# dfm/tinygp

Measured on AMD Instinct MI355X. Metric: GP log_probability evals/sec + Cholesky TFLOP/s (fp64), N=16,384, higher is better.
Workload: dtype f64; 1 GPU; c2: 1.5^2 ExpSquared(2.5), 1-D X, N=16384, fp64, diag=0.01, constant-density synthetic inputs (SURVEY 8d), dense Cholesky + tri-solve; n=16384, d=1, parallelism=single, nb_outer=1024

## Files before the change

### tinygp_amd/csrc/capi.hip

```cpp
#include <cmath>
#include <cstdlib>
#include <chrono>
#include <cstring>
#include <string>

#include "tgp_common.h"
#define CHAIN_HD __host__ __device__
#include "chain_tasks.h"
#define TILE_HD
#include "tile_order.h"

namespace tgp {

static thread_local std::string g_error;

void set_error(const char* fmt, ...) {
  char buf[1024];
  va_list ap;
  va_start(ap, fmt);
  vsnprintf(buf, sizeof(buf), fmt, ap);
  va_end(ap);
  g_error = buf;
}

// ... 17 lines not shown
}

int ensure_work(tgp_ctx* ctx, size_t bytes) { return grow(&ctx->d_work, &ctx->work_bytes, bytes); }

template <typename F>
static int dispatch(int dtype, F&& f) {
  if (dtype == TGP_F64) return f(double{});
  if (dtype == TGP_F32) return f(float{});
  set_error("dtype must be TGP_F32 (0) or TGP_F64 (1), got %d", dtype);
  return TGP_E_ARG;
}

static inline size_t esize(int dtype) { return dtype == TGP_F64 ? 8 : 4; }

}

using namespace tgp;

struct tgp_solver {
  tgp_ctx* ctx = nullptr;
  int dtype = TGP_F64;
  int64_t n = 0, npad = 0;
  int d = 1;
  void* X = nullptr;
  void* diag = nullptr;
  void* A = nullptr;
  void* dinv = nullptr;
  void* vec = nullptr;
  void* vec2 = nullptr;
  void* resid = nullptr;
  void* scratch = nullptr;
  void* Minv = nullptr;
  void* winv = nullptr;
  bool winv_valid = false;
  size_t scratch_bytes = 0;
  KProg kp{};
  bool has_prog = false, factored = false, has_resid = false;
  int32_t info = 0;
  double logdet_half = 0;
  double ms[8] = {0, 0, 0, 0, 0, 0, 0, 0};
};

#define CTX_GUARD(ctx)                                                \
  TGP_ARG_CHECK((ctx) != nullptr, "null context");                    \
  std::unique_lock<std::recursive_mutex> _tgp_lock((ctx)->mu);        \
  TGP_HIP_TRY(hipSetDevice((ctx)->device))

#define SOLVER_GUARD(s)                                               \
  TGP_ARG_CHECK((s) != nullptr && (s)->ctx != nullptr, "null solver"); \
  std::unique_lock<std::recursive_mutex> _tgp_lock((s)->ctx->mu);     \
  TGP_HIP_TRY(hipSetDevice((s)->ctx->device))

template <typename T>
static int assemble_lower(tgp_ctx* ctx, const tgp::KProg& kp, int64_t n, int d, const T* X,
                          const T* diag, T* A, int64_t npad) {
  using namespace tgp;
  const int64_t tc = npad / 128;
  int64_t t1 = tc;
  if (ctx->lookahead != 0 && ctx->asm_stream != nullptr) {
    int64_t nb = ctx->nb_outer / 128;
    if (nb < 1) nb = 1;
    nb = std::max<int64_t>(nb, first_panel_cols(ctx, npad) / 128);
    if (nb < tc) t1 = nb;
  }
  const int flags = KMAT_LOWER | KMAT_PAD_IDENTITY;
  if (t1 < tc) {
    TGP_TRY(ev_record(ctx, ctx->ev_asm, ctx->stream));
    TGP_TRY(st_wait(ctx, ctx->asm_stream, ctx->ev_asm));
  }
  TGP_TRY(launch_kmat_cols<T>(ctx, ctx->stream, kp, n, n, d, X, X, diag, A, npad, npad, npad, flags, 0, t1));
  if (t1 < tc) {
    auto side = [=]() -> int {
      TGP_TRY(launch_kmat_cols<T>(ctx, ctx->asm_stream, kp, n, n, d, X, X, diag, A, npad, npad, npad,
                                  flags, t1, tc - t1));
      return ev_record(ctx, ctx->ev_asm, ctx->asm_stream);
    };
    if (ctx->asm_defer != 0) {
      ctx->deferred_asm = side;
    } else {
      TGP_TRY(side());
    }
    ctx->asm_pending = true;
  }
  return TGP_OK;
}

template <typename T>
static int ensure_winv(tgp_solver* s) {
  if (s->winv_valid) return TGP_OK;
  if (!s->winv) TGP_HIP_TRY(hipMalloc(&s->winv, 4 * size_t(s->npad / TILE) * 16384 * sizeof(T)));
  TGP_TRY(compute_winv<T>(s->ctx, s->npad, (const T*)s->A, s->npad, (T*)s->winv));
  s->winv_valid = true;
  return TGP_OK;
}

extern "C" {

int tgp_abi_version(void) { return TGP_ABI_VERSION; }
const char* tgp_last_error(void) { return g_error.c_str(); }

int tgp_ctx_create(int device, void* stream, tgp_ctx** out) {
  TGP_ARG_CHECK(out != nullptr, "null output pointer");
  int count = 0;
  hipError_t e = hipGetDeviceCount(&count);
  if (e != hipSuccess || count <= 0) {
    set_error("no HIP device visible (%s); tinygp_amd has no CPU fallback",
              e == hipSuccess ? "device count 0" : hipGetErrorString(e));
    return TGP_E_HIP;
  }
  TGP_ARG_CHECK(device >= 0 && device < count, "device %d out of range (0..%d)", device, count - 1);
  TGP_HIP_TRY(hipSetDevice(device));
  tgp_ctx* ctx = new tgp_ctx();
  ctx->device = device;
  ctx->has_device = true;
  if (stream) {
    ctx->stream = static_cast<hipStream_t>(stream);
  } else {
    TGP_HIP_TRY(hipStreamCreateWithFlags(&ctx->stream, hipStreamNonBlocking));
    ctx->own_stream = true;
  }
  int lo = 0, hi = 0;
  TGP_HIP_TRY(hipDeviceGetStreamPriorityRange(&lo, &hi));
  {
    int can = 0;
    if (hipDeviceGetAttribute(&can, hipDeviceAttributeCanUseStreamWaitValue, device) != hipSuccess) can = 0;
    (void)hipGetLastError();
    ctx->can_wait_value = can == 1;
  }
  {
    const char* a = getenv("ROCPROF_COUNTER_COLLECTION");
    const char* b = getenv("TGP_SERIALIZED_KERNELS");
    auto on = [](const char* v) { return v != nullptr && *v && strcmp(v, "0") != 0 && strcasecmp(v, "false") != 0; };
    if (on(a) || on(b)) {
      ctx->serializing_tool = true;
      ctx->chain_polls = 0;
    }
  }
  TGP_HIP_TRY(hipStreamCreateWithPriority(&ctx->panel_stream, hipStreamNonBlocking, hi));
  TGP_HIP_TRY(hipStreamCreateWithPriority(&ctx->update_stream, hipStreamNonBlocking, hi));
  TGP_HIP_TRY(hipStreamCreateWithPriority(&ctx->asm_stream, hipStreamNonBlocking, lo));
  TGP_HIP_TRY(hipEventCreateWithFlags(&ctx->ev_asm, hipEventDisableTiming));
  TGP_HIP_TRY(hipEventCreateWithFlags(&ctx->ev_d, hipEventDisableTiming));
  TGP_HIP_TRY(hipEventCreateWithFlags(&ctx->ev_e, hipEventDisableTiming));
  TGP_HIP_TRY(hipEventCreateWithFlags(&ctx->ev_f, hipEventDisableTiming));
  TGP_HIP_TRY(hipEventCreateWithFlags(&ctx->ev_g1, hipEventDisableTiming));
  TGP_HIP_TRY(hipEventCreateWithFlags(&ctx->ev_g2, hipEventDisableTiming));
  TGP_HIP_TRY(hipEventCreateWithFlags(&ctx->ev_h, hipEventDisableTiming));
  TGP_HIP_TRY(hipEventCreateWithFlags(&ctx->ev_i, hipEventDisableTiming));
  TGP_HIP_TRY(hipEventCreateWithFlags(&ctx->ev_j, hipEventDisableTiming));
  TGP_HIP_TRY(hipEventCreateWithFlags(&ctx->ev_c, hipEventDisableTiming));
  TGP_HIP_TRY(hipEventCreateWithFlags(&ctx->ev_join, hipEventDisableTiming));
  TGP_HIP_TRY(hipEventCreateWithFlags(&ctx->ev_a, hipEventDisableTiming));
  TGP_HIP_TRY(hipEventCreateWithFlags(&ctx->ev_b, hipEventDisableTiming));
  TGP_HIP_TRY(hipMalloc(&ctx->d_scal, 16 * sizeof(double)));
  TGP_HIP_TRY(hipMalloc(&ctx->d_info, sizeof(int32_t)));
  TGP_HIP_TRY(hipMalloc(&ctx->d_step_flag, 64));
  TGP_HIP_TRY(hipMemset(ctx->d_step_flag, 0, 64));
  TGP_HIP_TRY(hipMalloc(&ctx->d_chain_flags, size_t(tgp::CHAIN_MAX_ROW_TILES) * 64 * sizeof(uint32_t)));
  TGP_HIP_TRY(hipMemset(ctx->d_chain_flags, 0, size_t(tgp::CHAIN_MAX_ROW_TILES) * 64 * sizeof(uint32_t)));
  TGP_HIP_TRY(hipMalloc(&ctx->d_chain_ticket, 4096));
  TGP_HIP_TRY(hipMemset(ctx->d_chain_ticket, 0, 4096));
  TGP_HIP_TRY(hipMalloc(&ctx->d_chain_red, size_t(2) * CHAIN_MAX_ROW_TILES * sizeof(double)));
  hipDeviceProp_t prop;
  TGP_HIP_TRY(hipGetDeviceProperties(&prop, device));
  ctx->cus = prop.multiProcessorCount;
  *out = ctx;
  return TGP_OK;
}

int tgp_ctx_destroy(tgp_ctx* ctx) {
  if (!ctx) return TGP_OK;
  hipSetDevice(ctx->device);
  hipStreamSynchronize(ctx->stream);
  if (ctx->panel_stream) hipStreamSynchronize(ctx->panel_stream);
  if (ctx->solve_stream) {
    hipStreamSynchronize(ctx->solve_stream);
    hipStreamDestroy(ctx->solve_stream);
  }
  if (ctx->ev_c) hipEventDestroy(ctx->ev_c);
  if (ctx->ev_join) hipEventDestroy(ctx->ev_join);
  if (ctx->ev_asm_gate) hipEventDestroy(ctx->ev_asm_gate);
  if (ctx->rescue_stream) hipStreamDestroy(ctx->rescue_stream);
  if (ctx->update_stream) {
    hipStreamSynchronize(ctx->update_stream);
    hipStreamDestroy(ctx->update_stream);
  }
  if (ctx->asm_stream) {
    hipStreamSynchronize(ctx->asm_stream);
    hipStreamDestroy(ctx->asm_stream);
  }
  if (ctx->ev_asm) hipEventDestroy(ctx->ev_asm);
  if (ctx->ev_d) hipEventDestroy(ctx->ev_d);
  if (ctx->ev_e) hipEventDestroy(ctx->ev_e);
  if (ctx->ev_f) hipEventDestroy(ctx->ev_f);
  if (ctx->ev_g1) hipEventDestroy(ctx->ev_g1);
  if (ctx->ev_g2) hipEventDestroy(ctx->ev_g2);
  if (ctx->ev_h) hipEventDestroy(ctx->ev_h);
  if (ctx->ev_i) hipEventDestroy(ctx->ev_i);
  if (ctx->ev_j) hipEventDestroy(ctx->ev_j);
  for (auto e : ctx->ev_pool) hipEventDestroy(e);
  if (ctx->ev_a) hipEventDestroy(ctx->ev_a);
  if (ctx->ev_b) hipEventDestroy(ctx->ev_b);
  if (ctx->d_scal) hipFree(ctx->d_scal);
  if (ctx->d_info) hipFree(ctx->d_info);
  if (ctx->d_step_flag) hipFree(ctx->d_step_flag);
  if (ctx->d_chain_flags) hipFree(ctx->d_chain_flags);
  if (ctx->d_chain_ticket) hipFree(ctx->d_chain_ticket);
  if (ctx->d_chain_red) hipFree(ctx->d_chain_red);
  if (ctx->d_chain_stamps) hipFree(ctx->d_chain_stamps);
  for (auto& kv : ctx->chain_tables)
    if (kv.second.dev) hipFree(kv.second.dev);
  if (ctx->d_dinv) hipFree(ctx->d_dinv);
  if (ctx->d_work) hipFree(ctx->d_work);
  if (ctx->d_gemm_ws) hipFree(ctx->d_gemm_ws);
  if (ctx->d_gemm_prefix_count) hipFree(ctx->d_gemm_prefix_count);
  if (ctx->panel_stream) hipStreamDestroy(ctx->panel_stream);
  if (ctx->own_stream && ctx->stream) hipStreamDestroy(ctx->stream);
  delete ctx;
  return TGP_OK;
}

int tgp_ctx_sync(tgp_ctx* ctx) {
  CTX_GUARD(ctx);
  TGP_HIP_TRY(hipStreamSynchronize(ctx->stream));
  return TGP_OK;
}

static int64_t* option_slot(tgp_ctx* ctx, const char* key) {
  if (!strcmp(key, "nb_outer")) return &ctx->nb_outer;
  if (!strcmp(key, "lookahead")) return &ctx->lookahead;
  if (!strcmp(key, "profile")) return &ctx->profile;
  if (!strcmp(key, "first_split")) return &ctx->first_split;
  if (!strcmp(key, "first_small_tiles")) return &ctx->first_small_tiles;
  if (!strcmp(key, "keep_grad_buffers")) return &ctx->keep_grad_buffers;
  if (!strcmp(key, "stream_trsv")) return &ctx->stream_trsv;
  if (!strcmp(key, "trsv_groups")) return &ctx->trsv_groups;
  if (!strcmp(key, "nb_wide_rows")) return &ctx->nb_wide_rows;
  if (!strcmp(key, "dist_solve_aux")) return &ctx->dist_solve_aux;
  if (!strcmp(key, "solve_on_update")) return &ctx->solve_on_update;
  if (!strcmp(key, "fused_step")) return &ctx->fused_step;
  if (!strcmp(key, "chain_kernel")) return &ctx->chain_kernel;
  if (!strcmp(key, "chain_stamps")) return &ctx->chain_stamps;
  if (!strcmp(key, "chain_full_rows")) return &ctx->chain_full_rows;
  if (!strcmp(key, "chain_lds_pad")) return &ctx->chain_lds_pad;
  if (!strcmp(key, "chain_depth2")) return &ctx->chain_depth2;
  if (!strcmp(key, "chain_merged")) return &ctx->chain_merged;
  if (!strcmp(key, "chain_sub_panel")) return &ctx->chain_sub_panel;
  if (!strcmp(key, "chain_sub_min_rows")) return &ctx->chain_sub_min_rows;
  if (!strcmp(key, "chain_sub_role")) return &ctx->chain_sub_role;
  if (!strcmp(key, "chain_pre_wait")) return &ctx->chain_pre_wait;
  if (!strcmp(key, "chain_gate_split")) return &ctx->chain_gate_split;
  if (!strcmp(key, "chain_polls")) return &ctx->chain_polls;
  if (!strcmp(key, "chain_fwd_tasks")) return &ctx->chain_fwd_tasks;
  if (!strcmp(key, "chain_fast_update")) return &ctx->chain_fast_update;
  if (!strcmp(key, "chain_batch")) return &ctx->chain_batch;
  if (!strcmp(key, "chain_batch_lag")) return &ctx->chain_batch_lag;
  if (!strcmp(key, "chain_batch_rowlag")) return &ctx->chain_batch_rowlag;
  if (!strcmp(key, "chain_batch_minrows")) return &ctx->chain_batch_minrows;
  if (!strcmp(key, "kmat_plain_div")) return &ctx->kmat_plain_div;
  if (!strcmp(key, "chain_reserve")) return &ctx->chain_reserve;
  if (!strcmp(key, "gate_split")) return &ctx->gate_split;
  if (!strcmp(key, "reserve_max_tiles")) return &ctx->reserve_max_tiles;
  if (!strcmp(key, "sub_panel")) return &ctx->sub_panel;
  if (!strcmp(key, "sub_panel_min_rows")) return &ctx->sub_panel_min_rows;
  if (!strcmp(key, "nb_first")) return &ctx->nb_first;
  if (!strcmp(key, "split_tail")) return &ctx->split_tail;
  if (!strcmp(key, "gemm_role")) return &ctx->gemm_role;
  if (!strcmp(key, "gemm_reserve")) return &ctx->gemm_reserve;
  if (!strcmp(key, "gemm_prefix_cols")) return &ctx->gemm_prefix_cols;
  if (!strcmp(key, "gemm_prefix_count")) return &ctx->gemm_prefix_count;
  if (!strcmp(key, "host_join")) return &ctx->host_join;
  if (!strcmp(key, "late_join")) return &ctx->late_join;
  if (!strcmp(key, "chain_reduce")) return &ctx->chain_reduce;
  if (!strcmp(key, "asm_defer")) return &ctx->asm_defer;
  if (!strcmp(key, "tile_band")) return &ctx->tile_band;
  if (!strcmp(key, "fault_inject")) return &ctx->fault_inject;
  if (!strcmp(key, "poll_timeout_ms")) return &ctx->poll_timeout_ms;
  if (!strcmp(key, "timeout_retries")) return &ctx->timeout_retries;
  return nullptr;
}

static int set_option_checked(tgp_ctx* ctx, const char* key, int64_t value, int64_t* old) {
  int64_t* slot = option_slot(ctx, key);
  TGP_ARG_CHECK(slot != nullptr, "unknown option '%s'", key);
  if (slot == &ctx->nb_outer)
    TGP_ARG_CHECK(value >= TILE && value % TILE == 0, "nb_outer must be a positive multiple of %d", TILE);
  if (slot == &ctx->sub_panel || slot == &ctx->nb_first)
    TGP_ARG_CHECK(value >= 0 && value % TILE == 0, "%s must be a multiple of %d (0: off)", key, TILE);
  if (slot == &ctx->chain_batch) TGP_ARG_CHECK(value >= 0 && value <= 32, "chain_batch must be in [0, 32]");
  if (slot == &ctx->chain_batch_lag) TGP_ARG_CHECK(value >= 1 && value <= 64, "chain_batch_lag must be in [1, 64]");
  if (slot == &ctx->chain_batch_minrows) TGP_ARG_CHECK(value >= 0 && value <= 4096, "chain_batch_minrows must be in [0, 4096]");
  if (slot == &ctx->chain_batch_rowlag) TGP_ARG_CHECK(value >= 2 && value <= 4096, "chain_batch_rowlag must be in [2, 4096]");
  if (old) *old = *slot;
  if (slot == &ctx->poll_timeout_ms && ctx->has_device) return set_poll_limit(ctx, value);
  *slot = value;
  return TGP_OK;
}

int tgp_ctx_set_option(tgp_ctx* ctx, const char* key, int64_t value, int64_t* old) {
  TGP_ARG_CHECK(ctx != nullptr && key != nullptr, "null argument");
  return set_option_checked(ctx, key, value, old);
}

int tgp_ctx_get_option(tgp_ctx* ctx, const char* key, int64_t* value) {
  TGP_ARG_CHECK(ctx != nullptr && key != nullptr && value != nullptr, "null argument");
  int64_t* slot = option_slot(ctx, key);
  TGP_ARG_CHECK(slot != nullptr, "unknown option '%s'", key);
  if (slot == &ctx->poll_timeout_ms && ctx->has_device) ctx->poll_timeout_ms = tgp::poll_limit_ms();
  *value = *slot;
  return TGP_OK;
}

static int apply_options(tgp_ctx* ctx, const char* options) {
  if (options == nullptr) return TGP_OK;
  std::string all(options);
  size_t pos = 0;
  while (pos < all.size()) {
    size_t end = all.find(',', pos);
    if (end == std::string::npos) end = all.size();
    const std::string item = all.substr(pos, end - pos);
    pos = end + 1;
    if (item.empty()) continue;
    const size_t eq = item.find('=');
    TGP_ARG_CHECK(eq != std::string::npos && eq > 0, "option '%s' is not key=value", item.c_str());
    char* stop = nullptr;
    const long long v = strtoll(item.c_str() + eq + 1, &stop, 10);
    TGP_ARG_CHECK(stop != nullptr && *stop == 0 && eq + 1 < item.size(), "option '%s': bad integer", item.c_str());
    TGP_TRY(set_option_checked(ctx, item.substr(0, eq).c_str(), (int64_t)v, nullptr));
  }
  return TGP_OK;
}

int tgp_ctx_device_info(tgp_ctx* ctx, char* name, int name_len, int32_t* cus, int64_t* mem_bytes,
                        int32_t* clock_khz) {
  CTX_GUARD(ctx);
  hipDeviceProp_t prop;
  TGP_HIP_TRY(hipGetDeviceProperties(&prop, ctx->device));
  if (name && name_len > 0) {
    snprintf(name, (size_t)name_len, "%s (%s)", prop.name, prop.gcnArchName);
  }
  if (cus) *cus = prop.multiProcessorCount;
  if (mem_bytes) *mem_bytes = (int64_t)prop.totalGlobalMem;
  if (clock_khz) *clock_khz = prop.clockRate;
  return TGP_OK;
}

int tgp_malloc(tgp_ctx* ctx, size_t bytes, void** dev) {
  CTX_GUARD(ctx);
  TGP_ARG_CHECK(dev != nullptr, "null output pointer");
  TGP_HIP_TRY(hipMalloc(dev, bytes ? bytes : 8));
  return TGP_OK;
}
int tgp_free(tgp_ctx* ctx, void* dev) {
  CTX_GUARD(ctx);
  if (dev) {
    TGP_HIP_TRY(hipStreamSynchronize(ctx->stream));
    TGP_HIP_TRY(hipFree(dev));
  }
  return TGP_OK;
}
int tgp_memcpy_h2d(tgp_ctx* ctx, void* dst, const void* src, size_t bytes) {
  CTX_GUARD(ctx);
  TGP_HIP_TRY(hipMemcpyAsync(dst, src, bytes, hipMemcpyHostToDevice, ctx->stream));
  TGP_HIP_TRY(hipStreamSynchronize(ctx->stream));
  return TGP_OK;
}
int tgp_memcpy_d2h(tgp_ctx* ctx, void* dst, const void* src, size_t bytes) {
  CTX_GUARD(ctx);
  TGP_HIP_TRY(hipMemcpyAsync(dst, src, bytes, hipMemcpyDeviceToHost, ctx->stream));
  TGP_HIP_TRY(hipStreamSynchronize(ctx->stream));
  return TGP_OK;
}
int tgp_memset(tgp_ctx* ctx, void* dst, int byte, size_t bytes) {
  CTX_GUARD(ctx);
  TGP_HIP_TRY(hipMemsetAsync(dst, byte, bytes, ctx->stream));
  return TGP_OK;
}

int tgp_kmat(tgp_ctx* ctx, int dtype, const tgp_kop* prog, int nops, int64_t n1, int64_t n2,
             int32_t d, const void* X1, const void* X2, const void* diag, void* out, int64_t ld,
             int64_t rows_out, int64_t cols_out, int lower_only) {
  CTX_GUARD(ctx);
  KProg kp;
  TGP_TRY(make_kprog(prog, nops, &kp));
  TGP_ARG_CHECK(n1 >= 0 && n2 >= 0 && X1 && X2 && out, "kmat: null or negative argument");
  return dispatch(dtype, [&](auto tag) {
    using T = decltype(tag);
    const int flags = (lower_only ? KMAT_LOWER : 0) | KMAT_PAD_IDENTITY;
    return launch_kmat<T>(ctx, kp, n1, n2, d, (const T*)X1, (const T*)X2, (const T*)diag, (T*)out,
                          ld, rows_out, cols_out, flags);
  });
}

int tgp_kdiag(tgp_ctx* ctx, int dtype, const tgp_kop* prog, int nops, int64_t n, int32_t d,
              const void* X, void* out) {
  CTX_GUARD(ctx);
  KProg kp;
  TGP_TRY(make_kprog(prog, nops, &kp));
  return dispatch(dtype, [&](auto tag) {
    using T = decltype(tag);
    return launch_kdiag<T>(ctx, kp, n, d, (const T*)X, (const T*)nullptr, (T*)out);
  });
}

int tgp_kmat_gemv(tgp_ctx* ctx, int dtype, const tgp_kop* prog, int nops, int64_t n1, int64_t n2,
                  int32_t d, const void* X1, const void* X2, const void* v, void* out) {
  CTX_GUARD(ctx);
  KProg kp;
  TGP_TRY(make_kprog(prog, nops, &kp));
  return dispatch(dtype, [&](auto tag) {
    using T = decltype(tag);
    return launch_kmat_gemv<T>(ctx, kp, n1, n2, d, (const T*)X1, (const T*)X2, (const T*)v, (T*)out);
  });
}

int tgp_kmat_gemv_multi(tgp_ctx* ctx, int dtype, const tgp_kop* prog, int nops, int64_t n1, int64_t n2,
                        int32_t d, const void* X1, const void* X2, const void* V, int64_t nv, void* out) {
  CTX_GUARD(ctx);
  KProg kp;
  TGP_TRY(make_kprog(prog, nops, &kp));
  TGP_ARG_CHECK(nv >= 1 && X1 && X2 && V && out, "kmat_gemv_multi: bad argument");
  return dispatch(dtype, [&](auto tag) {
    using T = decltype(tag);
    return launch_kmat_gemv_multi<T>(ctx, kp, n1, n2, d, (const T*)X1, (const T*)X2, (const T*)V, nv, (T*)out);
  });
}

int tgp_potrf(tgp_ctx* ctx, int dtype, int64_t n, void* A, int64_t ld, int32_t* info) {
  CTX_GUARD(ctx);
  TGP_ARG_CHECK(A != nullptr && n >= 0, "potrf: null matrix");
  TGP_TRY(ensure_dinv(ctx, size_t(n / TILE + 1) * 2048 * esize(dtype)));
  return dispatch(dtype, [&](auto tag) {
    using T = decltype(tag);
    return potrf<T>(ctx, n, (T*)A, ld, (T*)ctx->d_dinv, info);
  });
}

int tgp_trsv(tgp_ctx* ctx, int dtype, int64_t n, const void* L, int64_t ld, int transpose, void* y) {
  CTX_GUARD(ctx);
  TGP_TRY(ensure_dinv(ctx, size_t(n / TILE + 1) * 2048 * esize(dtype)));
  return dispatch(dtype, [&](auto tag) {
    using T = decltype(tag);
    TGP_TRY(compute_dinv<T>(ctx, n, (const T*)L, ld, (T*)ctx->d_dinv));
    return trsv<T>(ctx, n, (const T*)L, ld, (const T*)ctx->d_dinv, transpose, (T*)y);
  });
}

int tgp_trsm_right_lt(tgp_ctx* ctx, int dtype, int64_t m, int64_t n, const void* L, int64_t ldl,
                      void* B, int64_t ldb) {
  CTX_GUARD(ctx);
  TGP_TRY(ensure_dinv(ctx, size_t(n / TILE + 1) * 2048 * esize(dtype)));
  return dispatch(dtype, [&](auto tag) {
    using T = decltype(tag);
    TGP_TRY(compute_dinv<T>(ctx, n, (const T*)L, ldl, (T*)ctx->d_dinv));
    return trsm_right_lt<T>(ctx, m, n, (const T*)L, ldl, (const T*)ctx->d_dinv, (T*)B, ldb);
  });
}

int tgp_gemv_sub(tgp_ctx* ctx, int dtype, int64_t m, int64_t k, const void* P, int64_t ld,
                 const void* x, void* y) {
  CTX_GUARD(ctx);
  return dispatch(dtype, [&](auto tag) {
    using T = decltype(tag);
    return gemv_sub<T>(ctx, m, k, (const T*)P, ld, (const T*)x, (T*)y);
  });
}

int tgp_gemm_nt(tgp_ctx* ctx, int dtype, int64_t m, int64_t n, int64_t k, double alpha,
                const void* A, int64_t lda, const void* B, int64_t ldb, double beta, void* C,
                int64_t ldc, int lower) {
  CTX_GUARD(ctx);
  int mode;
  if (alpha == -1.0 && beta == 1.0) mode = 0;
  else if (alpha == 1.0 && beta == 0.0) mode = 1;
  else {
    set_error("gemm_nt: (alpha, beta) must be (-1, 1) or (1, 0)");
    return TGP_E_UNSUPPORTED;
  }
  const bool counted = ctx->gemm_role == 0 && ctx->gemm_prefix_cols > 0;
  if (ctx->gemm_role == 0) ctx->reserve_hint = ctx->gemm_reserve;
  if (counted) {
    if (!ctx->d_gemm_prefix_count) TGP_HIP_TRY(hipMalloc(&ctx->d_gemm_prefix_count, sizeof(int32_t)));
    TGP_HIP_TRY(hipMemsetAsync(ctx->d_gemm_prefix_count, 0, sizeof(int32_t), ctx->stream));
    ctx->prefix_hint_cols = ctx->gemm_prefix_cols;
    ctx->prefix_hint_counter = ctx->d_gemm_prefix_count;
  }
  const int rc = dispatch(dtype, [&](auto tag) {
    using T = decltype(tag);
    return launch_gemm_nt<T>(ctx, ctx->stream, m, n, k, (const T*)A, lda, (const T*)B, ldb, (T*)C,
                             ldc, lower, mode, (int)ctx->gemm_role);
  });
  ctx->reserve_hint = 0;
  ctx->prefix_hint_cols = 0;
  ctx->prefix_hint_counter = nullptr;
  if (counted && rc == TGP_OK) {
    int32_t done = 0;
    TGP_HIP_TRY(hipStreamSynchronize(ctx->stream));
    TGP_HIP_TRY(hipMemcpy(&done, ctx->d_gemm_prefix_count, sizeof(int32_t), hipMemcpyDeviceToHost));
    ctx->gemm_prefix_count = done;
  }
  return rc;
}

int tgp_sum_log_diag(tgp_ctx* ctx, int dtype, int64_t n, const void* L, int64_t ld, double* out) {
  CTX_GUARD(ctx);
  TGP_TRY(dispatch(dtype, [&](auto tag) {
    using T = decltype(tag);
    return launch_sum_log_diag<T>(ctx, n, (const T*)L, ld, 0);
  }));
  TGP_HIP_TRY(hipMemcpyAsync(out, ctx->d_scal, sizeof(double), hipMemcpyDeviceToHost, ctx->stream));
  TGP_HIP_TRY(hipStreamSynchronize(ctx->stream));
  return TGP_OK;
}

int tgp_sum_squares(tgp_ctx* ctx, int dtype, int64_t n, const void* y, double* out) {
  CTX_GUARD(ctx);
  TGP_TRY(dispatch(dtype, [&](auto tag) {
    using T = decltype(tag);
    return launch_sum_squares<T>(ctx, n, (const T*)y, 0);
  }));
  TGP_HIP_TRY(hipMemcpyAsync(out, ctx->d_scal, sizeof(double), hipMemcpyDeviceToHost, ctx->stream));
  TGP_HIP_TRY(hipStreamSynchronize(ctx->stream));
  return TGP_OK;
}

int tgp_ubench_mfma(tgp_ctx* ctx, int dtype, double* tflops_out) {
  CTX_GUARD(ctx);
  TGP_ARG_CHECK(tflops_out != nullptr && (dtype == TGP_F32 || dtype == TGP_F64), "bad argument");
  return ubench_mfma(ctx, dtype, tflops_out);
}

int tgp_ubench(tgp_ctx* ctx, int kind, int blocks_per_cu, double* tflops_out,
               double* cycles_per_op_out) {
  CTX_GUARD(ctx);
  TGP_ARG_CHECK(tflops_out != nullptr, "null output pointer");
  return ubench(ctx, kind, blocks_per_cu, tflops_out, cycles_per_op_out);
}

static int solver_scratch(tgp_solver* s, size_t bytes) {
  return tgp::grow(&s->scratch, &s->scratch_bytes, bytes);
}

int tgp_solver_create(tgp_ctx* ctx, int dtype, int64_t n, int32_t d, const void* X_host,
                      const void* noise_diag_host, tgp_solver** out) {
  CTX_GUARD(ctx);
  TGP_ARG_CHECK(out != nullptr, "null output pointer");
  TGP_ARG_CHECK(dtype == TGP_F32 || dtype == TGP_F64, "dtype must be TGP_F32 or TGP_F64");
  TGP_ARG_CHECK(n >= 1, "need at least one data point (n = %lld)", (long long)n);
  TGP_ARG_CHECK(d >= 1 && d <= TGP_MAX_DIM, "input dimension must be 1..%d (got %d)", TGP_MAX_DIM, d);
  TGP_ARG_CHECK(X_host != nullptr && noise_diag_host != nullptr, "null input array");
  tgp_solver* s = new tgp_solver();
  s->ctx = ctx;
  s->dtype = dtype;
  s->n = n;
  s->npad = round_up(n, TILE);
  s->d = d;
  const size_t es = esize(dtype);
  auto fail = [&](int code) { tgp_solver_destroy(s); return code; };
#define S_TRY(expr) do { hipError_t _e = (expr); if (_e != hipSuccess) { \
    set_error("%s failed: %s", #expr, hipGetErrorString(_e));            \
    return fail(_e == hipErrorOutOfMemory ? TGP_E_NOMEM : TGP_E_HIP); } } while (0)
  S_TRY(hipMalloc(&s->X, size_t(n) * d * es));
  S_TRY(hipMalloc(&s->diag, size_t(n) * es));
  S_TRY(hipMalloc(&s->A, size_t(s->npad) * s->npad * es));
  S_TRY(hipMalloc(&s->dinv, size_t(s->npad / TILE) * 2048 * es));
  S_TRY(hipMalloc(&s->vec, size_t(s->npad) * es));
  S_TRY(hipMalloc(&s->vec2, size_t(s->npad) * es));
  S_TRY(hipMalloc(&s->resid, size_t(s->npad) * es));
  S_TRY(hipMemcpyAsync(s->X, X_host, size_t(n) * d * es, hipMemcpyHostToDevice, ctx->stream));
  S_TRY(hipMemcpyAsync(s->diag, noise_diag_host, size_t(n) * es, hipMemcpyHostToDevice, ctx->stream));
  S_TRY(hipMemsetAsync(s->vec, 0, size_t(s->npad) * es, ctx->stream));
  S_TRY(hipMemsetAsync(s->vec2, 0, size_t(s->npad) * es, ctx->stream));
  S_TRY(hipMemsetAsync(s->resid, 0, size_t(s->npad) * es, ctx->stream));
  S_TRY(hipStreamSynchronize(ctx->stream));
#undef S_TRY
  *out = s;
  return TGP_OK;
}

int tgp_solver_destroy(tgp_solver* s) {
  if (!s) return TGP_OK;
  if (s->ctx) {
    hipSetDevice(s->ctx->device);
    hipStreamSynchronize(s->ctx->stream);
  }
  void* bufs[] = {s->X, s->diag, s->A, s->dinv, s->vec, s->vec2, s->resid, s->scratch, s->Minv, s->winv};
  for (void* b : bufs)
    if (b) hipFree(b);
  delete s;
  return TGP_OK;
}

int tgp_solver_set_noise(tgp_solver* s, const void* noise_diag_host) {
  SOLVER_GUARD(s);
  TGP_ARG_CHECK(noise_diag_host != nullptr, "null input array");
  TGP_HIP_TRY(hipMemcpyAsync(s->diag, noise_diag_host, size_t(s->n) * esize(s->dtype),
                             hipMemcpyHostToDevice, s->ctx->stream));
  TGP_HIP_TRY(hipStreamSynchronize(s->ctx->stream));
  return TGP_OK;
}

static int upload_vec(tgp_solver* s, void* dst, const void* src_host) {
  const size_t es = esize(s->dtype);
  TGP_HIP_TRY(hipMemcpyAsync(dst, src_host, size_t(s->n) * es, hipMemcpyHostToDevice, s->ctx->stream));
  if (s->npad > s->n)
    TGP_HIP_TRY(hipMemsetAsync((char*)dst + size_t(s->n) * es, 0, size_t(s->npad - s->n) * es,
                               s->ctx->stream));
  return TGP_OK;
}

static int factor_body(tgp_solver* s, const tgp_kop* prog, int nops, const void* cov_host,
                       int32_t* info, int fused, const void* resid_host, double* logprob);

static int factor_impl(tgp_solver* s, const tgp_kop* prog, int nops, const void* cov_host,
                       int32_t* info, int fused, const void* resid_host, double* logprob) {
  int st = factor_body(s, prog, nops, cov_host, info, fused, resid_host, logprob);
  if (st == TGP_E_TIMEOUT && s->ctx->chain_kernel != 0) {
    tgp_ctx* ctx = s->ctx;
    for (hipStream_t q : {ctx->asm_stream, ctx->panel_stream, ctx->update_stream, ctx->solve_stream, ctx->stream})
      if (q) (void)hipStreamSynchronize(q);
    (void)hipGetLastError();
    ctx->asm_pending = false;
    ctx->deferred_asm = nullptr;
    ctx->ev_used = 0;
    ctx->timeout_retries++;
    const int64_t keep = ctx->chain_kernel;
    ctx->chain_kernel = 0;
    st = factor_body(s, prog, nops, cov_host, info, fused, resid_host, logprob);
    ctx->chain_kernel = keep;
  }
  if (st < 0) {
    tgp_ctx* ctx = s->ctx;
    ctx->asm_pending = false;
    ctx->deferred_asm = nullptr;
    ctx->ev_used = 0;
    s->factored = false;
    for (hipStream_t q : {ctx->asm_stream, ctx->panel_stream, ctx->update_stream, ctx->solve_stream,
                          ctx->stream})
      if (q) (void)hipStreamSynchronize(q);
    (void)hipGetLastError();
  }
  return st;
}

static int factor_body(tgp_solver* s, const tgp_kop* prog, int nops, const void* cov_host,
                       int32_t* info, int fused, const void* resid_host, double* logprob) {
  tgp_ctx* ctx = s->ctx;
  if (nops > 0) {
    TGP_TRY(make_kprog(prog, nops, &s->kp));
    s->has_prog = true;
  } else {
    s->has_prog = false;
  }
  TGP_ARG_CHECK(s->has_prog || cov_host != nullptr, "factor needs a kernel program or a covariance");
  s->winv_valid = false;
  const auto host0 = std::chrono::steady_clock::now();
  const size_t es = esize(s->dtype);
  hipEvent_t e0 = nullptr, e1 = nullptr, e2 = nullptr;
  const bool prof = ctx->profile != 0;
  if (prof) {
    TGP_HIP_TRY(hipEventCreate(&e0));
    TGP_HIP_TRY(hipEventCreate(&e1));
    TGP_HIP_TRY(hipEventCreate(&e2));
    TGP_HIP_TRY(hipEventRecord(e0, ctx->stream));
  }
  int status = dispatch(s->dtype, [&](auto tag) {
    using T = decltype(tag);
    T* A = (T*)s->A;
    if (fused) {
      if (resid_host) {
        TGP_TRY(upload_vec(s, s->vec, resid_host));
      } else {
        TGP_ARG_CHECK(s->has_resid, "no resident residual: call tgp_solver_set_resid first");
        TGP_HIP_TRY(hipMemcpyAsync(s->vec, s->resid, size_t(s->npad) * es, hipMemcpyDeviceToDevice,
                                   ctx->stream));
      }
    }
    if (cov_host != nullptr) {
      TGP_TRY(solver_scratch(s, size_t(s->n) * s->n * es));
      TGP_HIP_TRY(hipMemcpyAsync(s->scratch, cov_host, size_t(s->n) * s->n * es,
                                 hipMemcpyHostToDevice, ctx->stream));
      TGP_TRY(launch_set_lower_from_rowmajor<T>(ctx, s->n, s->npad, (const T*)s->scratch, A, s->npad));
    } else {
      TGP_TRY(assemble_lower<T>(ctx, s->kp, s->n, s->d, (const T*)s->X, (const T*)s->diag, A, s->npad));
    }
    if (prof) TGP_HIP_TRY(hipEventRecord(e1, ctx->stream));
    int32_t inf = 0;
    ctx->defer_join = ctx->late_join != 0;
    ctx->join_deferred = false;
    reductions_begin(ctx, s->npad, fused != 0);
    int st = potrf<T>(ctx, s->npad, A, s->npad, (T*)s->dinv, &inf, fused ? (T*)s->vec : (T*)nullptr);
    ctx->defer_join = false;
    const bool reduce = reductions_end(ctx);
    if (st < 0) return st;
    s->info = inf;
    if (prof) TGP_HIP_TRY(hipEventRecord(e2, ctx->stream));
    if (reduce) {
      TGP_TRY(launch_sum_log_diag<T>(ctx, s->n, A, s->npad, 1));
      if (fused) TGP_TRY(launch_sum_squares<T>(ctx, s->n, (const T*)s->vec, 0));
    }
    return TGP_OK;
  });
  if (status < 0) return status;
  double two[2] = {0, 0};
  int32_t inf_late = 0;
  const bool late = ctx->join_deferred;
  ctx->join_deferred = false;
  TGP_HIP_TRY(hipMemcpyAsync(two, ctx->d_scal, 2 * sizeof(double), hipMemcpyDeviceToHost, ctx->stream));
  if (late) TGP_HIP_TRY(hipMemcpyAsync(&inf_late, ctx->d_info, sizeof(int32_t), hipMemcpyDeviceToHost, ctx->stream));
  TGP_HIP_TRY(hipStreamSynchronize(ctx->stream));
  if (late) {
    if (inf_late == INT32_MIN) {
      tgp::set_error("potrf: a device-side hand-off did not arrive within poll_timeout_ms (a lost or starved chain launch)");
      if (prof) { hipEventDestroy(e0); hipEventDestroy(e1); hipEventDestroy(e2); }
      return TGP_E_TIMEOUT;
    }
    s->info = inf_late;
  }
  s->ms[5] = std::chrono::duration<double, std::milli>(ctx->submitted - host0).count();
  s->logdet_half = two[1];
  if (fused && logprob)
    *logprob = -0.5 * two[0] - (s->logdet_half + 0.5 * double(s->n) * std::log(2.0 * M_PI));
  if (prof) {
    float a = 0, b = 0;
    TGP_HIP_TRY(hipEventElapsedTime(&a, e0, e1));
    TGP_HIP_TRY(hipEventElapsedTime(&b, e1, e2));
    s->ms[0] = a;
    s->ms[1] = b;
    s->ms[2] = ctx->prof_syrk_ms;
    s->ms[3] = (double)ctx->prof_syrk_launches;
    s->ms[6] = ctx->prof_syrk_flops;
    s->ms[7] = ctx->prof_syrk_union_ms;
    hipEventDestroy(e0);
    hipEventDestroy(e1);
    hipEventDestroy(e2);
  }
  s->factored = true;
  if (info) *info = s->info;
  return s->info > 0 ? s->info : TGP_OK;
}

int tgp_solver_factor(tgp_solver* s, const tgp_kop* prog, int nops, const void* cov_host,
                      int32_t* info) {
  SOLVER_GUARD(s);
  return factor_impl(s, prog, nops, cov_host, info, 0, nullptr, nullptr);
}

int tgp_solver_factor_logprob(tgp_solver* s, const tgp_kop* prog, int nops, const void* cov_host,
                              const void* resid_host, int32_t* info, double* logprob) {
  SOLVER_GUARD(s);
  TGP_ARG_CHECK(logprob != nullptr, "null output pointer");
  return factor_impl(s, prog, nops, cov_host, info, 1, resid_host, logprob);
}

#define NEED_FACTOR(s) TGP_ARG_CHECK((s)->factored, "solver has not been factored yet")

int tgp_solver_normalization(tgp_solver* s, double* out) {
  SOLVER_GUARD(s);
  NEED_FACTOR(s);
  TGP_ARG_CHECK(out != nullptr, "null output pointer");
  *out = s->logdet_half + 0.5 * double(s->n) * std::log(2.0 * M_PI);
  return TGP_OK;
}

int tgp_solver_solve_tri(tgp_solver* s, int transpose, int64_t nrhs, const void* y_host,
                         void* x_host) {
  SOLVER_GUARD(s);
  NEED_FACTOR(s);
  TGP_ARG_CHECK(nrhs >= 1 && y_host && x_host, "solve_tri: bad argument");
  tgp_ctx* ctx = s->ctx;
  const size_t es = esize(s->dtype);
  return dispatch(s->dtype, [&](auto tag) {
    using T = decltype(tag);
    const T* L = (const T*)s->A;
    if (nrhs == 1) {
      TGP_TRY(upload_vec(s, s->vec, y_host));
      const T* winv = nullptr;
      if (ctx->stream_trsv != 0 && s->info == 0) {
        TGP_TRY(ensure_winv<T>(s));
        winv = (const T*)s->winv;
      }
      TGP_TRY(trsv<T>(ctx, s->npad, L, s->npad, (const T*)s->dinv, transpose, (T*)s->vec, winv));
      TGP_HIP_TRY(hipMemcpyAsync(x_host, s->vec, size_t(s->n) * es, hipMemcpyDeviceToHost, ctx->stream));
      TGP_HIP_TRY(hipStreamSynchronize(ctx->stream));
      return TGP_OK;
    }
    if (!transpose) {
      const int64_t mpad = round_up(nrhs, TILE);
      TGP_TRY(solver_scratch(s, size_t(mpad) * s->npad * es));
      TGP_HIP_TRY(hipMemsetAsync(s->scratch, 0, size_t(mpad) * s->npad * es, ctx->stream));
      TGP_HIP_TRY(hipMemcpy2DAsync(s->scratch, size_t(mpad) * es, y_host, size_t(nrhs) * es,
                                   size_t(nrhs) * es, size_t(s->n), hipMemcpyHostToDevice, ctx->stream));
      TGP_TRY(trsm_right_lt<T>(ctx, mpad, s->npad, L, s->npad, (const T*)s->dinv, (T*)s->scratch, mpad));
      TGP_HIP_TRY(hipMemcpy2DAsync(x_host, size_t(nrhs) * es, s->scratch, size_t(mpad) * es,
                                   size_t(nrhs) * es, size_t(s->n), hipMemcpyDeviceToHost, ctx->stream));
      TGP_HIP_TRY(hipStreamSynchronize(ctx->stream));
      return TGP_OK;
    }
    const T* winv_t = nullptr;
    if (ctx->stream_trsv != 0 && s->info == 0) {
      TGP_TRY(ensure_winv<T>(s));
      winv_t = (const T*)s->winv;
    }
    for (int64_t r = 0; r < nrhs; ++r) {
      TGP_HIP_TRY(hipMemsetAsync(s->vec, 0, size_t(s->npad) * es, ctx->stream));
      TGP_HIP_TRY(hipMemcpy2DAsync(s->vec, es, (const char*)y_host + r * es, size_t(nrhs) * es, es,
                                   size_t(s->n), hipMemcpyHostToDevice, ctx->stream));
      TGP_TRY(trsv<T>(ctx, s->npad, L, s->npad, (const T*)s->dinv, 1, (T*)s->vec, winv_t));
      TGP_HIP_TRY(hipMemcpy2DAsync((char*)x_host + r * es, size_t(nrhs) * es, s->vec, es, es,
                                   size_t(s->n), hipMemcpyDeviceToHost, ctx->stream));
    }
    TGP_HIP_TRY(hipStreamSynchronize(ctx->stream));
    return TGP_OK;
  });
}

int tgp_solver_dot_tri(tgp_solver* s, int64_t nrhs, const void* y_host, void* out_host) {
  SOLVER_GUARD(s);
  NEED_FACTOR(s);
  TGP_ARG_CHECK(nrhs >= 1 && y_host && out_host, "dot_tri: bad argument");
  tgp_ctx* ctx = s->ctx;
  const size_t es = esize(s->dtype);
  return dispatch(s->dtype, [&](auto tag) {
    using T = decltype(tag);
    if (nrhs >= 8) {
      const int64_t mpad = round_up(nrhs, TILE);
      const size_t bytes = size_t(mpad) * s->npad * es;
      TGP_TRY(solver_scratch(s, 2 * bytes));
      char* Zt = (char*)s->scratch;
      char* Ct = Zt + bytes;
      TGP_HIP_TRY(hipMemsetAsync(Zt, 0, bytes, ctx->stream));
      TGP_HIP_TRY(hipMemcpy2DAsync(Zt, size_t(mpad) * es, y_host, size_t(nrhs) * es, size_t(nrhs) * es,
                                   size_t(s->n), hipMemcpyHostToDevice, ctx->stream));
      TGP_TRY(launch_gemm_nt<T>(ctx, ctx->stream, mpad, s->npad, s->npad, (const T*)Zt, mpad,
                                (const T*)s->A, s->npad, (T*)Ct, mpad, 0, 3, 1));
      TGP_HIP_TRY(hipMemcpy2DAsync(out_host, size_t(nrhs) * es, Ct, size_t(mpad) * es, size_t(nrhs) * es,
                                   size_t(s->n), hipMemcpyDeviceToHost, ctx->stream));
      TGP_HIP_TRY(hipStreamSynchronize(ctx->stream));
      return TGP_OK;
    }
    for (int64_t r = 0; r < nrhs; ++r) {
      TGP_HIP_TRY(hipMemcpy2DAsync(s->vec, es, (const char*)y_host + r * es, size_t(nrhs) * es, es,
                                   size_t(s->n), hipMemcpyHostToDevice, ctx->stream));
      TGP_TRY(launch_trmv_lower<T>(ctx, s->n, (const T*)s->A, s->npad, (const T*)s->vec, (T*)s->vec2));
      TGP_HIP_TRY(hipMemcpy2DAsync((char*)out_host + r * es, size_t(nrhs) * es, s->vec2, es, es,
                                   size_t(s->n), hipMemcpyDeviceToHost, ctx->stream));
    }
    TGP_HIP_TRY(hipStreamSynchronize(ctx->stream));
    return TGP_OK;
  });
}

int tgp_solver_set_resid(tgp_solver* s, const void* resid_host) {
  SOLVER_GUARD(s);
  TGP_ARG_CHECK(resid_host != nullptr, "null input array");
  TGP_TRY(upload_vec(s, s->resid, resid_host));
  TGP_HIP_TRY(hipStreamSynchronize(s->ctx->stream));
  s->has_resid = true;
  return TGP_OK;
}

static int logprob_device(tgp_solver* s, const void* resid_host, double* out) {
  tgp_ctx* ctx = s->ctx;
// ... 425 lines not shown
```

### tinygp_amd/csrc/chol.hip

```cpp
#include <algorithm>
#include <atomic>
#include <functional>
#include <type_traits>

#include <thread>

#include "tgp_common.h"
#define CHAIN_HD __host__ __device__
#include "chain_tasks.h"

namespace tgp {

namespace {

typedef double d4 __attribute__((ext_vector_type(4)));
typedef float f4 __attribute__((ext_vector_type(4)));

template <typename T> struct Mfma;
template <> struct Mfma<double> {
  using acc_t = d4;
  static __device__ __forceinline__ acc_t mma(double a, double b, acc_t c) {
    return __builtin_amdgcn_mfma_f64_16x16x4f64(a, b, c, 0, 0, 0);
  }
  static __device__ __forceinline__ int drow(int lane, int r) { return (lane >> 4) + 4 * r; }
  static constexpr bool FAST4 = false;
  static __device__ __forceinline__ double mma4(double a, double b, double c) {
    return __builtin_amdgcn_mfma_f64_4x4x4f64(a, b, c, 0, 0, 0);
  }
  static __device__ __forceinline__ int rot4(int lane, int t) { return 4 * ((((lane >> 2) & 3) + t) & 3) + (lane & 3); }
  static __device__ __forceinline__ int arow4(int lane) { return 4 * ((lane >> 2) & 3) + (lane >> 4); }
};
template <> struct Mfma<float> {
  using acc_t = f4;
  static __device__ __forceinline__ acc_t mma(float a, float b, acc_t c) {
    return __builtin_amdgcn_mfma_f32_16x16x4f32(a, b, c, 0, 0, 0);
  }
  static __device__ __forceinline__ int drow(int lane, int r) { return (lane >> 4) * 4 + r; }
  static constexpr bool FAST4 = false;
  static __device__ __forceinline__ float mma4(float a, float b, float c) { return c + a * b; }
  static __device__ __forceinline__ int rot4(int lane, int t) { return (lane + t) & 15; }
  static __device__ __forceinline__ int arow4(int lane) { return lane & 15; }
};

__device__ __forceinline__ double fast_rcp(double x) {
  double r = __builtin_amdgcn_rcp(x);
  double e = __builtin_fma(-x, r, 1.0);
  r = __builtin_fma(r, e, r);
  e = __builtin_fma(-x, r, 1.0);
  return __builtin_fma(r, e, r);
}
__device__ __forceinline__ float fast_rcp(float x) {
  float r = __builtin_amdgcn_rcpf(x);
  float e = __builtin_fmaf(-x, r, 1.0f);
  return __builtin_fmaf(r, e, r);
}
__device__ __forceinline__ double fast_rsqrt(double x) {
  double y = __builtin_amdgcn_rsq(x);
  double e = __builtin_fma(-x * y, y, 1.0);
  y = __builtin_fma(0.5 * y, e, y);
  e = __builtin_fma(-x * y, y, 1.0);
  return __builtin_fma(0.5 * y, e, y);
}
__device__ __forceinline__ float fast_rsqrt(float x) {
  float y = __builtin_amdgcn_rsqf(x);
  float e = __builtin_fmaf(-x * y, y, 1.0f);
  return __builtin_fmaf(0.5f * y, e, y);
}

__device__ __forceinline__ double readlane(double v, int lane) {
  int lo = __double2loint(v), hi = __double2hiint(v);
  lo = __builtin_amdgcn_readlane(lo, lane);
  hi = __builtin_amdgcn_readlane(hi, lane);
  return __hiloint2double(hi, lo);
}
__device__ __forceinline__ float readlane(float v, int lane) {
  return __int_as_float(__builtin_amdgcn_readlane(__float_as_int(v), lane));
}

#define TGP_HD __device__ __forceinline__
#include "potf2_layout.h"
#define TGP_OPAQUE_VGPR(x) asm volatile("" : "+v"(x))

#ifdef TGP_POTF2_STAMPS
__device__ long long g_potf2_stamps[64];
#define POTF2_STAMP(i) do { if (threadIdx.x == 0) g_potf2_stamps[i] = __builtin_readcyclecounter(); } while (0)
#else
#define POTF2_STAMP(i) do {} while (0)
#endif

__device__ void potf2_prefix_wait(const int32_t* count, int32_t target, int32_t* info);

template <typename T, bool FOLD>
__global__ __launch_bounds__(512) __attribute__((amdgpu_waves_per_eu(4, 4))) void potf2_kernel(T* __restrict__ A, int64_t ld,
                                                    T* __restrict__ dinv,
                                                    int32_t* __restrict__ info,
                                                    int32_t pivot_base,
                                                    const T* __restrict__ Xp, int64_t ldx,
                                                    const int32_t* __restrict__ wait_count, int32_t wait_target) {
  __shared__ __attribute__((aligned(16))) T S[36 * 256];
  __shared__ T Rs[2 * 16];
  __shared__ T Dg[256];
  if (wait_count != nullptr) {
    if (threadIdx.x == 0) potf2_prefix_wait(wait_count, wait_target, info);
    __syncthreads();
  }
#include "potf2_body.inc"
}

constexpr int32_t STEP_TIMEOUT = INT32_MIN;

__device__ long long g_poll_limit = 400000000LL;
struct PollClock {
  long long t0 = 0;
  __device__ __forceinline__ bool expired(long spin) {
    if ((spin & 255) != 255) return false;
    const long long now = (long long)__builtin_amdgcn_s_memrealtime();
    if (t0 == 0) {
      t0 = now;
      return false;
    }
    return now - t0 > __hip_atomic_load(&g_poll_limit, __ATOMIC_RELAXED, __HIP_MEMORY_SCOPE_AGENT);
  }
};
__device__ __forceinline__ bool poisoned(const int32_t* info) {
  return __hip_atomic_load(info, __ATOMIC_RELAXED, __HIP_MEMORY_SCOPE_AGENT) == STEP_TIMEOUT;
}

template <typename T, bool FOLD>
__device__ __forceinline__ void trsm_fold_body(T* S, int it, const T* __restrict__ Ljj,
                                               int64_t ld, const T* __restrict__ dinv,
                                               const T* __restrict__ Xp, const uint32_t* flag,
                                               uint32_t epoch, int wait_flag, int32_t* info) {
  using M = Mfma<T>;
  using acc_t = typename M::acc_t;
  typedef T T2 __attribute__((ext_vector_type(2)));
  const int tid = threadIdx.x, lane = tid & 63;
  const int w = __builtin_amdgcn_readfirstlane(tid >> 6);
  const int lrow = lane & 15, lk = lane >> 4;
  __builtin_amdgcn_s_setprio(2);
  T* Bt = const_cast<T*>(Ljj) + TILE + int64_t(it) * TILE;

  if constexpr (FOLD) {
    constexpr int FK = 16, F_LD = 144;
    static_assert(4 * FK * F_LD == 36 * 256, "the fold's operand buffers are exactly potf2's tile image");
    T* sA = S;
    T* sB = S + 2 * FK * F_LD;
    const T* Xi = Xp + TILE + int64_t(it) * TILE;
    const int wr = w >> 1, wc = w & 1;
    T2 ra[2], rb[2];
    auto load_global = [&](int kt) {
#pragma unroll
      for (int r = 0; r < 2; ++r) {
        const int64_t kk = int64_t(kt) * FK + w + 8 * r;
        ra[r] = *reinterpret_cast<const T2*>(Xi + kk * ld + lane * 2);
        rb[r] = *reinterpret_cast<const T2*>(Xp + kk * ld + lane * 2);
      }
    };
    auto store_lds = [&](int buf) {
#pragma unroll
      for (int r = 0; r < 2; ++r) {
        const int kk = w + 8 * r;
        *reinterpret_cast<T2*>(&sA[buf * FK * F_LD + kk * F_LD + lane * 2]) = ra[r];
        *reinterpret_cast<T2*>(&sB[buf * FK * F_LD + kk * F_LD + lane * 2]) = rb[r];
      }
    };
    acc_t acc[4][2];
#pragma unroll
    for (int a = 0; a < 4; ++a)
#pragma unroll
      for (int b = 0; b < 2; ++b) acc[a][b] = acc_t{0, 0, 0, 0};
    load_global(0);
    store_lds(0);
    __syncthreads();
    constexpr int nkt = TILE / FK;
    for (int kt = 0; kt < nkt; ++kt) {
      const int buf = kt & 1;
      if (kt + 1 < nkt) load_global(kt + 1);
      const T* pa = &sB[buf * FK * F_LD + lk * F_LD + wc * 64 + lrow];
      const T* pb = &sA[buf * FK * F_LD + lk * F_LD + wr * 32 + lrow];
#pragma unroll
      for (int ks = 0; ks < FK / 4; ++ks) {
        T aop[4], bop[2];
#pragma unroll
        for (int a = 0; a < 4; ++a) aop[a] = pa[ks * 4 * F_LD + a * 16];
#pragma unroll
        for (int b = 0; b < 2; ++b) bop[b] = pb[ks * 4 * F_LD + b * 16];
#pragma unroll
        for (int a = 0; a < 4; ++a)
#pragma unroll
          for (int b = 0; b < 2; ++b) acc[a][b] = M::mma(aop[a], bop[b], acc[a][b]);
      }
      if (kt + 1 < nkt) store_lds(buf ^ 1);
      __syncthreads();
    }
    T* Cu = Bt + int64_t(wc * 64) * ld + wr * 32;
    const uint32_t coff = uint32_t(M::drow(lane, 0) * int(ld) + lrow);
#pragma unroll
    for (int a = 0; a < 4; ++a) {
      T c[2][4];
#pragma unroll
      for (int b = 0; b < 2; ++b)
#pragma unroll
        for (int r = 0; r < 4; ++r) c[b][r] = (Cu + int64_t(a * 16 + M::drow(0, r)) * ld + b * 16)[coff];
#pragma unroll
      for (int b = 0; b < 2; ++b)
#pragma unroll
        for (int r = 0; r < 4; ++r) (Cu + int64_t(a * 16 + M::drow(0, r)) * ld + b * 16)[coff] = c[b][r] - acc[a][b][r];
      __builtin_amdgcn_sched_barrier(0);
    }
    __syncthreads();
  }

  T* bu = Bt + w * 16;
  const uint32_t boff = uint32_t(M::drow(lane, 0) * int(ld) + lrow);
  acc_t V[8];
#pragma unroll
  for (int jb = 0; jb < 8; ++jb)
#pragma unroll
    for (int r = 0; r < 4; ++r) V[jb][r] = (bu + int64_t(jb * 16 + M::drow(0, r)) * ld)[boff];
  asm volatile("s_waitcnt vmcnt(0)" ::: "memory");
  __builtin_amdgcn_sched_barrier(0);

  if (wait_flag) {
    if (tid == 0) {
      uint32_t seen = __hip_atomic_load(flag, __ATOMIC_RELAXED, __HIP_MEMORY_SCOPE_AGENT);
      PollClock clk;
      for (unsigned spin = 0; seen != epoch; ++spin) {
        __builtin_amdgcn_s_sleep(2);
        seen = __hip_atomic_load(flag, __ATOMIC_RELAXED, __HIP_MEMORY_SCOPE_AGENT);
        if (clk.expired(spin)) break;
      }
      if (seen != epoch) atomicExch(info, STEP_TIMEOUT);
      __builtin_amdgcn_fence(__ATOMIC_ACQUIRE, "agent");
    }
    __syncthreads();
  }

  {
    T tr[5][4];
#pragma unroll
    for (int trip = 0; trip < 5; ++trip) {
      const int b = w + 8 * trip;
      if (b < 36) {
        int i = 0;
        while ((i + 1) * (i + 2) / 2 <= b) ++i;
        const int j = b - i * (i + 1) / 2;
        if (i == j) {
#pragma unroll
          for (int q = 0; q < 4; ++q) tr[trip][q] = dinv[i * 256 + q * 64 + lane];
        } else {
          const int voff = lk * int(ld) + lrow;
#pragma unroll
          for (int q = 0; q < 4; ++q) tr[trip][q] = (Ljj + int64_t(j * 16 + q * 4) * ld + i * 16)[voff];
        }
      }
    }
#pragma unroll
    for (int trip = 0; trip < 5; ++trip) {
      const int b = w + 8 * trip;
      if (b < 36) {
#pragma unroll
        for (int q = 0; q < 4; ++q) S[b * 256 + q * 64 + lane] = tr[trip][q];
      }
    }
  }
  __syncthreads();
  T* bs = bu;
  asm volatile("" : "+s"(bs));
#pragma unroll
  for (int jb = 0; jb < 8; ++jb) {
    acc_t acc = V[jb], acc2 = acc_t{0, 0, 0, 0};
#pragma unroll
    for (int kb = 0; kb < jb; ++kb) {
      const T* Lb = &S[blk(jb, kb)];
#pragma unroll
      for (int s = 0; s < 4; ++s) {
        const T l = Lb[M::drow(lane, s) * 16 + lrow];
        if (s & 1) acc2 = M::mma(l, V[kb][s], acc2);
        else acc = M::mma(l, V[kb][s], acc);
      }
    }
    acc += acc2;
    const T* Db = &S[blk(jb, jb)];
    acc_t y = acc_t{0, 0, 0, 0}, y2 = acc_t{0, 0, 0, 0};
#pragma unroll
    for (int s = 0; s < 4; ++s) {
      const T d = Db[M::drow(lane, s) * 16 + lrow];
      if (s & 1) y2 = M::mma(d, acc[s], y2);
      else y = M::mma(d, acc[s], y);
    }
    y += y2;
#pragma unroll
    for (int r = 0; r < 4; ++r) (bs + int64_t(jb * 16 + M::drow(0, r)) * ld)[boff] = y[r];
    V[jb] = -y;
  }
}

template <typename T, bool FOLD>
__global__ __launch_bounds__(512) __attribute__((amdgpu_waves_per_eu(4, 4))) void panel_step_kernel(
    T* __restrict__ A, int64_t ld, T* __restrict__ dinv, int32_t* __restrict__ info, int32_t pivot_base,
    const T* __restrict__ Xp, int has_p, uint32_t* __restrict__ flag, uint32_t epoch) {
  __shared__ __attribute__((aligned(16))) T S[36 * 256];
  __shared__ T Rs[2 * 16];
  __shared__ T Dg[256];
  const int b = __builtin_amdgcn_readfirstlane(blockIdx.x);
  if (b < has_p) {
    {
      const int64_t ldx = ld;
#include "potf2_body.inc"
    }
    asm volatile("s_waitcnt vmcnt(0)" ::: "memory");
    __syncthreads();
    if (threadIdx.x == 0) {
      __builtin_amdgcn_fence(__ATOMIC_RELEASE, "agent");
      asm volatile("s_waitcnt vmcnt(0)" ::: "memory");
      __hip_atomic_store(flag, epoch, __ATOMIC_RELAXED, __HIP_MEMORY_SCOPE_AGENT);
    }
    return;
  }
  trsm_fold_body<T, FOLD>(S, b - has_p, A, ld, dinv, Xp, flag, epoch, has_p, info);
}

template <typename T> struct AgentBits;
template <> struct AgentBits<double> { using t = unsigned long long; };
template <> struct AgentBits<float> { using t = unsigned int; };
template <typename T>
__device__ __forceinline__ void st_agent(T* p, T v) {
  typename AgentBits<T>::t b;
  __builtin_memcpy(&b, &v, sizeof(T));
  __hip_atomic_store(reinterpret_cast<typename AgentBits<T>::t*>(p), b, __ATOMIC_RELAXED, __HIP_MEMORY_SCOPE_AGENT);
}

__device__ __forceinline__ void chain_stamp(long long* st, int k) {
  if (st != nullptr && threadIdx.x == 0) st[4 + k] = (long long)__builtin_amdgcn_s_memrealtime();
}

constexpr int CHAIN_FLAG_LD = 64;
constexpr uint32_t CHAIN_FINAL = 127;
constexpr int CHAIN_COLCNT_OFF = 16;
constexpr int CHAIN_QCNT_OFF = 96;
constexpr int CHAIN_XSTEP_OFF = 160;
constexpr int CHAIN_ZFLAG_OFF = 224;
constexpr int CHAIN_YSTATE_OFF = 288;
constexpr int CHAIN_TICKET_WORDS = CHAIN_YSTATE_OFF + int(CHAIN_MAX_ROW_TILES) / CHAIN_FWD_GROUP;
constexpr int CHAIN_PREFIX_OFF = CHAIN_TICKET_WORDS + 16;

template <typename T>
struct ChainArgs {
  T* A0;
  int64_t ld;
  T* dinv;
  int32_t* info;
  uint32_t* flags;
  int32_t* ticket;
  uint32_t epoch32;
  int32_t pivot_base;
  int32_t R;
  int32_t nblk;
  int32_t cb, ce;
  long long* stamps;
  int32_t launch;
  int32_t fast_update;
  const uint64_t* tasks;
  T* y;
  int32_t fgs;
  int32_t fprev;
  double* red;
  double* scal;
  int32_t red_total;
};

template <int NAP>
__device__ __forceinline__ void chain_wait(const uint32_t* f0, uint32_t v0, const uint32_t* f1, uint32_t v1,
                                           const uint32_t* f2, uint32_t v2, int32_t* info) {
  if (threadIdx.x < 64) {
    const int lane = threadIdx.x;
    const uint32_t* f = lane == 0 ? f0 : (lane == 1 ? f1 : (lane == 2 ? f2 : nullptr));
    const uint32_t want = lane == 0 ? v0 : (lane == 1 ? v1 : v2);
    bool ok = f == nullptr || __hip_atomic_load(f, __ATOMIC_RELAXED, __HIP_MEMORY_SCOPE_AGENT) == want;
    unsigned spin = 0;
    PollClock clk;
    while (!__all(ok)) {
      __builtin_amdgcn_s_sleep(NAP);
      if (!ok) ok = __hip_atomic_load(f, __ATOMIC_RELAXED, __HIP_MEMORY_SCOPE_AGENT) == want;
      bool dead = false;
      if ((spin & 255) == 255 && lane == 0)
        dead = clk.expired(spin) || poisoned(info);
      ++spin;
      if (__any(dead)) {
        if (lane == 0) atomicExch(info, STEP_TIMEOUT);
        break;
      }
    }
    if (lane == 0) __builtin_amdgcn_fence(__ATOMIC_ACQUIRE, "agent");
  }
  __syncthreads();
}

__device__ __forceinline__ void chain_publish(uint32_t* word, uint32_t value, int32_t* colcnt = nullptr) {
  asm volatile("s_waitcnt vmcnt(0)" ::: "memory");
  __syncthreads();
  if (threadIdx.x == 0) {
    __hip_atomic_store(word, value, __ATOMIC_RELAXED, __HIP_MEMORY_SCOPE_AGENT);
    if (colcnt != nullptr) __hip_atomic_fetch_add(colcnt, 1, __ATOMIC_RELAXED, __HIP_MEMORY_SCOPE_AGENT);
  }
}

__device__ void potf2_prefix_wait(const int32_t* count, int32_t target, int32_t* info) {
  PollClock clk;
  for (unsigned spin = 0;; ++spin) {
    if (__hip_atomic_load(count, __ATOMIC_RELAXED, __HIP_MEMORY_SCOPE_AGENT) >= target) break;
    __builtin_amdgcn_s_sleep(8);
    if ((spin & 255) == 255 && (clk.expired(spin) || poisoned(info))) {
      atomicExch(info, STEP_TIMEOUT);
      break;
    }
  }
  __builtin_amdgcn_fence(__ATOMIC_ACQUIRE, "agent");
}

__global__ __launch_bounds__(64) void chain_poll_kernel(const int32_t* __restrict__ count, int32_t target,
                                                        int32_t* __restrict__ info) {
  if (threadIdx.x != 0) return;
  PollClock clk;
  for (unsigned spin = 0;; ++spin) {
    if (__hip_atomic_load(count, __ATOMIC_RELAXED, __HIP_MEMORY_SCOPE_AGENT) >= target) break;
    __builtin_amdgcn_s_sleep(16);
    if ((spin & 255) == 255 && (clk.expired(spin) || poisoned(info))) {
      atomicExch(info, STEP_TIMEOUT);
      break;
    }
  }
}

template <typename T, int PARTS>
__device__ __forceinline__ void chain_update_full(const ChainArgs<T>& q, T* S, int i, int c, int k, int part) {
  static_assert(PARTS == 1 || PARTS == 4 || PARTS == 8, "whole tile, row quarters or row eighths");
  using M = Mfma<T>;
  using acc_t = typename M::acc_t;
  typedef T T2 __attribute__((ext_vector_type(2)));
  const int tid = threadIdx.x, lane = tid & 63;
  const int w = __builtin_amdgcn_readfirstlane(tid >> 6);
  const int lrow = lane & 15, lk = lane >> 4;
  const int64_t ld = q.ld;
  constexpr int FK = 16, F_LD = 144;
  static_assert(4 * FK * F_LD == 36 * 256, "the operand buffers are exactly potf2's tile image");
  T* sA = S;
  T* sB = S + 2 * FK * F_LD;
  const int rbase = PARTS == 1 ? (w >> 1) * 32 : (PARTS == 4 ? part * 32 : part * 16);
  const int cbase = PARTS == 1 ? (w & 1) * 64 : w * 16;
  constexpr int NA = PARTS == 1 ? 4 : 1;
  constexpr int NBR = PARTS == 8 ? 1 : 2;
  acc_t acc[NA][NBR];
#pragma unroll
  for (int a = 0; a < NA; ++a)
#pragma unroll
    for (int b = 0; b < NBR; ++b) acc[a][b] = acc_t{0, 0, 0, 0};
  const T* Xi = q.A0 + int64_t(k) * TILE * ld + int64_t(i) * TILE;
  const T* Xj = q.A0 + int64_t(k) * TILE * ld + int64_t(c) * TILE;
  T2 ra[2], rb[2];
  auto load_global = [&](int kt) {
#pragma unroll
    for (int r = 0; r < 2; ++r) {
      const int64_t kk = int64_t(kt) * FK + w + 8 * r;
      ra[r] = *reinterpret_cast<const T2*>(Xi + kk * ld + lane * 2);
      rb[r] = *reinterpret_cast<const T2*>(Xj + kk * ld + lane * 2);
    }
  };
  auto store_lds = [&](int buf) {
#pragma unroll
    for (int r = 0; r < 2; ++r) {
      const int kk = w + 8 * r;
      *reinterpret_cast<T2*>(&sA[buf * FK * F_LD + kk * F_LD + lane * 2]) = ra[r];
      *reinterpret_cast<T2*>(&sB[buf * FK * F_LD + kk * F_LD + lane * 2]) = rb[r];
    }
  };
  int rot[4];
#pragma unroll
  for (int t = 0; t < 4; ++t) rot[t] = M::rot4(lane, t);
  load_global(0);
  store_lds(0);
  __syncthreads();
  constexpr int nkt = TILE / FK;
  for (int kt = 0; kt < nkt; ++kt) {
    const int buf = kt & 1;
    if (kt + 1 < nkt) load_global(kt + 1);
    const T* pa = &sB[buf * FK * F_LD + lk * F_LD + cbase + lrow];
    if constexpr (M::FAST4) {
      const T* pb = &sA[buf * FK * F_LD + lk * F_LD + rbase];
#pragma unroll
      for (int ks = 0; ks < FK / 4; ++ks) {
        T aop[NA];
#pragma unroll
        for (int a = 0; a < NA; ++a) aop[a] = pa[ks * 4 * F_LD + a * 16];
#pragma unroll
        for (int b = 0; b < NBR; ++b) {
          T bop[4];
#pragma unroll
          for (int t = 0; t < 4; ++t) bop[t] = pb[ks * 4 * F_LD + b * 16 + rot[t]];
#pragma unroll
          for (int a = 0; a < NA; ++a)
#pragma unroll
            for (int t = 0; t < 4; ++t) acc[a][b][t] = M::mma4(aop[a], bop[t], acc[a][b][t]);
        }
      }
    } else {
      const T* pb = &sA[buf * FK * F_LD + lk * F_LD + rbase + lrow];
#pragma unroll
      for (int ks = 0; ks < FK / 4; ++ks) {
        T aop[NA], bop[NBR];
#pragma unroll
        for (int a = 0; a < NA; ++a) aop[a] = pa[ks * 4 * F_LD + a * 16];
#pragma unroll
        for (int b = 0; b < NBR; ++b) bop[b] = pb[ks * 4 * F_LD + b * 16];
#pragma unroll
        for (int a = 0; a < NA; ++a)
#pragma unroll
          for (int b = 0; b < NBR; ++b) acc[a][b] = M::mma(aop[a], bop[b], acc[a][b]);
      }
    }
    if (kt + 1 < nkt) store_lds(buf ^ 1);
    __syncthreads();
  }
  T* Cu = q.A0 + int64_t(c) * TILE * ld + int64_t(i) * TILE + int64_t(cbase) * ld + rbase;
  if constexpr (M::FAST4) {
    const int64_t ccol = M::arow4(lane);
#pragma unroll
    for (int a = 0; a < NA; ++a) {
      T cc[NBR][4];
      T* col = Cu + (int64_t(a * 16) + ccol) * ld;
#pragma unroll
      for (int b = 0; b < NBR; ++b)
#pragma unroll
        for (int t = 0; t < 4; ++t) cc[b][t] = col[b * 16 + rot[t]];
#pragma unroll
      for (int b = 0; b < NBR; ++b)
#pragma unroll
        for (int t = 0; t < 4; ++t) st_agent(col + b * 16 + rot[t], T(cc[b][t] - acc[a][b][t]));
      __builtin_amdgcn_sched_barrier(0);
    }
  } else {
    const uint32_t coff = uint32_t(M::drow(lane, 0) * int(ld) + lrow);
#pragma unroll
    for (int a = 0; a < NA; ++a) {
      T cc[NBR][4];
#pragma unroll
      for (int b = 0; b < NBR; ++b)
#pragma unroll
        for (int r = 0; r < 4; ++r) cc[b][r] = (Cu + int64_t(a * 16 + M::drow(0, r)) * ld + b * 16)[coff];
#pragma unroll
      for (int b = 0; b < NBR; ++b)
#pragma unroll
        for (int r = 0; r < 4; ++r)
          st_agent(Cu + int64_t(a * 16 + M::drow(0, r)) * ld + b * 16 + coff, T(cc[b][r] - acc[a][b][r]));
      __builtin_amdgcn_sched_barrier(0);
    }
  }
}

__device__ __forceinline__ void chain_update_fast(const ChainArgs<double>& q, double* S, int i, int c, int k, int k1) {
  using M = Mfma<double>;
  const int tid = threadIdx.x, lane = tid & 63;
  const int wu = __builtin_amdgcn_readfirstlane(tid >> 6);
  const int wr = wu >> 1, wc = wu & 1;
  const int lk = lane >> 4, lrow = lane & 15;
  constexpr int FK = 16, F_LD = 144;
  const int64_t ld = q.ld;
  const double* Xi = q.A0 + int64_t(k) * TILE * ld + int64_t(i) * TILE;
  const double* Xj = q.A0 + int64_t(k) * TILE * ld + int64_t(c) * TILE;
  double* sA = S;
  double* sB = S + 2 * FK * F_LD;
  const uint32_t lds_a = uint32_t(size_t((__attribute__((address_space(3))) double*)(sA))) + uint32_t(wu * F_LD * 8);
  const uint32_t lds_b = uint32_t(size_t((__attribute__((address_space(3))) double*)(sB))) + uint32_t(wu * F_LD * 8);
  const uint32_t lane16 = uint32_t(lane) * 16u;
  auto issue_tile = [&](int kt, int buf) {
#pragma unroll
    for (int r = 0; r < 2; ++r) {
      const double* ap = Xi + (int64_t(kt) * FK + wu + 8 * r) * ld;
      const double* bp = Xj + (int64_t(kt) * FK + wu + 8 * r) * ld;
// ... 130 lines not shown
        for (int tt = 0; tt < 5; ++tt) {
          if (tt < nt) {
            const int t = t0 + tt;
            const bool first = t <= pr;
            const int jj = first ? t : t - pr - 1;
            Cf[tt] = M::mma(row[jj * 16], first ? b1 : b2, Cf[tt]);
          }
        }
      }
    }
  }
  T* Acc = q.A0 + int64_t(c) * TILE * ld + int64_t(c) * TILE;
#pragma unroll
  for (int tt = 0; tt < 5; ++tt) {
    if (tt < nt) {
      const int t = t0 + tt;
      const bool first = t <= pr;
      const int ii = first ? i1 : i2, jj = first ? t : t - pr - 1;
#pragma unroll
      for (int r = 0; r < 4; ++r) {
        const int br = M::FAST4 ? M::rot4(lane, r) : lrow, bc = M::FAST4 ? M::arow4(lane) : M::drow(lane, r);
        T* pe = Acc + int64_t(jj * 16 + bc) * ld + ii * 16 + br;
        st_agent(pe, T(*pe - Cf[tt][r]));
      }
    }
  }
}

template <typename T>
__device__ __forceinline__ void chain_load_tile(const ChainArgs<T>& q, int i, int c, typename Mfma<T>::acc_t (&V)[8]) {
  using M = Mfma<T>;
  const int lane = threadIdx.x & 63;
  const int w = __builtin_amdgcn_readfirstlane(threadIdx.x >> 6);
  const int64_t ld = q.ld;
  const T* bu = q.A0 + int64_t(c) * TILE * ld + int64_t(i) * TILE + w * 16;
  const uint32_t boff = uint32_t(M::drow(lane, 0) * int(ld) + (lane & 15));
#pragma unroll
  for (int jb = 0; jb < 8; ++jb)
#pragma unroll
    for (int r = 0; r < 4; ++r) V[jb][r] = (bu + int64_t(jb * 16 + M::drow(0, r)) * ld)[boff];
  asm volatile("s_waitcnt vmcnt(0)" ::: "memory");
  __builtin_amdgcn_sched_barrier(0);
}

template <typename T>
__device__ __forceinline__ void chain_solve(const ChainArgs<T>& q, T* S, int i, int c,
                                            typename Mfma<T>::acc_t (&V)[8], long long* st, int s0) {
  using M = Mfma<T>;
  using acc_t = typename M::acc_t;
  const int tid = threadIdx.x, lane = tid & 63;
  const int w = __builtin_amdgcn_readfirstlane(tid >> 6);
  const int lrow = lane & 15, lk = lane >> 4;
  const int64_t ld = q.ld;
  T* Bt = q.A0 + int64_t(c) * TILE * ld + int64_t(i) * TILE;
  const T* Ljj = q.A0 + int64_t(c) * TILE * ld + int64_t(c) * TILE;
  const T* dinv = q.dinv + int64_t(c) * 2048;
  T* bu = Bt + w * 16;
  const uint32_t boff = uint32_t(M::drow(lane, 0) * int(ld) + lrow);
#pragma unroll
  for (int round = 0; round < 2; ++round) {
    constexpr int NTR = 3;
    T tr[NTR][4];
    const int t_lo = round * NTR, t_n = round == 0 ? NTR : 5 - NTR;
#pragma unroll
    for (int tq = 0; tq < NTR; ++tq) {
      const int b = w + 8 * (t_lo + tq);
      if (tq < t_n && b < 36) {
        int bi = 0;
        while ((bi + 1) * (bi + 2) / 2 <= b) ++bi;
        const int bj = b - bi * (bi + 1) / 2;
        if (bi == bj) {
#pragma unroll
          for (int qq = 0; qq < 4; ++qq) tr[tq][qq] = dinv[bi * 256 + qq * 64 + lane];
        } else {
          const int voff = lk * int(ld) + lrow;
#pragma unroll
          for (int qq = 0; qq < 4; ++qq) tr[tq][qq] = (Ljj + int64_t(bj * 16 + qq * 4) * ld + bi * 16)[voff];
        }
      }
    }
#pragma unroll
    for (int tq = 0; tq < NTR; ++tq) {
      const int b = w + 8 * (t_lo + tq);
      if (tq < t_n && b < 36) {
#pragma unroll
        for (int qq = 0; qq < 4; ++qq) S[b * 256 + qq * 64 + lane] = tr[tq][qq];
      }
    }
    __builtin_amdgcn_sched_barrier(0);
  }
  __syncthreads();
  chain_stamp(st, s0);
  T* bs = bu;
  asm volatile("" : "+s"(bs));
#pragma unroll
  for (int jb = 0; jb < 8; ++jb) {
    acc_t acc = V[jb], acc2 = acc_t{0, 0, 0, 0};
#pragma unroll
    for (int kb = 0; kb < jb; ++kb) {
      const T* Lb = &S[blk(jb, kb)];
#pragma unroll
      for (int s = 0; s < 4; ++s) {
        const T l = Lb[M::drow(lane, s) * 16 + lrow];
        if (s & 1) acc2 = M::mma(l, V[kb][s], acc2);
        else acc = M::mma(l, V[kb][s], acc);
      }
    }
    acc += acc2;
    const T* Db = &S[blk(jb, jb)];
    acc_t y = acc_t{0, 0, 0, 0}, y2 = acc_t{0, 0, 0, 0};
#pragma unroll
    for (int s = 0; s < 4; ++s) {
      const T d = Db[M::drow(lane, s) * 16 + lrow];
      if (s & 1) y2 = M::mma(d, acc[s], y2);
      else y = M::mma(d, acc[s], y);
    }
    y += y2;
#pragma unroll
    for (int r = 0; r < 4; ++r) st_agent(bs + int64_t(jb * 16 + M::drow(0, r)) * ld + boff, T(y[r]));
    V[jb] = -y;
  }
  chain_stamp(st, s0 + 1);
}

template <typename T>
struct ChainStream {
  static constexpr int XC_LD = 144;
  static constexpr int LC = 8 * 256;
  static constexpr int XC = 16 * XC_LD;
  static_assert(2 * (LC + XC) <= 36 * 256, "both double buffers live in S");
};

__device__ __forceinline__ uint32_t chain_wave_wait_ge(const uint32_t* word, uint32_t want, int32_t* info) {
  PollClock clk;
  for (unsigned spin = 0;; ++spin) {
    const uint32_t v = __hip_atomic_load(word, __ATOMIC_RELAXED, __HIP_MEMORY_SCOPE_AGENT);
    if (int32_t(v - want) >= 0 && int32_t(v - want) < 128) return v;
    __builtin_amdgcn_s_sleep(1);
    if ((spin & 255) == 255 && (clk.expired(spin) || poisoned(info))) {
      if ((threadIdx.x & 63) == 0) atomicExch(info, STEP_TIMEOUT);
      return want;
    }
  }
}

__device__ __forceinline__ void chain_lds_barrier() {
  asm volatile("s_waitcnt lgkmcnt(0)\n\ts_barrier" ::: "memory");
}

__device__ __forceinline__ int chain_wave_wait_count(const int32_t* p, int want, int32_t* info) {
  PollClock clk;
  for (unsigned spin = 0;; ++spin) {
    const int v = __hip_atomic_load(p, __ATOMIC_RELAXED, __HIP_MEMORY_SCOPE_AGENT);
    if (v >= want) return v;
    __builtin_amdgcn_s_sleep(1);
    if ((spin & 255) == 255 && (clk.expired(spin) || poisoned(info))) {
      if ((threadIdx.x & 63) == 0) atomicExch(info, STEP_TIMEOUT);
      return want;
    }
  }
}

template <typename T>
__device__ __forceinline__ void chain_xsolve_stream(const ChainArgs<T>& q, T* S, int i, int c,
                                                    typename Mfma<T>::acc_t (&V)[8], const uint32_t* steps,
                                                    const uint32_t* final_word, uint32_t E, int32_t* xstep) {
  using M = Mfma<T>;
  using acc_t = typename M::acc_t;
  using CS = ChainStream<T>;
  using bits_t = typename AgentBits<T>::t;
  const int lane = threadIdx.x & 63;
  const int w = __builtin_amdgcn_readfirstlane(threadIdx.x >> 6);
  const int lrow = lane & 15, lk = lane >> 4;
  const int64_t ld = q.ld;
  const T* Ljj = q.A0 + int64_t(c) * TILE * ld + int64_t(c) * TILE;
  const T* dinv = q.dinv + int64_t(c) * 2048;
  T* bs = q.A0 + int64_t(c) * TILE * ld + int64_t(i) * TILE + w * 16;
  asm volatile("" : "+s"(bs));
  const uint32_t boff = uint32_t(M::drow(lane, 0) * int(ld) + lrow);
  T tr[4];
  auto issue_loads = [&](int jn) {
    const int bi = jn + w;
    if (bi < 8) {
      const T* src = bi == jn ? dinv + jn * 256 + lane : Ljj + int64_t(jn * 16) * ld + bi * 16 + (lk * int(ld) + lrow);
      const int64_t stride = bi == jn ? 64 : 4 * ld;
#pragma unroll
      for (int qq = 0; qq < 4; ++qq) {
        const bits_t u = __hip_atomic_load(reinterpret_cast<const bits_t*>(src + qq * stride), __ATOMIC_RELAXED,
                                           __HIP_MEMORY_SCOPE_AGENT);
        __builtin_memcpy(&tr[qq], &u, sizeof(T));
      }
    }
  };
  int known = steps == nullptr ? 8 : 0;
  bool have = false;
#pragma unroll
  for (int j = 0; j < 8; ++j) {
    T* Lc = S + (j & 1) * CS::LC;
    if (!have) {
      if (known <= j) {
        if (j < 7) known = int(chain_wave_wait_ge(steps, E + uint32_t(j + 1), q.info) - E);
        else { chain_wave_wait_ge(final_word, E + CHAIN_FINAL, q.info); known = 8; }
        known = __builtin_amdgcn_readfirstlane(known);
      }
      issue_loads(j);
    }
    if (j + w < 8) {
#pragma unroll
      for (int qq = 0; qq < 4; ++qq) Lc[w * 256 + qq * 64 + lane] = tr[qq];
    }
    if (j >= 1) asm volatile("s_waitcnt vmcnt(0)" ::: "memory");
    chain_lds_barrier();
    if (j >= 1 && threadIdx.x == 0) __hip_atomic_store(xstep, j, __ATOMIC_RELAXED, __HIP_MEMORY_SCOPE_AGENT);
    have = j < 7 && known > j + 1;
    if (have) issue_loads(j + 1);
    {
      acc_t y = acc_t{0, 0, 0, 0}, y2 = acc_t{0, 0, 0, 0};
#pragma unroll
      for (int s = 0; s < 4; ++s) {
        const T d = Lc[M::drow(lane, s) * 16 + lrow];
        if (s & 1) y2 = M::mma(d, V[j][s], y2);
        else y = M::mma(d, V[j][s], y);
      }
      y += y2;
#pragma unroll
      for (int r = 0; r < 4; ++r) st_agent(bs + int64_t(j * 16 + M::drow(0, r)) * ld + boff, T(y[r]));
      V[j] = -y;
    }
#pragma unroll
    for (int jb = j + 1; jb < 8; ++jb) {
      const T* Lb = Lc + (jb - j) * 256;
#pragma unroll
      for (int s = 0; s < 4; ++s) V[jb] = M::mma(Lb[M::drow(lane, s) * 16 + lrow], V[j][s], V[jb]);
    }
  }
}

template <typename T>
__device__ __forceinline__ void chain_fold_stream(const ChainArgs<T>& q, T* S, int i, int c,
                                                  typename Mfma<T>::acc_t (&Cf)[5], const int32_t* xstep) {
  using M = Mfma<T>;
  using acc_t = typename M::acc_t;
  using CS = ChainStream<T>;
  using bits_t = typename AgentBits<T>::t;
  const int lane = threadIdx.x & 63;
  const int w = __builtin_amdgcn_readfirstlane(threadIdx.x >> 6);
  const int lrow = lane & 15, lk = lane >> 4;
  const int64_t ld = q.ld;
  const T* bu = q.A0 + int64_t(c) * TILE * ld + int64_t(i) * TILE + w * 16;
  const uint32_t boff = uint32_t(M::drow(lane, 0) * int(ld) + lrow);
  const int pr = w & 3, i1 = pr, i2 = 7 - pr;
  const int t0 = (w < 4) ? 0 : 5, nt = (w < 4) ? 5 : 4;
#pragma unroll
  for (int tt = 0; tt < 5; ++tt) Cf[tt] = acc_t{0, 0, 0, 0};
  T xr[4];
  auto issue_loads = [&](int jn) {
#pragma unroll
    for (int r = 0; r < 4; ++r) {
      const bits_t u = __hip_atomic_load(reinterpret_cast<const bits_t*>(bu + int64_t(jn * 16 + M::drow(0, r)) * ld + boff),
                                         __ATOMIC_RELAXED, __HIP_MEMORY_SCOPE_AGENT);
      __builtin_memcpy(&xr[r], &u, sizeof(T));
    }
  };
  int known = xstep == nullptr ? 8 : 0;
  bool have = false;
#pragma unroll
  for (int j = 0; j < 8; ++j) {
    T* Xc = S + (j & 1) * CS::XC;
    if (!have) {
      if (known <= j) known = __builtin_amdgcn_readfirstlane(chain_wave_wait_count(xstep, j + 1, q.info));
      issue_loads(j);
    }
#pragma unroll
    for (int r = 0; r < 4; ++r) Xc[(r * 4 + lk) * CS::XC_LD + w * 16 + lrow] = xr[r];
    chain_lds_barrier();
    have = j < 7 && known > j + 1;
    if (have) issue_loads(j + 1);
#pragma unroll
    for (int ks = 0; ks < 4; ++ks) {
      const T* row = &Xc[(ks * 4 + lk) * CS::XC_LD + lrow];
      const T b1 = row[i1 * 16], b2 = row[i2 * 16];
#pragma unroll
      for (int tt = 0; tt < 5; ++tt) {
        if (tt < nt) {
          const int t = t0 + tt;
          const bool first = t <= pr;
          const int jj = first ? t : t - pr - 1;
          Cf[tt] = M::mma(row[jj * 16], first ? b1 : b2, Cf[tt]);
        }
      }
    }
  }
}

__device__ __forceinline__ void chain_wait_counts(const int32_t* p0, int want0, const int32_t* p1, int want1,
                                                  const int32_t* p2, int want2, int32_t* info) {
  if (threadIdx.x < 64) {
    const int lane = threadIdx.x;
    const int32_t* f = lane == 0 ? p0 : (lane == 1 ? p1 : (lane == 2 ? p2 : nullptr));
    const int want = lane == 0 ? want0 : (lane == 1 ? want1 : want2);
    auto ready = [&]() {
      const int v = __hip_atomic_load(f, __ATOMIC_RELAXED, __HIP_MEMORY_SCOPE_AGENT);
      return lane == 1 ? v == want : v >= want;
    };
    bool ok = f == nullptr || ready();
    unsigned spin = 0;
    PollClock clk;
    while (!__all(ok)) {
      __builtin_amdgcn_s_sleep(4);
      if (!ok) ok = ready();
      bool dead = false;
      if ((spin & 255) == 255 && lane == 0) dead = clk.expired(spin) || poisoned(info);
      ++spin;
      if (__any(dead)) {
        if (lane == 0) atomicExch(info, STEP_TIMEOUT);
        break;
      }
    }
    if (lane == 0) __builtin_amdgcn_fence(__ATOMIC_ACQUIRE, "agent");
  }
  __syncthreads();
}

template <typename T>
__device__ __forceinline__ void chain_fsolve(const ChainArgs<T>& q, T* S, int c, bool prev) {
  const int r = threadIdx.x, rb = (r >> 4) & 7, rl = r & 15;
  const bool act = r < 128;
  const int64_t ld = q.ld;
  const T* Lkk = q.A0 + int64_t(c) * TILE * ld + int64_t(c) * TILE;
  const T* dinv = q.dinv + int64_t(c) * 2048;
  T* y = q.y + int64_t(c) * TILE;
  T* st = S;
  T* sx = S + 128;
  T* sz = S + 256;
  T t = act ? y[r] : T(0);
  if (prev) {
    if (act) sz[r] = y[r - TILE];
    __syncthreads();
    if (act) {
      const T* Xp = Lkk - int64_t(TILE) * ld + r;
      T a0 = 0, a1 = 0;
#pragma unroll 1
      for (int j0 = 0; j0 < TILE; j0 += 16) {
        T v[16];
#pragma unroll
        for (int j = 0; j < 16; ++j) v[j] = Xp[int64_t(j0 + j) * ld];
#pragma unroll
        for (int j = 0; j < 16; j += 2) {
          a0 += v[j] * sz[j0 + j];
          a1 += v[j + 1] * sz[j0 + j + 1];
        }
      }
      t -= a0 + a1;
    }
  }
  T di[16];
#pragma unroll
  for (int qq = 0; qq < 16; ++qq) di[qq] = act ? dinv[rb * 256 + qq * 16 + rl] : T(0);
#pragma unroll 1
  for (int jb = 0; jb < 8; ++jb) {
    T cur[16];
    const bool below = act && rb > jb;
#pragma unroll
    for (int qq = 0; qq < 16; ++qq) cur[qq] = below ? Lkk[int64_t(jb * 16 + qq) * ld + r] : T(0);
    if (act) st[r] = t;
    __syncthreads();
    if (act && rb == jb) {
      T x = 0;
#pragma unroll
      for (int qq = 0; qq < 16; ++qq) x += di[qq] * st[jb * 16 + qq];
      sx[rl] = x;
      t = x;
    }
    __syncthreads();
    if (below) {
#pragma unroll
      for (int qq = 0; qq < 16; ++qq) t -= cur[qq] * sx[qq];
    }
  }
  if (act) st_agent(y + r, t);
  if (q.red != nullptr) {
    __syncthreads();
    double* ra = reinterpret_cast<double*>(S);
    double* rq = ra + 128;
    if (act) {
      const double zv = double(t);
      ra[r] = zv * zv;
      rq[r] = log(double(Lkk[int64_t(r) * ld + r]));
    }
    __syncthreads();
    for (int sft = 64; sft > 0; sft >>= 1) {
      if (r < sft) {
        ra[r] += ra[r + sft];
        rq[r] += rq[r + sft];
      }
      __syncthreads();
    }
    const int g = q.pivot_base / TILE + c;
    if (r == 0) {
      st_agent(q.red + 2 * g, ra[0]);
      st_agent(q.red + 2 * g + 1, rq[0]);
    }
    if (q.red_total > 0 && g == q.red_total - 1) {
      asm volatile("s_waitcnt vmcnt(0)" ::: "memory");
      __syncthreads();
      double* ta = ra + 256;
      double* tb = ta + 512;
      double a = 0, b = 0;
      for (int gg = r; gg < q.red_total; gg += 512) {
        const unsigned long long ua = __hip_atomic_load(reinterpret_cast<const unsigned long long*>(q.red + 2 * gg), __ATOMIC_RELAXED,
                                                        __HIP_MEMORY_SCOPE_AGENT);
        const unsigned long long ub = __hip_atomic_load(reinterpret_cast<const unsigned long long*>(q.red + 2 * gg + 1),
                                                        __ATOMIC_RELAXED, __HIP_MEMORY_SCOPE_AGENT);
        a += __longlong_as_double((long long)ua);
        b += __longlong_as_double((long long)ub);
      }
      ta[r] = a;
      tb[r] = b;
      __syncthreads();
      for (int sft = 256; sft > 0; sft >>= 1) {
        if (r < sft) {
          ta[r] += ta[r + sft];
          tb[r] += tb[r + sft];
        }
        __syncthreads();
      }
      if (r == 0) {
        q.scal[0] = ta[0];
        q.scal[1] = tb[0];
      }
    }
  }
}

template <typename T>
__device__ __forceinline__ void chain_fupdate(const ChainArgs<T>& q, T* S, int c, int g) {
  typedef T T2 __attribute__((ext_vector_type(2)));
  const int tid = threadIdx.x, lane = tid & 63;
  const int w = __builtin_amdgcn_readfirstlane(tid >> 6);
  const int64_t ld = q.ld;
  T* z = S;
  if (tid < 128) z[tid] = q.y[int64_t(c) * TILE + tid];
  __syncthreads();
  const int lo = g * q.fgs > c + 2 ? g * q.fgs : c + 2;
  const int hi = (g + 1) * q.fgs < q.R ? (g + 1) * q.fgs : q.R;
  for (int i = lo + w; i < hi; i += 8) {
    const T* Lic = q.A0 + int64_t(c) * TILE * ld + int64_t(i) * TILE + 2 * lane;
    T a0 = 0, a1 = 0;
#pragma unroll 1
    for (int j0 = 0; j0 < TILE; j0 += 16) {
      T2 v[16];
#pragma unroll
      for (int j = 0; j < 16; ++j) v[j] = *reinterpret_cast<const T2*>(Lic + int64_t(j0 + j) * ld);
#pragma unroll
      for (int j = 0; j < 16; ++j) {
        a0 += v[j].x * z[j0 + j];
        a1 += v[j].y * z[j0 + j];
      }
    }
    T* yi = q.y + int64_t(i) * TILE + 2 * lane;
    st_agent(yi, T(yi[0] - a0));
    st_agent(yi + 1, T(yi[1] - a1));
  }
}

#ifdef TGP_PROBE_WIDE
#define CHAIN_WAVES_PER_EU(T) 2
#else
#define CHAIN_WAVES_PER_EU(T) (sizeof(T) == 8 ? 4 : 3)
#endif
template <typename T>
__global__ __launch_bounds__(512) __attribute__((amdgpu_waves_per_eu(CHAIN_WAVES_PER_EU(T), 4))) void chain_kernel(const ChainArgs<T> q) {
  __shared__ __attribute__((aligned(16))) T S[36 * 256];
  __shared__ T Rs[2 * 16];
  __shared__ T Dg[256];
  __shared__ int s_task[7];
  using acc_t = typename Mfma<T>::acc_t;
  if (threadIdx.x == 0) {
    const int t = atomicAdd(q.ticket, 1);
    s_task[4] = t;
    const ChainTask task = chain_unpack(q.tasks[t]);
    const int kind = task.kind, ti = task.i, tc = task.c, tk = task.k;
    s_task[5] = task.part;
    s_task[6] = task.k0;
    s_task[0] = kind; s_task[1] = ti; s_task[2] = tc; s_task[3] = tk;
  }
  __syncthreads();
  const int kind = __builtin_amdgcn_readfirstlane(s_task[0]);
  const int ti = __builtin_amdgcn_readfirstlane(s_task[1]);
  const int tc = __builtin_amdgcn_readfirstlane(s_task[2]);
  const int tk = __builtin_amdgcn_readfirstlane(s_task[3]);
  if (kind > 8) return;
  long long* st = nullptr;
  if (q.stamps != nullptr) {
    st = q.stamps + int64_t(__builtin_amdgcn_readfirstlane(s_task[4])) * 16;
    if (threadIdx.x == 0) {
      st[0] = kind; st[1] = kind == 1 ? tc : ti; st[2] = tc; st[3] = q.launch | (tk << 8) | (s_task[6] << 16);
      for (int k = 1; k < 12; ++k) st[4 + k] = 0;
    }
    chain_stamp(st, 0);
  }
  const uint32_t E = q.epoch32;
  const bool head_final = q.cb == 0;
  if (kind == 7) {
    const int c = tc;
    const int g = c / q.fgs;
    const bool prev = c > 0 || q.fprev != 0;
    chain_wait_counts(c - 1 > q.cb ? q.ticket + CHAIN_YSTATE_OFF + g : nullptr, c - 1 - q.cb,
                      (c == 0 && head_final) ? nullptr : reinterpret_cast<const int32_t*>(q.flags + c * CHAIN_FLAG_LD + c),
                      int32_t(E + CHAIN_FINAL), c > q.cb ? q.ticket + CHAIN_ZFLAG_OFF + (c - 1) : nullptr, 1, q.info);
    chain_stamp(st, 1);
    chain_fsolve<T>(q, S, c, prev);
    chain_stamp(st, 2);
    asm volatile("s_waitcnt vmcnt(0)" ::: "memory");
    __syncthreads();
    if (threadIdx.x == 0) __hip_atomic_store(q.ticket + CHAIN_ZFLAG_OFF + c, 1, __ATOMIC_RELAXED, __HIP_MEMORY_SCOPE_AGENT);
    chain_stamp(st, 3);
    return;
  }
  if (kind == 8) {
    const int c = tc, g = ti;
    const int target = q.R - c - ((c == 0 && head_final) ? 1 : 0);
    chain_wait_counts(q.ticket + CHAIN_COLCNT_OFF + c, target, q.ticket + CHAIN_ZFLAG_OFF + c, 1,
                      c > q.cb ? q.ticket + CHAIN_YSTATE_OFF + g : nullptr, c - q.cb, q.info);
    chain_stamp(st, 1);
    chain_fupdate<T>(q, S, c, g);
    chain_stamp(st, 2);
    asm volatile("s_waitcnt vmcnt(0)" ::: "memory");
    __syncthreads();
    if (threadIdx.x == 0)
      __hip_atomic_store(q.ticket + CHAIN_YSTATE_OFF + g, c - q.cb + 1, __ATOMIC_RELAXED, __HIP_MEMORY_SCOPE_AGENT);
    chain_stamp(st, 3);
    return;
  }
  if constexpr (sizeof(T) == 8) {
    if (kind == 6) {
      const int i = ti, c = tc, k = tk, k0 = __builtin_amdgcn_readfirstlane(s_task[6]);
      uint32_t* wt = q.flags + i * CHAIN_FLAG_LD + c;
      chain_wait<8>(q.flags + i * CHAIN_FLAG_LD + k, E + CHAIN_FINAL, q.flags + c * CHAIN_FLAG_LD + k, E + CHAIN_FINAL,
                    k0 > q.cb ? wt : nullptr, E + uint32_t(k0), q.info);
      chain_stamp(st, 1);
      chain_update_fast(q, S, i, c, k0, k + 1);
      chain_stamp(st, 2);
      chain_publish(wt, E + uint32_t(k + 1));
      chain_stamp(st, 3);
      return;
    }
  }
  if (kind >= 2 && kind <= 4) {
    const int i = ti, c = tc, k = tk;
    uint32_t* wt = q.flags + i * CHAIN_FLAG_LD + c;
    chain_wait<8>(q.flags + i * CHAIN_FLAG_LD + k, E + CHAIN_FINAL, q.flags + c * CHAIN_FLAG_LD + k, E + CHAIN_FINAL,
                  k > q.cb ? wt : nullptr, E + uint32_t(k), q.info);
    chain_stamp(st, 1);
    if (kind == 2) {
      if constexpr (sizeof(T) == 8) {
        if (q.fast_update) chain_update_fast(q, S, i, c, k, k + 1);
        else chain_update_full<T, 1>(q, S, i, c, k, 0);
      } else {
        chain_update_full<T, 1>(q, S, i, c, k, 0);
      }
    }
    else if (kind == 4) chain_update_full<T, CHAIN_CRIT_PARTS>(q, S, i, c, k, __builtin_amdgcn_readfirstlane(s_task[5]));
    else chain_update_diag<T>(q, S, c, k);
    chain_stamp(st, 2);
    if (kind == 4) {
      asm volatile("s_waitcnt vmcnt(0)" ::: "memory");
      __syncthreads();
      if (threadIdx.x == 0 &&
          __hip_atomic_fetch_add(q.ticket + CHAIN_QCNT_OFF + k, 1, __ATOMIC_RELAXED, __HIP_MEMORY_SCOPE_AGENT) ==
              CHAIN_CRIT_PARTS - 1)
        __hip_atomic_store(wt, E + uint32_t(k + 1), __ATOMIC_RELAXED, __HIP_MEMORY_SCOPE_AGENT);
    } else {
      chain_publish(wt, E + uint32_t(k + 1));
    }
    chain_stamp(st, 3);
    return;
  }
  __builtin_amdgcn_s_setprio(2);
  if (kind == 0) {
    const int i = ti, c = tc;
    uint32_t* wt = q.flags + i * CHAIN_FLAG_LD + c;
    const uint32_t* wl = q.flags + c * CHAIN_FLAG_LD + c;
    if (c > q.cb) chain_wait<4>(wt, E + uint32_t(c), nullptr, 0, nullptr, 0, q.info);
    acc_t V[8];
    chain_load_tile<T>(q, i, c, V);
    if (!(c == 0 && head_final)) chain_wait<4>(wl, E + CHAIN_FINAL, nullptr, 0, nullptr, 0, q.info);
    chain_stamp(st, 1);
    chain_solve<T>(q, S, i, c, V, st, 2);
    chain_publish(wt, E + CHAIN_FINAL, q.ticket + CHAIN_COLCNT_OFF + c);
    chain_stamp(st, 4);
    return;
  }
  const int c = tc;
  T* A = q.A0 + int64_t(c) * TILE * q.ld + int64_t(c) * TILE;
  const int64_t ld = q.ld;
  T* dinv = q.dinv + int64_t(c) * 2048;
  int32_t* info = q.info;
  const int32_t pivot_base = q.pivot_base + c * TILE;
  uint32_t* frow = q.flags + c * CHAIN_FLAG_LD;
  if (kind == 5) {
    acc_t Vx[8];
    if (c - 1 > q.cb) chain_wait<4>(frow + (c - 1), E + uint32_t(c - 1), nullptr, 0, nullptr, 0, q.info);
    chain_load_tile<T>(q, c, c - 1, Vx);
    chain_stamp(st, 1);
    const uint32_t* steps = c - 1 >= 1 ? q.flags + (c - 2) * CHAIN_FLAG_LD + (c - 1) : nullptr;
    int32_t* xstep = q.ticket + CHAIN_XSTEP_OFF + c;
    chain_xsolve_stream<T>(q, S, c, c - 1, Vx, steps, q.flags + (c - 1) * CHAIN_FLAG_LD + (c - 1), E, xstep);
    chain_stamp(st, 3);
    chain_publish(frow + (c - 1), E + CHAIN_FINAL, q.ticket + CHAIN_COLCNT_OFF + (c - 1));
    if (threadIdx.x == 0) __hip_atomic_store(xstep, 8, __ATOMIC_RELAXED, __HIP_MEMORY_SCOPE_AGENT);
    chain_stamp(st, 4);
    return;
  }
  acc_t Vx[8];
  acc_t Cfx[5];
  chain_fold_stream<T>(q, S, c, c - 1, Cfx, c > q.cb ? q.ticket + CHAIN_XSTEP_OFF + c : nullptr);
  chain_stamp(st, 3);
  if (c - 1 > q.cb) chain_wait<1>(frow + c, E + uint32_t(c - 1), nullptr, 0, nullptr, 0, q.info);
  else __syncthreads();
  chain_stamp(st, 5);
  {
    constexpr bool FOLD = true;
    uint32_t* step_word = q.flags + (c - 1) * CHAIN_FLAG_LD + c;
#define POTF2_ST(p, v) st_agent((p), T(v))
#define POTF2_V_IN_REGS Vx
#define POTF2_CF_IN_REGS Cfx
#define POTF2_PRE_SYNC(kb) do { if ((kb) >= 1) asm volatile("s_waitcnt vmcnt(0)" ::: "memory"); } while (0)
#define POTF2_POST_SYNC(kb)                                                                            \
  do {                                                                                                \
    if ((kb) >= 1 && threadIdx.x == 0)                                                                \
      __hip_atomic_store(step_word, E + uint32_t(kb), __ATOMIC_RELAXED, __HIP_MEMORY_SCOPE_AGENT);    \
  } while (0)
#include "potf2_body.inc"
#undef POTF2_POST_SYNC
#undef POTF2_PRE_SYNC
#undef POTF2_CF_IN_REGS
#undef POTF2_V_IN_REGS
#undef POTF2_ST
  }
  chain_stamp(st, 6);
  chain_publish(frow + c, E + CHAIN_FINAL, q.ticket + CHAIN_COLCNT_OFF + c);
  chain_stamp(st, 7);
}

template <typename T>
__global__ __launch_bounds__(256) void dinv_kernel(int64_t n, const T* __restrict__ L, int64_t ld,
                                                   T* __restrict__ dinv) {
  const int64_t t = int64_t(blockIdx.x) * 256 + threadIdx.x;
  const int64_t blk = t >> 4;
  const int c = int(t & 15);
  if (blk * 16 >= n) return;
  const T* D = L + blk * 16 * ld + blk * 16;
  T x[16];
#pragma unroll
  for (int i = 0; i < 16; ++i) {
    T s = (i == c) ? T(1) : T(0);
#pragma unroll
    for (int k = 0; k < i; ++k) s -= D[int64_t(k) * ld + i] * x[k];
    x[i] = s / D[int64_t(i) * ld + i];
  }
#pragma unroll
  for (int i = 0; i < 16; ++i) dinv[blk * 256 + c * 16 + i] = x[i];
}

template <typename T>
__global__ __launch_bounds__(256) __attribute__((amdgpu_waves_per_eu(2))) void trsm_kernel(int64_t m, const T* __restrict__ L, int64_t ldl,
                                                   const T* __restrict__ dinv, T* __restrict__ B,
                                                   int64_t ldb) {
  using M = Mfma<T>;
  using acc_t = typename M::acc_t;
  __builtin_amdgcn_s_setprio(2);
  const int lane = threadIdx.x & 63;
  const int64_t r0 = (int64_t(blockIdx.x) * 4 + (threadIdx.x >> 6)) * 16;
  if (r0 >= m) return;
  const int lrow = lane & 15;
  T* bp = B + r0 + lrow;
  acc_t V[8];
#pragma unroll
  for (int jb = 0; jb < 8; ++jb)
#pragma unroll
    for (int r = 0; r < 4; ++r) V[jb][r] = bp[int64_t(jb * 16 + M::drow(lane, r)) * ldb];
  T Dn[4], Ln[7][4];
#pragma unroll
  for (int s = 0; s < 4; ++s) Dn[s] = dinv[M::drow(lane, s) * 16 + lrow];
#pragma unroll
  for (int jb = 0; jb < 8; ++jb) {
    T Dc[4], Lc[7][4];
#pragma unroll
    for (int s = 0; s < 4; ++s) Dc[s] = Dn[s];
#pragma unroll
    for (int kb = 0; kb < jb; ++kb)
#pragma unroll
      for (int s = 0; s < 4; ++s) Lc[kb][s] = Ln[kb][s];
    if (jb + 1 < 8) {
#pragma unroll
      for (int s = 0; s < 4; ++s) Dn[s] = dinv[(jb + 1) * 256 + M::drow(lane, s) * 16 + lrow];
#pragma unroll
      for (int kb = 0; kb <= jb; ++kb)
#pragma unroll
        for (int s = 0; s < 4; ++s)
          Ln[kb][s] = L[int64_t(kb * 16 + M::drow(lane, s)) * ldl + (jb + 1) * 16 + lrow];
    }
    acc_t acc = V[jb], acc2 = acc_t{0, 0, 0, 0};
#pragma unroll
    for (int kb = 0; kb < jb; ++kb) {
#pragma unroll
      for (int s = 0; s < 4; ++s) {
        if (s & 1) acc2 = M::mma(Lc[kb][s], V[kb][s], acc2);
        else acc = M::mma(Lc[kb][s], V[kb][s], acc);
      }
    }
    acc += acc2;
    acc_t y = acc_t{0, 0, 0, 0}, y2 = acc_t{0, 0, 0, 0};
#pragma unroll
    for (int s = 0; s < 4; ++s) {
      if (s & 1) y2 = M::mma(Dc[s], acc[s], y2);
      else y = M::mma(Dc[s], acc[s], y);
    }
    y += y2;
#pragma unroll
    for (int r = 0; r < 4; ++r) bp[int64_t(jb * 16 + M::drow(lane, r)) * ldb] = y[r];
    V[jb] = -y;
  }
}

template <typename T>
__global__ __launch_bounds__(128) void trsv_diag_fwd_kernel(const T* __restrict__ Lkk,
                                                            int64_t ld,
                                                            const T* __restrict__ dinv,
                                                            T* __restrict__ y) {
  __shared__ T st[128];
  __shared__ T sx[16];
  const int r = threadIdx.x, rb = r >> 4, rl = r & 15;
  T di[16];
#pragma unroll
  for (int q = 0; q < 16; ++q) di[q] = dinv[rb * 256 + q * 16 + rl];
  T cur[16], nxt[16];
#pragma unroll
  for (int q = 0; q < 16; ++q) cur[q] = (rb > 0) ? Lkk[int64_t(q) * ld + r] : T(0);
  T t = y[r];
#pragma unroll
  for (int jb = 0; jb < 8; ++jb) {
    if (jb + 1 < 7) {
#pragma unroll
      for (int q = 0; q < 16; ++q)
        nxt[q] = (rb > jb + 1) ? Lkk[int64_t((jb + 1) * 16 + q) * ld + r] : T(0);
    }
    st[r] = t;
    __syncthreads();
    if (rb == jb) {
      T x = 0;
#pragma unroll
      for (int q = 0; q < 16; ++q) x += di[q] * st[jb * 16 + q];
      sx[rl] = x;
      t = x;
    }
    __syncthreads();
    if (jb < 7) {
      if (rb > jb) {
#pragma unroll
        for (int q = 0; q < 16; ++q) t -= cur[q] * sx[q];
      }
#pragma unroll
      for (int q = 0; q < 16; ++q) cur[q] = nxt[q];
    }
  }
  y[r] = t;
}

template <typename T>
__global__ __launch_bounds__(128, 1) void trsv_diag_bwd_kernel(const T* __restrict__ Lkk,
                                                               int64_t ld,
                                                               const T* __restrict__ dinv,
                                                               T* __restrict__ y) {
  __shared__ T st[128];
  __shared__ T sx[16];
  const int c = threadIdx.x, cb = c >> 4, cl = c & 15;
  T Lc[7][16];
#pragma unroll
  for (int jb = 1; jb < 8; ++jb)
#pragma unroll
    for (int q = 0; q < 16; ++q) Lc[jb - 1][q] = (cb < jb) ? Lkk[int64_t(c) * ld + jb * 16 + q] : T(0);
  T di[16];
#pragma unroll
  for (int q = 0; q < 16; ++q) di[q] = dinv[cb * 256 + cl * 16 + q];
  T t = y[c];
#pragma unroll
  for (int jb = 7; jb >= 0; --jb) {
    st[c] = t;
    __syncthreads();
    if (cb == jb) {
      T x = 0;
#pragma unroll
      for (int q = 0; q < 16; ++q) x += di[q] * st[jb * 16 + q];
// ... 357 lines not shown
    if (tid < 128) {
      PollClock xclk;
      for (long spin = 0; xb == Sent<T>::value && !xclk.expired(spin); ++spin) {
        if (spin) __builtin_amdgcn_s_sleep(1);
        xb = load_x_bits<T>(x + int64_t(c) * 128 + tid);
      }
      sx[slot][tid] = bits_to<T>(xb);
    }
    __syncthreads();
    if (tid < 128) xb = (next == 1) ? load_x_bits<T>(x + int64_t(c - 2) * 128 + tid) : Sent<T>::value;
    const T x0 = sx[slot][2 * rq], x1 = sx[slot][2 * rq + 1];
#pragma unroll
    for (int j = 0; j < NC; ++j) acc[j] += cur[j].x * x0 + cur[j].y * x1;
  };
  auto finish = [&](T2 (&wf)[NC]) {
#pragma unroll
    for (int j = 0; j < NC; ++j) redT[cg][j][rq] = acc[j];
    __syncthreads();
    {
      const int jj = tid >> 2, h = tid & 3;
      const T* src = &redT[jj / NC][jj % NC][16 * h];
      T s0 = 0, s1 = 0;
#pragma unroll
      for (int l = 0; l < 16; l += 2) {
        s0 += src[l];
        s1 += src[l + 1];
      }
      red[h][jj] = s0 + s1;
    }
    __syncthreads();
    if (helper) {
      if (tid < 128) {
        const T pv = (red[0][tid] + red[1][tid]) + (red[2][tid] + red[3][tid]);
        bits_t out;
        __builtin_memcpy(&out, &pv, sizeof(T));
        if (out == Sent<T>::value) out ^= 1;
        __hip_atomic_store(reinterpret_cast<bits_t*>(part + int64_t(b) * 128 + tid), out, __ATOMIC_RELAXED,
                           __HIP_MEMORY_SCOPE_AGENT);
      }
      return;
    }
    if (tid < 128) {
      T pv = T(0);
      if (b + 2 <= nblk - 1) {
        bits_t pb = Sent<T>::value;
        PollClock pclk;
        for (long spin = 0; pb == Sent<T>::value && !pclk.expired(spin); ++spin) {
          if (spin) __builtin_amdgcn_s_sleep(1);
          pb = load_x_bits<T>(part + int64_t(b) * 128 + tid);
        }
        pv = bits_to<T>(pb);
      }
      sr[tid] = (zin[int64_t(b) * 128 + tid] - ((red[0][tid] + red[1][tid]) + (red[2][tid] + red[3][tid]))) - pv;
    }
    __syncthreads();
    T p0 = 0, p1 = 0;
#pragma unroll
    for (int j0 = 0; j0 < NC; j0 += 8) {
#pragma unroll
      for (int j = j0; j < j0 + 8; ++j) {
        const T rj = sr[NC * cg + j];
        p0 += wf[j].x * rj;
        p1 += wf[j].y * rj;
      }
      __builtin_amdgcn_sched_barrier(0);
    }
    __syncthreads();
    red[cg][2 * rq] = p0;
    red[cg][2 * rq + 1] = p1;
    __syncthreads();
    if (tid < 128) {
      const T xv = ((red[0][tid] + red[1][tid]) + (red[2][tid] + red[3][tid])) +
                   ((red[4][tid] + red[5][tid]) + (red[6][tid] + red[7][tid]));
      bits_t out;
      __builtin_memcpy(&out, &xv, sizeof(T));
      if (out == Sent<T>::value) out ^= 1;
      __hip_atomic_store(reinterpret_cast<bits_t*>(x + int64_t(b) * 128 + tid), out, __ATOMIC_RELAXED,
                         __HIP_MEMORY_SCOPE_AGENT);
    }
  };
  const int last = helper ? b + 2 : b + 1;
  if (last > nblk - 1) {
    if (helper) return;
    load_w(bufA);
    finish(bufA);
    return;
  }
  const int cnt = (nblk - 1 - last) / 2 + 1;
  int c = last + 2 * (cnt - 1), left = cnt;
  load_tile(bufA, c);
  for (; left > 2; left -= 2, c -= 4) {
    step(c, bufA, bufB, 1);
    step(c - 2, bufB, bufA, 1);
  }
  const int tail_next = helper ? 0 : 2;
  if (left == 2) {
    step(c, bufA, bufB, 1);
    step(c - 2, bufB, bufA, tail_next);
    finish(bufA);
  } else {
    step(c, bufA, bufB, tail_next);
    finish(bufB);
  }
}

}

int run_deferred_asm(tgp_ctx* ctx, hipStream_t behind) {
  if (!ctx->deferred_asm) return TGP_OK;
  auto f = std::move(ctx->deferred_asm);
  ctx->deferred_asm = nullptr;
  if (behind != nullptr && ctx->asm_stream != nullptr) {
    if (ctx->ev_asm_gate == nullptr) TGP_HIP_TRY(hipEventCreateWithFlags(&ctx->ev_asm_gate, hipEventDisableTiming));
    TGP_HIP_TRY(hipEventRecord(ctx->ev_asm_gate, behind));
    TGP_HIP_TRY(hipStreamWaitEvent(ctx->asm_stream, ctx->ev_asm_gate, 0));
  }
  return f();
}

static std::atomic<int64_t> g_poll_ms_host{4000};
int64_t poll_limit_ms() { return g_poll_ms_host.load(); }
int set_poll_limit(tgp_ctx* ctx, int64_t ms) {
  TGP_ARG_CHECK(ms >= 1 && ms <= 3600000, "poll_timeout_ms must be in [1, 3600000]");
  const long long ticks = (long long)ms * 100000LL;
  TGP_HIP_TRY(hipMemcpyToSymbol(HIP_SYMBOL(g_poll_limit), &ticks, sizeof(ticks)));
  g_poll_ms_host.store(ms);
  ctx->poll_timeout_ms = ms;
  return TGP_OK;
}

int join_bounded(tgp_ctx* ctx, hipStream_t st, int64_t n) {
  TGP_TRY(ev_record(ctx, ctx->ev_join, st));
  const auto t0 = std::chrono::steady_clock::now();
  const double budget_ms = double(poll_limit_ms()) + 3.0 * (double(n) * double(n) * double(n) / 3.0) / 2e13 * 1e3;
  for (long spin = 0;; ++spin) {
    const hipError_t e = hipEventQuery(ctx->ev_join);
    if (e == hipSuccess) return TGP_OK;
    if (e != hipErrorNotReady) {
      set_error("hipEventQuery failed: %s", hipGetErrorString(e));
      return TGP_E_HIP;
    }
    (void)hipGetLastError();
    if (ctx->fault_inject == 1) {
      ctx->fault_inject = 0;
      break;
    }
    if ((spin & 63) != 63) continue;
    const double ms = std::chrono::duration<double, std::milli>(std::chrono::steady_clock::now() - t0).count();
    if (ms > budget_ms) break;
    if (ms > 50.0) std::this_thread::sleep_for(std::chrono::microseconds(200));
  }
  if (ctx->rescue_stream == nullptr) TGP_HIP_TRY(hipStreamCreateWithFlags(&ctx->rescue_stream, hipStreamNonBlocking));
  for (int c = 0; c < CHAIN_FLAG_LD; ++c)
    (void)hipStreamWriteValue32(ctx->rescue_stream, ctx->d_chain_ticket + CHAIN_COLCNT_OFF + c, 0x7fffffffu, 0);
  for (hipStream_t q : {ctx->rescue_stream, ctx->asm_stream, ctx->panel_stream, ctx->update_stream, ctx->solve_stream, ctx->stream})
    if (q) (void)hipStreamSynchronize(q);
  (void)hipGetLastError();
  set_error("potrf: the followers of a chain launch were still waiting after %.0f ms (stream wait-values released by the host)", budget_ms);
  return TGP_E_TIMEOUT;
}

template <typename T>
int launch_potf2(tgp_ctx* ctx, hipStream_t st, T* A, int64_t ld, T* dinv, int32_t* info,
                 int32_t pivot_base, const T* Xp, int64_t ldx) {
  if (ctx->trace) {
    trace_push(ctx, 1, st, trace_off(ctx, A), trace_off(ctx, Xp), ld);
    return TGP_OK;
  }
  const int32_t* wc = ctx->potf2_wait_counter;
  const int32_t wt = (int32_t)ctx->potf2_wait_target;
  ctx->potf2_wait_counter = nullptr;
  if (Xp != nullptr)
    hipLaunchKernelGGL((potf2_kernel<T, true>), dim3(1), dim3(512), 0, st, A, ld, dinv, info, pivot_base, Xp, ldx, wc, wt);
  else
    hipLaunchKernelGGL((potf2_kernel<T, false>), dim3(1), dim3(512), 0, st, A, ld, dinv, info, pivot_base, Xp, ldx, wc, wt);
  TGP_HIP_TRY(hipGetLastError());
  return TGP_OK;
}

template <typename T>
int launch_trsm(tgp_ctx* ctx, hipStream_t st, int64_t m, const T* L, int64_t ldl, const T* dinv,
                T* B, int64_t ldb) {
  if (m == 0) return TGP_OK;
  TGP_ARG_CHECK(m % 16 == 0, "trsm: m must be a multiple of 16");
  if (ctx->trace) {
    trace_push(ctx, 2, st, trace_off(ctx, L), trace_off(ctx, B), m, ldl);
    return TGP_OK;
  }
  hipLaunchKernelGGL((trsm_kernel<T>), dim3((unsigned)((m + 63) / 64)), dim3(256), 0, st, m, L,
                     ldl, dinv, B, ldb);
  TGP_HIP_TRY(hipGetLastError());
  return TGP_OK;
}

template <typename T>
int launch_panel_step(tgp_ctx* ctx, hipStream_t st, int64_t m, T* Ljj, int64_t ld, T* dj, int32_t* info,
                      int32_t pivot_base, const T* Xp, bool has_p) {
  TGP_ARG_CHECK(m >= 0 && m % TILE == 0, "panel step: rows below must be a multiple of %d", TILE);
  if (ctx->trace) {
    trace_push(ctx, 10, st, trace_off(ctx, Ljj), trace_off(ctx, Xp), m, ld, has_p ? 1 : 0);
    return TGP_OK;
  }
  const unsigned grid = (unsigned)(m / TILE) + (has_p ? 1u : 0u);
  if (grid == 0) return TGP_OK;
  const uint32_t epoch = ++ctx->step_epoch;
  if (Xp != nullptr)
    hipLaunchKernelGGL((panel_step_kernel<T, true>), dim3(grid), dim3(512), 0, st, Ljj, ld, dj, info, pivot_base,
                       Xp, has_p ? 1 : 0, ctx->d_step_flag, epoch);
  else
    hipLaunchKernelGGL((panel_step_kernel<T, false>), dim3(grid), dim3(512), 0, st, Ljj, ld, dj, info, pivot_base,
                       Xp, has_p ? 1 : 0, ctx->d_step_flag, epoch);
  TGP_HIP_TRY(hipGetLastError());
  return TGP_OK;
}

template <typename T>
ChainPolicy chain_policy(const tgp_ctx* ctx) {
  if (sizeof(T) != 8 || ctx->chain_batch <= 1) return ChainPolicy{1, 1, 2, 0};
  return ChainPolicy{(int)ctx->chain_batch, (int)ctx->chain_batch_lag, (int)ctx->chain_batch_rowlag, (int)ctx->chain_batch_minrows};
}

template <typename T>
int launch_chain(tgp_ctx* ctx, hipStream_t st, T* A0, int64_t ld, T* dinv0, int64_t pivot_base, int64_t R,
                 int64_t nblk, int64_t cb, int64_t ce, bool head_done, hipEvent_t counters_ready, T* y0, bool fprev) {
  TGP_ARG_CHECK(R >= 1 && R <= CHAIN_MAX_ROW_TILES && cb >= 0 && cb < ce && ce <= nblk && nblk <= CHAIN_FLAG_LD && nblk <= R,
                "chain: bad panel shape (R=%lld, columns [%lld, %lld))", (long long)R, (long long)cb, (long long)ce);
  if (cb == 0 && !head_done) {
    TGP_TRY(launch_potf2<T>(ctx, st, A0, ld, dinv0, ctx->d_info, (int32_t)pivot_base));
    if (!ctx->trace) TGP_TRY(run_deferred_asm(ctx, st));
  }
  if (ctx->chain_polls_pending) {
    TGP_TRY(st_wait(ctx, st, ctx->ev_f));
    ctx->chain_polls_pending = false;
  }
  const int fwd = y0 != nullptr ? 1 : 0;
  int red = 0;
  if (fwd != 0 && ctx->chain_red_total > 0 && ctx->chain_red_total <= CHAIN_MAX_ROW_TILES && pivot_base % TILE == 0) {
    red = 1;
    ctx->chain_red_written += ce - cb;
    if (pivot_base / TILE + ce == ctx->chain_red_total && ctx->chain_red_written == ctx->chain_red_total) {
      red = 2;
      ctx->reductions_done = true;
    }
  }
  if (ctx->trace) {
    if (counters_ready != nullptr) TGP_TRY(ev_record(ctx, counters_ready, st));
    trace_push(ctx, 11, st, trace_off(ctx, A0), ld, R, cb, ce, nblk, fwd, red);
    return TGP_OK;
  }
  const ChainPolicy pol = chain_policy<T>(ctx);
  const std::array<int64_t, 9> key = {R, nblk, cb, ce, pol.batch, pol.lag, pol.rowlag, pol.minrows, fwd};
  auto found = ctx->chain_tables.find(key);
  if (found == ctx->chain_tables.end()) {
    const std::vector<ChainTask> list = chain_build((int)R, (int)nblk, (int)cb, (int)ce, pol, fwd, CHAIN_FWD_GROUP);
    tgp_ctx::ChainTable tab;
    tab.count = (int64_t)list.size();
    if (tab.count > 0) {
      std::vector<uint64_t> words(list.size());
      for (size_t u = 0; u < list.size(); ++u) words[u] = chain_pack(list[u]);
      TGP_HIP_TRY(hipMalloc((void**)&tab.dev, words.size() * sizeof(uint64_t)));
      TGP_HIP_TRY(hipMemcpy(tab.dev, words.data(), words.size() * sizeof(uint64_t), hipMemcpyHostToDevice));
    }
    found = ctx->chain_tables.emplace(key, tab).first;
  }
  const int64_t tasks = found->second.count;
  if (tasks == 0) {
    if (counters_ready != nullptr) TGP_TRY(ev_record(ctx, counters_ready, st));
    return TGP_OK;
  }
  ctx->step_epoch = (ctx->step_epoch + 1) & 0x1FFFFFFu;
  if (ctx->step_epoch == 0) ctx->step_epoch = 1;
  const uint32_t epoch = ctx->step_epoch;
  ChainArgs<T> q;
  q.A0 = A0; q.ld = ld; q.dinv = dinv0; q.info = ctx->d_info; q.flags = ctx->d_chain_flags;
  q.ticket = ctx->d_chain_ticket; q.epoch32 = epoch * 128u; q.pivot_base = (int32_t)pivot_base; q.R = (int32_t)R;
  q.nblk = (int32_t)nblk;
  q.cb = (int32_t)cb; q.ce = (int32_t)ce;
  q.stamps = nullptr;
  q.launch = (int32_t)ctx->chain_launches++;
  q.fast_update = (int32_t)ctx->chain_fast_update;
  q.tasks = found->second.dev;
  q.y = y0;
  q.fgs = CHAIN_FWD_GROUP;
  q.fprev = fprev ? 1 : 0;
  q.red = red != 0 ? ctx->d_chain_red : nullptr;
  q.scal = red != 0 ? ctx->d_scal : nullptr;
  q.red_total = red == 2 ? (int32_t)ctx->chain_red_total : 0;
  if (ctx->chain_stamps != 0 && ctx->chain_stamp_base + tasks <= CHAIN_STAMP_TASKS) {
    if (ctx->d_chain_stamps == nullptr)
      TGP_HIP_TRY(hipMalloc((void**)&ctx->d_chain_stamps, size_t(CHAIN_STAMP_TASKS) * 16 * sizeof(long long)));
    q.stamps = ctx->d_chain_stamps + ctx->chain_stamp_base * 16;
    ctx->chain_stamp_base += tasks;
  }
  TGP_HIP_TRY(hipMemsetAsync(ctx->d_chain_ticket, 0, size_t(CHAIN_TICKET_WORDS) * sizeof(int32_t), st));
  if (counters_ready != nullptr) TGP_TRY(ev_record(ctx, counters_ready, st));
  const size_t dyn = ctx->chain_lds_pad > 0 ? size_t(ctx->chain_lds_pad) + (sizeof(T) == 4 ? 36 * 256 * 4 : 0) : 0;
  hipLaunchKernelGGL((chain_kernel<T>), dim3((unsigned)tasks), dim3(512), dyn, st, q);
  TGP_HIP_TRY(hipGetLastError());
  return TGP_OK;
}

int launch_chain_poll(tgp_ctx* ctx, hipStream_t st, const void* A0, int64_t ld, int64_t R, int64_t c, bool first_external) {
  if (ctx->trace) {
    trace_push(ctx, 12, st, trace_off(ctx, static_cast<const double*>(A0)), ld, c);
    return TGP_OK;
  }
  const int32_t target = (int32_t)(R - c - ((c == 0 && first_external) ? 1 : 0));
  int32_t* count = ctx->d_chain_ticket + CHAIN_COLCNT_OFF + c;
  if (ctx->chain_polls == 3 && ctx->can_wait_value) {
    ctx->wait_values_inflight = true;
    TGP_HIP_TRY(hipStreamWaitValue32(st, count, (uint32_t)target, hipStreamWaitValueGte, 0xffffffffu));
    return TGP_OK;
  }
  hipLaunchKernelGGL(chain_poll_kernel, dim3(1), dim3(64), 0, st, count, target, ctx->d_info);
  TGP_HIP_TRY(hipGetLastError());
  return TGP_OK;
}

int launch_prefix_poll(tgp_ctx* ctx, hipStream_t st, const int32_t* counter, int64_t target, int64_t c_off, int64_t ld) {
  if (ctx->trace) {
    trace_push(ctx, 13, st, c_off, ld);
    return TGP_OK;
  }
  hipLaunchKernelGGL(chain_poll_kernel, dim3(1), dim3(64), 0, st, counter, (int32_t)target, ctx->d_info);
  TGP_HIP_TRY(hipGetLastError());
  return TGP_OK;
}

template <typename T>
int compute_dinv(tgp_ctx* ctx, int64_t n, const T* L, int64_t ld, T* dinv) {
  if (n == 0) return TGP_OK;
  hipLaunchKernelGGL((dinv_kernel<T>), dim3((unsigned)((n + 255) / 256)), dim3(256), 0,
                     ctx->stream, n, L, ld, dinv);
  TGP_HIP_TRY(hipGetLastError());
  return TGP_OK;
}

template <typename T>
int launch_trsv_fwd_step(tgp_ctx* ctx, hipStream_t st, int64_t m_below, const T* Ljj, int64_t ld,
                         const T* dj, T* yj) {
  if (ctx->trace) {
    trace_push(ctx, 4, st, trace_off(ctx, Ljj), m_below, ld);
    return TGP_OK;
  }
  hipLaunchKernelGGL((trsv_diag_fwd_kernel<T>), dim3(1), dim3(128), 0, st, Ljj, ld, dj, yj);
  if (m_below > 0)
    hipLaunchKernelGGL((trsv_update_fwd_kernel<T>), dim3((unsigned)((m_below + 255) / 256)),
                       dim3(256), 0, st, m_below, Ljj + TILE, ld, yj, yj + TILE);
  TGP_HIP_TRY(hipGetLastError());
  return TGP_OK;
}

namespace {
struct ProfSpan {
  hipEvent_t e0, e1;
  double flops;
};

int prof_event(tgp_ctx* ctx, hipEvent_t* out) {
  if (ctx->ev_used == ctx->ev_pool.size()) {
    hipEvent_t e;
    TGP_HIP_TRY(hipEventCreate(&e));
    ctx->ev_pool.push_back(e);
  }
  *out = ctx->ev_pool[ctx->ev_used++];
  return TGP_OK;
}
}

template <typename T>
int panel_potf2(tgp_ctx* ctx, hipStream_t st, T* A, int64_t ld, T* dinv, int64_t pivot_off,
                int64_t j0, bool pend) {
  return launch_potf2<T>(ctx, st, A + j0 * ld + j0, ld, dinv + (j0 / TILE) * 2048, ctx->d_info,
                         (int32_t)(pivot_off + j0),
                         pend ? (const T*)(A + (j0 - TILE) * ld + j0) : (const T*)nullptr, ld);
}

template <typename T>
int panel_chain(tgp_ctx* ctx, hipStream_t st, int64_t n, T* A, int64_t ld, T* dinv,
                int64_t pivot_off, int64_t k0, int64_t kb, bool head_done, T* y,
                int64_t after_blocks, const std::function<int(hipEvent_t)>& mid, int64_t blk_begin,
                int64_t blk_end) {
  const int64_t j_first = k0 + blk_begin * TILE;
  const int64_t j_stop = blk_end < 0 ? k0 + kb : std::min<int64_t>(k0 + kb, k0 + blk_end * TILE);
  hipStream_t S3 = ctx->update_stream;
  hipStream_t S2 = ctx->solve_on_update != 0 ? S3 : ctx->solve_stream;
  if (ctx->chain_kernel != 0 && kb / TILE <= CHAIN_FLAG_LD && (n - k0) / TILE <= CHAIN_MAX_ROW_TILES) {
    const int64_t nblk = kb / TILE, R = (n - k0) / TILE;
    const int64_t cb = blk_begin, ce = blk_end < 0 ? nblk : std::min<int64_t>(nblk, blk_end);
    T* A0 = A + k0 * ld + k0;
    T* d0 = dinv + (k0 / TILE) * 2048;
    if (cb >= ce) return TGP_OK;
    const bool mid_in = after_blocks > cb && after_blocks <= ce && after_blocks < nblk && R > after_blocks;
    const bool fwd_in = y != nullptr && ctx->chain_fwd_now;
    T* y_follow = fwd_in ? (T*)nullptr : y;
    const bool follow = y_follow != nullptr || mid_in;
    const bool polls = follow && ctx->chain_polls != 0;
    TGP_TRY(launch_chain<T>(ctx, st, A0, ld, d0, pivot_off + k0, R, nblk, cb, ce, head_done && cb == 0,
                            polls ? ctx->ev_d : (hipEvent_t) nullptr, fwd_in ? y + k0 : (T*)nullptr, k0 > 0));
    if (follow && !polls) TGP_TRY(ev_record(ctx, ctx->ev_d, st));
    if (follow) TGP_TRY(st_wait(ctx, S2, ctx->ev_d));
    for (int64_t c = cb; c < ce && follow; ++c) {
      const int64_t j0 = k0 + c * TILE;
      const bool mid_here = mid_in && c + 1 == after_blocks;
      if (y_follow == nullptr && !mid_here) continue;
      if (polls) TGP_TRY(launch_chain_poll(ctx, S2, A0, ld, R, c, cb == 0));
      if (y_follow != nullptr)
        TGP_TRY(launch_trsv_fwd_step<T>(ctx, S2, n - (j0 + TILE), A + j0 * ld + j0, ld, dinv + (j0 / TILE) * 2048,
                                        y + j0));
      if (mid_here) {
        TGP_TRY(ev_record(ctx, ctx->ev_e, S2));
        TGP_TRY(mid(ctx->ev_e));
      }
    }
    if (polls) {
      TGP_TRY(ev_record(ctx, ctx->ev_f, S2));
      ctx->chain_polls_pending = true;
    }
    return TGP_OK;
  }
  if (ctx->fused_step != 0 && blk_begin == 0 && blk_end < 0) {
    hipEvent_t far_ev[2] = {ctx->ev_e, ctx->ev_f};
    const bool gate = ctx->gate_pending;
    ctx->gate_pending = false;
    int64_t q = 0;
    for (int64_t j0 = k0; j0 < k0 + kb; j0 += TILE, ++q) {
      T* Ljj = A + j0 * ld + j0;
      T* dj = dinv + (j0 / TILE) * 2048;
      const bool pend = j0 > k0;
      const bool has_p = pend || !head_done;
      const int64_t mb = n - (j0 + TILE);
      if (q >= 2) TGP_TRY(st_wait(ctx, st, far_ev[q & 1]));
      if (gate && q == 1) TGP_TRY(st_wait(ctx, st, ctx->ev_g1));
      TGP_TRY(launch_panel_step<T>(ctx, st, mb, Ljj, ld, dj, ctx->d_info, (int32_t)(pivot_off + j0),
                                   pend ? (const T*)(A + (j0 - TILE) * ld + j0) : (const T*)nullptr, has_p));
      const int64_t nc = (k0 + kb) - (j0 + 2 * TILE);
      const int64_t mb2 = mb - TILE;
      const bool upd = mb2 > 0 && nc > 0;
      const bool need_mid = after_blocks > 0 && mb > 0 && (k0 + kb) - (j0 + TILE) > 0 &&
                            j0 + TILE == k0 + after_blocks * TILE;
      if (y != nullptr || upd || need_mid) TGP_TRY(ev_record(ctx, ctx->ev_d, st));
      if (upd) {
        TGP_TRY(st_wait(ctx, S3, ctx->ev_d));
        if (gate && q == 0) TGP_TRY(st_wait(ctx, S3, ctx->ev_g2));
        TGP_TRY(launch_gemm_nt<T>(ctx, S3, mb2, nc, TILE, Ljj + 2 * TILE, ld, Ljj + 2 * TILE, ld,
                                  A + (j0 + 2 * TILE) * ld + j0 + 2 * TILE, ld, 1, 0, 1));
        TGP_TRY(ev_record(ctx, far_ev[q & 1], S3));
      }
      if (y != nullptr) {
        if (S2 != S3 || !upd) TGP_TRY(st_wait(ctx, S2, ctx->ev_d));
        TGP_TRY(launch_trsv_fwd_step<T>(ctx, S2, mb, Ljj, ld, dj, y + j0));
      }
      if (need_mid) TGP_TRY(mid(ctx->ev_d));
    }
    return TGP_OK;
  }
  int64_t SB = ctx->sub_panel;
  if (SB < 2 * TILE || SB >= kb || kb % SB != 0 || n - k0 < ctx->sub_panel_min_rows) SB = 0;
  for (int64_t j0 = j_first; j0 < j_stop; j0 += TILE) {
    T* Ljj = A + j0 * ld + j0;
    T* dj = dinv + (j0 / TILE) * 2048;
    const int64_t sub_end = SB > 0 ? k0 + ((j0 - k0) / SB + 1) * SB : k0 + kb;
    const bool sub_first = SB > 0 && j0 > k0 && (j0 - k0) % SB == 0;
    const bool pend = j0 > k0 && !sub_first;
    if (pend || sub_first || !head_done) TGP_TRY(panel_potf2<T>(ctx, st, A, ld, dinv, pivot_off, j0, pend));
    if (pend) TGP_TRY(st_wait(ctx, st, ctx->ev_e));
    const int64_t mb = n - (j0 + TILE);
    if (mb > 0) TGP_TRY(launch_trsm<T>(ctx, st, mb, Ljj, ld, dj, Ljj + TILE, ld));
    const int64_t nc = sub_end - (j0 + TILE);
    const bool upd = mb > 0 && nc > 0;
    const bool need_mid = after_blocks > 0 && mb > 0 && (k0 + kb) - (j0 + TILE) > 0 &&
                          j0 + TILE == k0 + after_blocks * TILE;
    if (y != nullptr || upd || need_mid) TGP_TRY(ev_record(ctx, ctx->ev_d, st));
    if (upd) {
      TGP_TRY(st_wait(ctx, S3, ctx->ev_d));
      TGP_TRY(launch_gemm_nt<T>(ctx, S3, mb, nc, TILE, Ljj + TILE, ld, Ljj + TILE, ld,
                                A + (j0 + TILE) * ld + j0 + TILE, ld, 1, 0, 3));
      TGP_TRY(ev_record(ctx, ctx->ev_e, S3));
    }
    if (y != nullptr) {
      if (S2 != S3 || !upd) TGP_TRY(st_wait(ctx, S2, ctx->ev_d));
      TGP_TRY(launch_trsv_fwd_step<T>(ctx, S2, mb, Ljj, ld, dj, y + j0));
    }
    if (need_mid) TGP_TRY(mid(ctx->ev_d));
    if (SB > 0 && j0 + TILE == sub_end && sub_end < k0 + kb) {
      const int64_t s0 = sub_end - SB, mr = n - sub_end, ncr = k0 + kb - sub_end;
      const T* P = A + s0 * ld + sub_end;
      const int64_t tiles = (mr / TILE) * (ncr / TILE) - (ncr / TILE) * (ncr / TILE - 1) / 2;
      TGP_TRY(launch_gemm_nt<T>(ctx, st, mr, ncr, SB, P, ld, P, ld, A + sub_end * ld + sub_end, ld, 1, 0,
                                tiles <= ctx->first_small_tiles ? 4 : 1));
    }
  }
  return TGP_OK;
}

template <typename T>
int potrf(tgp_ctx* ctx, int64_t n, T* A, int64_t ld, T* dinv, int32_t* info_host, T* y) {
  TGP_ARG_CHECK(n % TILE == 0 && ld >= n, "potrf: n must be a multiple of %d and ld >= n", TILE);
  if (info_host) *info_host = 0;
  if (n == 0) return TGP_OK;
  ctx->potf2_wait_counter = nullptr;
  ctx->prefix_hint_cols = 0;
  ctx->prefix_hint_counter = nullptr;
  ctx->reserve_hint = 0;
  hipStream_t S0 = ctx->stream, S1 = ctx->panel_stream;
  if (ctx->solve_on_update == 0 && y != nullptr) TGP_TRY(ensure_solve_stream(ctx));
  hipStream_t S2 = ctx->solve_on_update != 0 ? ctx->update_stream : ctx->solve_stream;
  if (y != nullptr) {
    TGP_TRY(ev_record(ctx, ctx->ev_c, S0));
    TGP_TRY(st_wait(ctx, S2, ctx->ev_c));
  }
  int64_t NB = ctx->nb_outer;
  if (NB < TILE) NB = TILE;
  NB = NB / TILE * TILE;
  if (!ctx->trace) TGP_HIP_TRY(hipMemsetAsync(ctx->d_info, 0, sizeof(int32_t), S0));
  ctx->chain_stamp_base = 0;
  ctx->chain_launches = 0;
  ctx->chain_polls_pending = false;
  const bool prof_on = ctx->profile != 0 && !ctx->trace;
  std::vector<ProfSpan> spans;
  ctx->ev_used = 0;
  hipEvent_t prof_t0 = nullptr;
  const bool span_dump = prof_on && getenv("TGP_SPAN_DUMP") != nullptr;
  if (prof_on) {
    TGP_TRY(prof_event(ctx, &prof_t0));
    TGP_HIP_TRY(hipEventRecord(prof_t0, S0));
  }

  auto potf2_at = [&](hipStream_t st, int64_t j0, bool pend) -> int {
    return panel_potf2<T>(ctx, st, A, ld, dinv, 0, j0, pend);
  };
  auto panel = [&](hipStream_t st, int64_t k0, int64_t kb, bool head_done, int64_t after_blocks,
                   const std::function<int(hipEvent_t)>& mid) -> int {
    return panel_chain<T>(ctx, st, n, A, ld, dinv, 0, k0, kb, head_done, y, after_blocks, mid);
  };
  const std::function<int(hipEvent_t)> no_mid = [](hipEvent_t) { return TGP_OK; };
  auto trailing = [&](hipStream_t sq, int64_t m, int64_t nn, int64_t kb, const T* P, T* C, int role) -> int {
    ProfSpan sp{};
    const bool prof = prof_on && role != 4 && role != 5;
    if (prof) {
      TGP_TRY(prof_event(ctx, &sp.e0));
      TGP_TRY(prof_event(ctx, &sp.e1));
      TGP_HIP_TRY(hipEventRecord(sp.e0, sq));
    }
    TGP_TRY(launch_gemm_nt<T>(ctx, sq, m, nn, kb, P, ld, P, ld, C, ld, 1, 0, role));
    if (prof) {
      TGP_HIP_TRY(hipEventRecord(sp.e1, sq));
      const double entries = double(nn) * double(m) - double(nn) * double(nn - 1) / 2.0;
      sp.flops = 2.0 * entries * double(kb);
      spans.push_back(sp);
    }
    return TGP_OK;
  };

  auto join_assembly = [&]() -> int {
    TGP_TRY(run_deferred_asm(ctx, nullptr));
    if (ctx->asm_pending) {
      TGP_TRY(st_wait(ctx, S0, ctx->ev_asm));
      ctx->asm_pending = false;
    }
    return TGP_OK;
  };
  auto width = [&](int64_t k0) -> int64_t {
    const int64_t rem = n - k0;
    int64_t w = NB;
    if (k0 == 0 && ctx->nb_first >= TILE) w = ctx->nb_first / TILE * TILE;
    if (ctx->nb_wide_rows > 0 && k0 > 0 && rem >= ctx->nb_wide_rows) w = 2 * NB;
    if (ctx->chain_kernel != 0 && rem <= ctx->chain_full_rows && rem / TILE <= 64) w = rem;
    return rem < w ? rem : w;
  };
  bool all_chain = ctx->chain_kernel != 0;
  for (int64_t k0 = 0; k0 < n && all_chain; k0 += width(k0))
    all_chain = width(k0) / TILE <= CHAIN_FLAG_LD && (n - k0) / TILE <= CHAIN_MAX_ROW_TILES;
  ctx->chain_fwd_now = y != nullptr && ctx->chain_fwd_tasks != 0 && all_chain;
  auto chain_of_panel = [&](hipStream_t st, int64_t k0, int64_t w) -> int {
    const int64_t sp = ctx->chain_sub_panel / TILE * TILE;
    if (sp >= TILE && sp < w && w % sp == 0 && n - k0 > w && n - k0 >= ctx->chain_sub_min_rows) {
      for (int64_t o = 0; o < w; o += sp) {
        if (o > 0) TGP_TRY(potf2_at(st, k0 + o, false));
        TGP_TRY(panel(st, k0 + o, sp, true, 0, no_mid));
        const int64_t c0 = k0 + o + sp;
        if (c0 < k0 + w)
          TGP_TRY(trailing(st, n - c0, k0 + w - c0, sp, A + (k0 + o) * ld + c0, A + c0 * ld + c0, (int)ctx->chain_sub_role));
      }
      return TGP_OK;
    }
    return panel(st, k0, w, true, 0, no_mid);
  };
  const bool la = ctx->lookahead != 0 && S1 != nullptr;
  if (la && ctx->chain_kernel != 0 && ctx->chain_merged != 0) {
    std::vector<int64_t> s0;
    for (int64_t k0 = 0; k0 < n; k0 += width(k0)) s0.push_back(k0);
    s0.push_back(n);
    const int64_t P = (int64_t)s0.size() - 1;
    hipEvent_t ev_chain[2] = {ctx->ev_b, ctx->ev_g1}, ev_pfx[2] = {ctx->ev_g2, ctx->ev_e}, ev_T[2] = {ctx->ev_i, ctx->ev_j};
    const bool asm_side = ctx->asm_pending;
    ctx->asm_pending = false;
    if (P == 1 && !asm_side) {
      TGP_TRY(panel(S0, 0, s0[1] - s0[0], false, 0, no_mid));
      TGP_TRY(run_deferred_asm(ctx, nullptr));
    } else {
    TGP_TRY(ev_record(ctx, ctx->ev_a, S0));
    TGP_TRY(st_wait(ctx, S1, ctx->ev_a));
    TGP_TRY(panel(S1, 0, s0[1] - s0[0], false, 0, no_mid));
    TGP_TRY(run_deferred_asm(ctx, nullptr));
    TGP_TRY(ev_record(ctx, ev_chain[0], S1));
    for (int64_t p = 0; p + 1 < P; ++p) {
      const int64_t kb = s0[p + 1] - s0[p], next = s0[p + 1], wn = s0[p + 2] - s0[p + 1], mt = n - next;
      const T* Pp = A + s0[p] * ld + next;
      T* C = A + next * ld + next;
      TGP_TRY(st_wait(ctx, S0, ev_chain[p & 1]));
      if (p == 0 && asm_side) TGP_TRY(st_wait(ctx, S0, ctx->ev_asm));
      const bool prefix = wn < mt && ctx->chain_polls != 0;
      int32_t* counter = ctx->d_chain_ticket + CHAIN_PREFIX_OFF + (p & 3);
      if (prefix) {
        if (!ctx->trace) TGP_HIP_TRY(hipMemsetAsync(counter, 0, sizeof(int32_t), S0));
        TGP_TRY(ev_record(ctx, ev_pfx[p & 1], S0));
        ctx->prefix_hint_cols = wn;
        ctx->prefix_hint_counter = counter;
      }
      const int64_t t = mt / TILE;
      if (t * (t + 1) / 2 <= ctx->reserve_max_tiles) ctx->reserve_hint = ctx->chain_reserve;
      TGP_TRY(trailing(S0, mt, mt, kb, Pp, C, 0));
      if (!prefix) TGP_TRY(ev_record(ctx, ev_T[p & 1], S0));
      if (prefix) {
        const int64_t tm = mt / TILE, tp = wn / TILE;
        TGP_TRY(st_wait(ctx, S1, ev_pfx[p & 1]));
        if (ctx->trace || ctx->chain_polls == 2) {
          TGP_TRY(launch_prefix_poll(ctx, S1, counter, tp * tm - tp * (tp - 1) / 2, trace_off(ctx, C), ld));
        } else {
          ctx->potf2_wait_counter = counter;
          ctx->potf2_wait_target = tp * tm - tp * (tp - 1) / 2;
        }
      } else {
        TGP_TRY(st_wait(ctx, S1, ev_T[p & 1]));
      }
      if (p == 0 && asm_side) TGP_TRY(st_wait(ctx, S1, ctx->ev_asm));
      TGP_TRY(potf2_at(S1, next, false));
      TGP_TRY(chain_of_panel(S1, next, wn));
      TGP_TRY(ev_record(ctx, ev_chain[(p + 1) & 1], S1));
    }
    TGP_TRY(st_wait(ctx, S0, ev_chain[(P - 1) & 1]));
    }
  } else
  if (la && ctx->chain_kernel != 0 && ctx->chain_depth2 != 0) {
    std::vector<int64_t> s0;
    for (int64_t k0 = 0; k0 < n; k0 += width(k0)) s0.push_back(k0);
    s0.push_back(n);
    const int64_t P = (int64_t)s0.size() - 1;
    hipEvent_t ev_chain[2] = {ctx->ev_b, ctx->ev_g1}, ev_pre[2] = {ctx->ev_g2, ctx->ev_e};
    auto first_role = [&](int64_t m, int64_t nn) -> int {
      const int64_t tiles = (m / TILE) * (nn / TILE) - (nn / TILE) * (nn / TILE - 1) / 2;
      return tiles <= ctx->first_small_tiles ? 4 : 0;
    };
    const bool asm_side = ctx->asm_pending;
    ctx->asm_pending = false;
    TGP_TRY(ev_record(ctx, ctx->ev_a, S0));
    TGP_TRY(st_wait(ctx, S1, ctx->ev_a));
    TGP_TRY(panel(S1, 0, s0[1] - s0[0], false, 0, no_mid));
    TGP_TRY(run_deferred_asm(ctx, nullptr));
    TGP_TRY(ev_record(ctx, ev_chain[0], S1));
    for (int64_t p = 0; p + 1 < P; ++p) {
      const int64_t kb = s0[p + 1] - s0[p], next = s0[p + 1], wn = s0[p + 2] - s0[p + 1], mt = n - next;
      const int64_t t3p = p + 3 <= P ? (n - s0[p + 3 < P ? p + 3 : P]) / TILE : 0;
      const bool pre_waits = ctx->chain_pre_wait != 0 && ctx->chain_depth2 != 2 &&
                             t3p * (t3p + 1) / 2 <= ctx->reserve_max_tiles;
      auto main_part = [&]() -> int {
        TGP_TRY(st_wait(ctx, S0, ev_chain[p & 1]));
        if (p == 0 && asm_side) TGP_TRY(st_wait(ctx, S0, ctx->ev_asm));
        if (p + 2 < P) {
          if (pre_waits) TGP_TRY(st_wait(ctx, S0, ctx->ev_h));
          const int64_t next2 = s0[p + 2], wn2 = s0[p + 3] - s0[p + 2], mt2 = n - next2;
          TGP_TRY(trailing(S0, mt2, wn2, kb, A + s0[p] * ld + next2, A + next2 * ld + next2, first_role(mt2, wn2)));
          TGP_TRY(ev_record(ctx, ev_pre[p & 1], S0));
          const int64_t next3 = s0[p + 3], m3 = n - next3;
          if (m3 > 0) {
            const int64_t t3 = m3 / TILE;
            if (t3 * (t3 + 1) / 2 <= ctx->reserve_max_tiles) ctx->reserve_hint = ctx->chain_reserve;
            TGP_TRY(trailing(S0, m3, m3, kb, A + s0[p] * ld + next3, A + next3 * ld + next3, 0));
          }
        }
        return TGP_OK;
      };
      auto chain_part = [&]() -> int {
        if (p >= 1) TGP_TRY(st_wait(ctx, S1, ev_pre[(p - 1) & 1]));
        if (p == 0 && asm_side) TGP_TRY(st_wait(ctx, S1, ctx->ev_asm));
        const int grole = first_role(mt, wn);
        const bool gsplit = ctx->chain_gate_split != 0 && grole == 4 && mt > TILE && ctx->update_stream != nullptr &&
                            (y == nullptr || ctx->chain_fwd_now || ctx->solve_on_update == 0);
        if (gsplit) {
          hipStream_t S3 = ctx->update_stream;
          TGP_TRY(ev_record(ctx, ctx->ev_i, S1));
          TGP_TRY(st_wait(ctx, S3, ctx->ev_i));
          TGP_TRY(trailing(S3, TILE, TILE, kb, A + s0[p] * ld + next, A + next * ld + next, 4));
          TGP_TRY(potf2_at(S3, next, false));
          TGP_TRY(ev_record(ctx, ctx->ev_j, S3));
          if (pre_waits) TGP_TRY(ev_record(ctx, ctx->ev_h, S3));
          TGP_TRY(trailing(S1, mt, wn, kb, A + s0[p] * ld + next, A + next * ld + next, 5));
          TGP_TRY(st_wait(ctx, S1, ctx->ev_j));
        } else {
          TGP_TRY(trailing(S1, mt, wn, kb, A + s0[p] * ld + next, A + next * ld + next, grole));
          TGP_TRY(potf2_at(S1, next, false));
          if (pre_waits) TGP_TRY(ev_record(ctx, ctx->ev_h, S1));
        }
        TGP_TRY(panel(S1, next, wn, true, 0, no_mid));
        TGP_TRY(ev_record(ctx, ev_chain[(p + 1) & 1], S1));
        return TGP_OK;
      };
      if (ctx->chain_depth2 == 2) {
        TGP_TRY(main_part());
        TGP_TRY(chain_part());
      } else {
        TGP_TRY(chain_part());
        TGP_TRY(main_part());
      }
    }
    TGP_TRY(st_wait(ctx, S0, ev_chain[(P - 1) & 1]));
  } else
  if (!la) {
    TGP_TRY(join_assembly());
    for (int64_t k0 = 0, kb = 0; k0 < n; k0 += kb) {
      kb = ctx->chain_kernel != 0 ? width(k0) : ((n - k0 < NB) ? (n - k0) : NB);
      TGP_TRY(panel(S0, k0, kb, false, 0, no_mid));
      const int64_t next = k0 + kb, mt = n - next;
      if (mt > 0) TGP_TRY(trailing(S0, mt, mt, kb, A + k0 * ld + next, A + next * ld + next, 0));
    }
  } else {
    int64_t k_done = 0;
    auto first_role = [&](int64_t m, int64_t nn) -> int {
      const int64_t tiles = (m / TILE) * (nn / TILE) - (nn / TILE) * (nn / TILE - 1) / 2;
      return tiles <= ctx->first_small_tiles ? 4 : 0;
    };
    {
      const int64_t kb0 = width(0), mt0 = n - kb0;
      const int64_t kbn0 = width(kb0);
      const int64_t split = (mt0 > 0 && ctx->first_split > 0 && ctx->first_split < kb0 / TILE)
                                ? ctx->first_split : 0;
      const std::function<int(hipEvent_t)> early = [&](hipEvent_t ready) -> int {
        TGP_TRY(join_assembly());
        TGP_TRY(st_wait(ctx, S0, ready));
        TGP_TRY(trailing(S0, mt0, kbn0, split * TILE, A + kb0, A + kb0 * ld + kb0, first_role(mt0, kbn0)));
        k_done = split * TILE;
        return TGP_OK;
      };
      TGP_TRY(ev_record(ctx, ctx->ev_a, S0));
      TGP_TRY(st_wait(ctx, S1, ctx->ev_a));
      TGP_TRY(panel(S1, 0, kb0, false, split, early));
      TGP_TRY(ev_record(ctx, ctx->ev_b, S1));
      TGP_TRY(st_wait(ctx, S0, ctx->ev_b));
      TGP_TRY(join_assembly());
    }
    for (int64_t k0 = 0, kb = 0; k0 < n; k0 += kb) {
      kb = width(k0);
      const int64_t next = k0 + kb, mt = n - next;
      if (mt <= 0) break;
      const int64_t kbn = width(next);
      const T* P = A + k0 * ld + next;
      const bool gsplit = ctx->gate_split != 0 && ctx->fused_step != 0 && kbn >= 3 * TILE && mt > 2 * TILE;
      if (!gsplit) {
        TGP_TRY(trailing(S0, mt, kbn, kb - k_done, P + k_done * ld, A + next * ld + next, first_role(mt, kbn)));
        TGP_TRY(potf2_at(S0, next, false));
        TGP_TRY(ev_record(ctx, ctx->ev_a, S0));
      } else {
        const T* Pk = P + k_done * ld;
        const int64_t kk = kb - k_done;
        T* C0 = A + next * ld + next;
        TGP_TRY(trailing(S0, mt, TILE, kk, Pk, C0, first_role(mt, TILE)));
        TGP_TRY(potf2_at(S0, next, false));
        TGP_TRY(ev_record(ctx, ctx->ev_a, S0));
        TGP_TRY(trailing(S0, mt - TILE, TILE, kk, Pk + TILE, C0 + TILE * ld + TILE, first_role(mt - TILE, TILE)));
        TGP_TRY(ev_record(ctx, ctx->ev_g1, S0));
        TGP_TRY(trailing(S0, mt - 2 * TILE, kbn - 2 * TILE, kk, Pk + 2 * TILE, C0 + 2 * TILE * ld + 2 * TILE,
                         first_role(mt - 2 * TILE, kbn - 2 * TILE)));
        TGP_TRY(ev_record(ctx, ctx->ev_g2, S0));
      }
      k_done = 0;
      const int64_t m2 = mt - kbn;
      if (m2 > 0) {
        const int64_t t2 = m2 / TILE;
        if (t2 * (t2 + 1) / 2 <= ctx->reserve_max_tiles) ctx->reserve_hint = ctx->chain_reserve;
        TGP_TRY(trailing(S0, m2, m2, kb, P + kbn, A + (next + kbn) * ld + next + kbn, 0));
      }
      TGP_TRY(st_wait(ctx, S1, ctx->ev_a));
      const int64_t next2 = next + kbn, mt2 = n - next2;
      const int64_t kbn2 = mt2 > 0 ? width(next2) : 0;
// ... 324 lines not shown
```

### tinygp_amd/csrc/tgp_common.h

```cpp
#pragma once

#include <hip/hip_runtime.h>

#include <cstdarg>
#include <cstdint>
#include <cstdio>
#include <chrono>
#include <array>
#include <functional>
#include <map>
#include <mutex>
#include <vector>

#include "../../include/tgp_hip.h"

namespace tgp {

constexpr int TILE = TGP_TILE;
constexpr int SUB = 16;

void set_error(const char* fmt, ...);

#define TGP_HIP_TRY(expr)                                                                  \
  do {                                                                                     \
    hipError_t _e = (expr);                                                                \
    if (_e != hipSuccess) {                                                                \
      ::tgp::set_error("%s failed: %s (%s:%d)", #expr, hipGetErrorString(_e), __FILE__,    \
                       __LINE__);                                                          \
      return (_e == hipErrorOutOfMemory) ? TGP_E_NOMEM : TGP_E_HIP;                        \
    }                                                                                      \
  } while (0)

#define TGP_ARG_CHECK(cond, ...)        \
  do {                                  \
    if (!(cond)) {                      \
      ::tgp::set_error(__VA_ARGS__);    \
      return TGP_E_ARG;                 \
    }                                   \
  } while (0)

#define TGP_TRY(expr)          \
  do {                         \
    int _s = (expr);           \
    if (_s < 0) return _s;     \
  } while (0)

struct KProg {
  int32_t n;
  int32_t op[TGP_KPROG_MAX];
  int32_t metric[TGP_KPROG_MAX];
  double p0[TGP_KPROG_MAX];
  double p1[TGP_KPROG_MAX];
};

int make_kprog(const tgp_kop* prog, int nops, KProg* out);

inline int64_t round_up(int64_t x, int64_t m) { return (x + m - 1) / m * m; }

}

struct tgp_trace_rec {
  int64_t kind;
  int64_t stream;
  int64_t v[8];
};

struct tgp_ctx {
  std::recursive_mutex mu;
  int device = 0;
  hipStream_t stream = nullptr;
  bool own_stream = false;
  hipStream_t panel_stream = nullptr;
  hipStream_t solve_stream = nullptr;
  hipStream_t update_stream = nullptr;
  hipStream_t asm_stream = nullptr;

  hipEvent_t ev_asm = nullptr;
  bool asm_pending = false;
  hipEvent_t ev_a = nullptr, ev_b = nullptr, ev_c = nullptr, ev_d = nullptr, ev_e = nullptr;
  hipEvent_t ev_f = nullptr;
  hipEvent_t ev_g1 = nullptr, ev_g2 = nullptr;
  hipEvent_t ev_h = nullptr;
  hipEvent_t ev_i = nullptr, ev_j = nullptr;
  bool gate_pending = false;
  int64_t nb_outer = 1024;
  int64_t lookahead = 1;
  int64_t dist_solve_aux = 1;
  int64_t solve_on_update = 1;
  std::chrono::steady_clock::time_point submitted;
  int64_t nb_wide_rows = 30000;
  int64_t profile = 0;
  int64_t first_split = 5;
  int64_t stream_trsv = 1;
  int64_t trsv_groups = 0;
  int64_t keep_grad_buffers = 0;
  int64_t first_small_tiles = 1100;
  int64_t fused_step = 0;
  int64_t chain_reserve = 96;
  int64_t reserve_max_tiles = 1200;
  int64_t gate_split = 1;
  int64_t sub_panel = 0;
  int64_t sub_panel_min_rows = 0;
  int64_t nb_first = 0;
  int64_t split_tail = 0;
  int64_t gemm_role = 1;
  int64_t gemm_reserve = 0;
  int64_t gemm_prefix_cols = 0;
  int64_t gemm_prefix_count = 0;
  int32_t* d_gemm_prefix_count = nullptr;
  int64_t late_join = 1;
  int64_t chain_reduce = 1;
  double* d_chain_red = nullptr;
  int64_t chain_red_total = 0;
  int64_t chain_red_written = 0;
  bool reductions_done = false;
  bool defer_join = false;
  bool join_deferred = false;
  int64_t reserve_hint = 0;
  int64_t prefix_hint_cols = 0;
  int32_t* prefix_hint_counter = nullptr;
  const int32_t* potf2_wait_counter = nullptr;
  int64_t potf2_wait_target = 0;
  uint32_t* d_step_flag = nullptr;
  uint32_t step_epoch = 0;
  int64_t chain_kernel = 1;
  uint32_t* d_chain_flags = nullptr;
  int32_t* d_chain_ticket = nullptr;
  int64_t chain_fast_update = 0;
  int64_t chain_batch = 1;
  int64_t chain_batch_lag = 1;
  int64_t chain_batch_rowlag = 4;
  int64_t chain_batch_minrows = 32;
  struct ChainTable {
    uint64_t* dev = nullptr;
    int64_t count = 0;
  };
  std::map<std::array<int64_t, 9>, ChainTable> chain_tables;
  int64_t chain_full_rows = 4096;
  int64_t chain_depth2 = 1;
  int64_t chain_merged = 1;
  int64_t chain_sub_panel = 0;
  int64_t chain_sub_min_rows = 0;
  int64_t chain_sub_role = 4;
  int64_t kmat_plain_div = 0;
  int64_t chain_polls = 1;
  int64_t chain_fwd_tasks = 1;
  bool chain_fwd_now = false;
  bool wait_values_inflight = false;
  int64_t tile_band = 8;
  int64_t asm_defer = 0;
  std::function<int()> deferred_asm;
  hipEvent_t ev_asm_gate = nullptr;
  int64_t fault_inject = 0;
  int64_t host_join = 1;
  bool serializing_tool = false;
  hipStream_t rescue_stream = nullptr;
  hipEvent_t ev_join = nullptr;
  bool has_device = false;
  bool can_wait_value = false;
  int64_t poll_timeout_ms = 4000;
  int64_t timeout_retries = 0;
  int64_t chain_pre_wait = 0;
  int64_t chain_gate_split = 0;
  int64_t chain_lds_pad = 10240;
  int64_t chain_stamps = 0;
  long long* d_chain_stamps = nullptr;
  int64_t chain_stamp_base = 0;
  int64_t chain_launches = 0;
  bool chain_polls_pending = false;
  double* d_scal = nullptr;
  int32_t* d_info = nullptr;
  void* d_dinv = nullptr;
  size_t dinv_bytes = 0;
  void* d_gemm_ws = nullptr;
  size_t gemm_ws_bytes = 0;
  void* d_work = nullptr;
  bool small_lds_raised = false;
  bool small_grad_lds_raised = false;
  bool small_pred_lds_raised = false;
  bool small_cond_lds_raised = false;
  size_t work_bytes = 0;
  std::vector<hipEvent_t> ev_pool;
  size_t ev_used = 0;
  double prof_syrk_ms = 0, prof_syrk_flops = 0, prof_syrk_union_ms = 0;
  int64_t prof_syrk_launches = 0;
  int cus = 0;
  std::vector<tgp_trace_rec>* trace = nullptr;
  const void* trace_base = nullptr;
};

namespace tgp {

inline int64_t trace_stream_id(const tgp_ctx* ctx, hipStream_t st) {
  if (st == ctx->stream) return 0;
  if (st == ctx->panel_stream) return 1;
  if (st == ctx->solve_stream) return 2;
  if (st == ctx->update_stream) return 3;
  if (st == ctx->asm_stream) return 4;
  return -1;
}
inline int64_t trace_event_id(const tgp_ctx* ctx, hipEvent_t ev) {
  if (ev == ctx->ev_a) return 0;
  if (ev == ctx->ev_b) return 1;
  if (ev == ctx->ev_c) return 2;
  if (ev == ctx->ev_d) return 3;
  if (ev == ctx->ev_e) return 4;
  if (ev == ctx->ev_asm) return 5;
  if (ev == ctx->ev_f) return 6;
  if (ev == ctx->ev_g1) return 7;
  if (ev == ctx->ev_g2) return 8;
  if (ev == ctx->ev_h) return 9;
  if (ev == ctx->ev_i) return 10;
  if (ev == ctx->ev_j) return 11;
  return -1;
}
template <typename T>
inline int64_t trace_off(const tgp_ctx* ctx, const T* p) {
  return p == nullptr ? -1 : int64_t(p - static_cast<const T*>(ctx->trace_base));
}
inline void trace_push(tgp_ctx* ctx, int64_t kind, hipStream_t st, int64_t a = 0, int64_t b = 0,
                       int64_t c = 0, int64_t d = 0, int64_t e = 0, int64_t f = 0, int64_t g = 0,
                       int64_t h = 0) {
  ctx->trace->push_back(tgp_trace_rec{kind, trace_stream_id(ctx, st), {a, b, c, d, e, f, g, h}});
}
inline int ev_record(tgp_ctx* ctx, hipEvent_t ev, hipStream_t st) {
  if (ctx->trace) {
    trace_push(ctx, 5, st, trace_event_id(ctx, ev));
    return TGP_OK;
  }
  TGP_HIP_TRY(hipEventRecord(ev, st));
  return TGP_OK;
}
inline int st_wait(tgp_ctx* ctx, hipStream_t st, hipEvent_t ev) {
  if (ctx->trace) {
    trace_push(ctx, 6, st, trace_event_id(ctx, ev));
    return TGP_OK;
  }
  TGP_HIP_TRY(hipStreamWaitEvent(st, ev, 0));
  return TGP_OK;
}

inline int64_t first_panel_cols(const tgp_ctx* ctx, int64_t n) {
  int64_t w = ctx->nb_outer < TILE ? TILE : ctx->nb_outer / TILE * TILE;
  if (ctx->nb_first >= TILE) w = ctx->nb_first / TILE * TILE;
  if (ctx->chain_kernel != 0 && n <= ctx->chain_full_rows && n / TILE <= 64) w = n;
  return n < w ? n : w;
}

inline void reductions_begin(tgp_ctx* ctx, int64_t npad, bool fused) {
  ctx->chain_red_total = fused && ctx->chain_reduce != 0 ? npad / TILE : 0;
  ctx->chain_red_written = 0;
  ctx->reductions_done = false;
}
inline bool reductions_end(tgp_ctx* ctx) {
  const bool launch = !ctx->reductions_done;
  ctx->chain_red_total = 0;
  ctx->chain_red_written = 0;
  ctx->reductions_done = false;
  return launch;
}

int ensure_dinv(tgp_ctx* ctx, size_t bytes);
int ensure_work(tgp_ctx* ctx, size_t bytes);
int ensure_solve_stream(tgp_ctx* ctx);

template <typename T>
int launch_kmat(tgp_ctx* ctx, const KProg& kp, int64_t n1, int64_t n2, int d, const T* X1,
                const T* X2, const T* diag, T* out, int64_t ld, int64_t rows_out, int64_t cols_out,
                int flags);
template <typename T>
int launch_kmat_cols(tgp_ctx* ctx, hipStream_t st, const KProg& kp, int64_t n1, int64_t n2, int d,
                     const T* X1, const T* X2, const T* diag, T* out, int64_t ld, int64_t rows_out,
                     int64_t cols_out, int flags, int64_t tc0, int64_t ntc);
constexpr int KMAT_LOWER = 1;
constexpr int KMAT_PAD_IDENTITY = 2;
constexpr int KMAT_PLAIN_DIV = 4;

template <typename T>
int launch_kdiag(tgp_ctx* ctx, const KProg& kp, int64_t n, int d, const T* X, const T* add, T* out);
template <typename T>
int launch_kmat_gemv(tgp_ctx* ctx, const KProg& kp, int64_t n1, int64_t n2, int d, const T* X1,
                     const T* X2, const T* v, T* out);
template <typename T>
int launch_kmat_gemv_multi(tgp_ctx* ctx, const KProg& kp, int64_t n1, int64_t n2, int d, const T* X1,
                           const T* X2, const T* v, int64_t nv, T* out);

template <typename T>
int launch_gemm_nt(tgp_ctx* ctx, hipStream_t st, int64_t m, int64_t n, int64_t k, const T* A,
                   int64_t lda, const T* B, int64_t ldb, T* C, int64_t ldc, int lower, int mode,
                   int role);

template <typename T>
int launch_gemm_tri(tgp_ctx* ctx, hipStream_t st, int64_t m, int64_t n, int64_t k, const T* A, int64_t lda,
                    const T* B, int64_t ldb, T* C, int64_t ldc, int lower, int mode, int batch, int64_t sA,
                    int64_t sB, int64_t sC);

template <typename T>
int launch_gemm_nt_dist(tgp_ctx* ctx, hipStream_t st, int64_t n_rows, int64_t nb, int64_t k,
                        const T* P, int64_t ldp, T* Cloc, int64_t ldc, int G, int rank, int64_t l0,
                        int64_t nloc, int64_t reserve = 0);

template <typename T>
int launch_potf2(tgp_ctx* ctx, hipStream_t st, T* A, int64_t ld, T* dinv, int32_t* info,
                 int32_t pivot_base, const T* Xp = nullptr, int64_t ldx = 0);
template <typename T>
int launch_trsm(tgp_ctx* ctx, hipStream_t st, int64_t m, const T* L, int64_t ldl, const T* dinv,
                T* B, int64_t ldb);
template <typename T>
int launch_panel_step(tgp_ctx* ctx, hipStream_t st, int64_t m, T* Ljj, int64_t ld, T* dj, int32_t* info,
                      int32_t pivot_base, const T* Xp, bool has_p);

constexpr int64_t CHAIN_MAX_ROW_TILES = 4096;
constexpr int64_t CHAIN_STAMP_TASKS = 32768;
template <typename T>
int launch_chain(tgp_ctx* ctx, hipStream_t st, T* A0, int64_t ld, T* dinv0, int64_t pivot_base, int64_t R,
                 int64_t nblk, int64_t cb, int64_t ce, bool head_done, hipEvent_t counters_ready = nullptr,
                 T* y0 = nullptr, bool fprev = false);
int launch_chain_poll(tgp_ctx* ctx, hipStream_t st, const void* A0, int64_t ld, int64_t R, int64_t c, bool first_external);
int launch_prefix_poll(tgp_ctx* ctx, hipStream_t st, const int32_t* counter, int64_t target, int64_t c_off, int64_t ld);
int set_poll_limit(tgp_ctx* ctx, int64_t ms);
int64_t poll_limit_ms();
int join_bounded(tgp_ctx* ctx, hipStream_t st, int64_t n);
int run_deferred_asm(tgp_ctx* ctx, hipStream_t behind);
template <typename T>
// ... 70 lines not shown
```

Before: 39.97 evals/s.

## Replace per-launch counter memsets with monotonic epoch-based counters and merged readback

Chain ticket, column-count, prefix and step counters are no longer zeroed with hipMemsetAsync before each chain launch or panel. They now advance monotonically under a host-tracked epoch and ticket base, with wraparound-safe comparisons and a resync only when flagged dirty or near overflow. The info clear is folded into the first potf2 kernel, and the info and scalar readback become one pinned-host copy. This removes several small memset and memcpy operations per evaluation, at the cost of more complex counter bookkeeping and more ways for device and host counter state to fall out of step.

```diff
diff --git a/tinygp_amd/csrc/capi.hip b/tinygp_amd/csrc/capi.hip
--- a/tinygp_amd/csrc/capi.hip
+++ b/tinygp_amd/csrc/capi.hip
@@ -193,8 +193,10 @@
   TGP_HIP_TRY(hipEventCreateWithFlags(&ctx->ev_join, hipEventDisableTiming));
   TGP_HIP_TRY(hipEventCreateWithFlags(&ctx->ev_a, hipEventDisableTiming));
   TGP_HIP_TRY(hipEventCreateWithFlags(&ctx->ev_b, hipEventDisableTiming));
-  TGP_HIP_TRY(hipMalloc(&ctx->d_scal, 16 * sizeof(double)));
-  TGP_HIP_TRY(hipMalloc(&ctx->d_info, sizeof(int32_t)));
+  TGP_HIP_TRY(hipMalloc(&ctx->d_info, 17 * sizeof(double)));
+  TGP_HIP_TRY(hipMemset(ctx->d_info, 0, 17 * sizeof(double)));
+  ctx->d_scal = reinterpret_cast<double*>(ctx->d_info) + 1;
+  TGP_HIP_TRY(hipHostMalloc((void**)&ctx->h_eval, 3 * sizeof(double), hipHostMallocDefault));
   TGP_HIP_TRY(hipMalloc(&ctx->d_step_flag, 64));
   TGP_HIP_TRY(hipMemset(ctx->d_step_flag, 0, 64));
   TGP_HIP_TRY(hipMalloc(&ctx->d_chain_flags, size_t(tgp::CHAIN_MAX_ROW_TILES) * 64 * sizeof(uint32_t)));
@@ -242,8 +244,8 @@
   for (auto e : ctx->ev_pool) hipEventDestroy(e);
   if (ctx->ev_a) hipEventDestroy(ctx->ev_a);
   if (ctx->ev_b) hipEventDestroy(ctx->ev_b);
-  if (ctx->d_scal) hipFree(ctx->d_scal);
   if (ctx->d_info) hipFree(ctx->d_info);
+  if (ctx->h_eval) hipHostFree(ctx->h_eval);
   if (ctx->d_step_flag) hipFree(ctx->d_step_flag);
   if (ctx->d_chain_flags) hipFree(ctx->d_chain_flags);
   if (ctx->d_chain_ticket) hipFree(ctx->d_chain_ticket);
@@ -316,6 +318,8 @@
   if (!strcmp(key, "asm_defer")) return &ctx->asm_defer;
   if (!strcmp(key, "tile_band")) return &ctx->tile_band;
   if (!strcmp(key, "fault_inject")) return &ctx->fault_inject;
+  if (!strcmp(key, "counter_start")) return &ctx->counter_start;
+  if (!strcmp(key, "counter_resyncs")) return &ctx->counter_resyncs;
   if (!strcmp(key, "poll_timeout_ms")) return &ctx->poll_timeout_ms;
   if (!strcmp(key, "timeout_retries")) return &ctx->timeout_retries;
   return nullptr;
@@ -332,7 +336,10 @@
   if (slot == &ctx->chain_batch_lag) TGP_ARG_CHECK(value >= 1 && value <= 64, "chain_batch_lag must be in [1, 64]");
   if (slot == &ctx->chain_batch_minrows) TGP_ARG_CHECK(value >= 0 && value <= 4096, "chain_batch_minrows must be in [0, 4096]");
   if (slot == &ctx->chain_batch_rowlag) TGP_ARG_CHECK(value >= 2 && value <= 4096, "chain_batch_rowlag must be in [2, 4096]");
+  if (slot == &ctx->counter_start)
+    TGP_ARG_CHECK(value >= 0 && value <= 0xf8000000LL, "counter_start must be in [0, 2^32 - 2^27]");
   if (old) *old = *slot;
+  ctx->counters.dirty = true;
   if (slot == &ctx->poll_timeout_ms && ctx->has_device) return set_poll_limit(ctx, value);
   *slot = value;
   return TGP_OK;
@@ -521,8 +528,11 @@
   const bool counted = ctx->gemm_role == 0 && ctx->gemm_prefix_cols > 0;
   if (ctx->gemm_role == 0) ctx->reserve_hint = ctx->gemm_reserve;
   if (counted) {
-    if (!ctx->d_gemm_prefix_count) TGP_HIP_TRY(hipMalloc(&ctx->d_gemm_prefix_count, sizeof(int32_t)));
-    TGP_HIP_TRY(hipMemsetAsync(ctx->d_gemm_prefix_count, 0, sizeof(int32_t), ctx->stream));
+    if (!ctx->d_gemm_prefix_count) {
+      TGP_HIP_TRY(hipMalloc(&ctx->d_gemm_prefix_count, sizeof(int32_t)));
+      TGP_HIP_TRY(hipMemset(ctx->d_gemm_prefix_count, 0, sizeof(int32_t)));
+      ctx->gemm_prefix_base = 0;
+    }
     ctx->prefix_hint_cols = ctx->gemm_prefix_cols;
     ctx->prefix_hint_counter = ctx->d_gemm_prefix_count;
   }
@@ -538,7 +548,8 @@
     int32_t done = 0;
     TGP_HIP_TRY(hipStreamSynchronize(ctx->stream));
     TGP_HIP_TRY(hipMemcpy(&done, ctx->d_gemm_prefix_count, sizeof(int32_t), hipMemcpyDeviceToHost));
-    ctx->gemm_prefix_count = done;
+    ctx->gemm_prefix_count = (int64_t)(int32_t)((uint32_t)done - ctx->gemm_prefix_base);
+    ctx->gemm_prefix_base = (uint32_t)done;
   }
   return rc;
 }
@@ -661,6 +672,7 @@
     for (hipStream_t q : {ctx->asm_stream, ctx->panel_stream, ctx->update_stream, ctx->solve_stream, ctx->stream})
       if (q) (void)hipStreamSynchronize(q);
     (void)hipGetLastError();
+    ctx->counters.dirty = true;
     ctx->asm_pending = false;
     ctx->deferred_asm = nullptr;
     ctx->ev_used = 0;
@@ -670,6 +682,7 @@
     st = factor_body(s, prog, nops, cov_host, info, fused, resid_host, logprob);
     ctx->chain_kernel = keep;
   }
+  if (st != TGP_OK) s->ctx->counters.dirty = true;
   if (st < 0) {
     tgp_ctx* ctx = s->ctx;
     ctx->asm_pending = false;
@@ -743,13 +756,13 @@
     return TGP_OK;
   });
   if (status < 0) return status;
-  double two[2] = {0, 0};
-  int32_t inf_late = 0;
   const bool late = ctx->join_deferred;
   ctx->join_deferred = false;
-  TGP_HIP_TRY(hipMemcpyAsync(two, ctx->d_scal, 2 * sizeof(double), hipMemcpyDeviceToHost, ctx->stream));
-  if (late) TGP_HIP_TRY(hipMemcpyAsync(&inf_late, ctx->d_info, sizeof(int32_t), hipMemcpyDeviceToHost, ctx->stream));
+  TGP_HIP_TRY(hipMemcpyAsync(ctx->h_eval, ctx->d_info, 3 * sizeof(double), hipMemcpyDeviceToHost, ctx->stream));
   TGP_HIP_TRY(hipStreamSynchronize(ctx->stream));
+  const double two[2] = {ctx->h_eval[1], ctx->h_eval[2]};
+  int32_t inf_late = 0;
+  memcpy(&inf_late, ctx->h_eval, sizeof(int32_t));
   if (late) {
     if (inf_late == INT32_MIN) {
       tgp::set_error("potrf: a device-side hand-off did not arrive within poll_timeout_ms (a lost or starved chain launch)");
diff --git a/tinygp_amd/csrc/chain_counters.h b/tinygp_amd/csrc/chain_counters.h
--- /dev/null
+++ b/tinygp_amd/csrc/chain_counters.h
@@ -0,0 +1,43 @@
+#pragma once
+#include <cstdint>
+
+namespace tgp {
+
+struct ChainCounters {
+  static constexpr uint32_t COUNT_SPAN = 8192;
+  static constexpr uint32_t RESYNC_MARGIN = 1u << 28;
+  static constexpr int PREFIX_WORDS = 4;
+
+  uint32_t epoch = 0;
+  uint32_t ticket_base = 0;
+  uint32_t prefix_base[PREFIX_WORDS] = {0, 0, 0, 0};
+  bool dirty = true;
+  uint32_t start = 0;
+
+  static bool reached(uint32_t seen, uint32_t target) { return int32_t(seen - target) >= 0; }
+  static bool near_limit(uint32_t v) { return v >= 0u - RESYNC_MARGIN; }
+
+  bool needs_resync() const {
+    if (dirty || near_limit(epoch) || near_limit(ticket_base)) return true;
+    for (uint32_t b : prefix_base)
+      if (near_limit(b)) return true;
+    return false;
+  }
+  uint32_t resync() {
+    epoch = start & ~(COUNT_SPAN - 1);
+    ticket_base = start;
+    for (uint32_t& b : prefix_base) b = start;
+    dirty = false;
+    return start;
+  }
+  uint32_t next_epoch() { return epoch += COUNT_SPAN; }
+  uint32_t take_tickets(uint32_t tasks) {
+    const uint32_t base = ticket_base;
+    ticket_base += tasks;
+    return base;
+  }
+  uint32_t prefix_target(int q, uint32_t tiles) { return prefix_base[q & (PREFIX_WORDS - 1)] += tiles; }
+  uint32_t release_value() const { return epoch + (COUNT_SPAN - 1); }
+};
+
+}
diff --git a/tinygp_amd/csrc/chol.hip b/tinygp_amd/csrc/chol.hip
--- a/tinygp_amd/csrc/chol.hip
+++ b/tinygp_amd/csrc/chol.hip
@@ -96,10 +96,15 @@
                                                     int32_t* __restrict__ info,
                                                     int32_t pivot_base,
                                                     const T* __restrict__ Xp, int64_t ldx,
-                                                    const int32_t* __restrict__ wait_count, int32_t wait_target) {
+                                                    const int32_t* __restrict__ wait_count, int32_t wait_target,
+                                                    int32_t clear_info) {
   __shared__ __attribute__((aligned(16))) T S[36 * 256];
   __shared__ T Rs[2 * 16];
   __shared__ T Dg[256];
+  if (clear_info != 0) {
+    if (threadIdx.x == 0) atomicExch(info, 0);
+    __syncthreads();
+  }
   if (wait_count != nullptr) {
     if (threadIdx.x == 0) potf2_prefix_wait(wait_count, wait_target, info);
     __syncthreads();
@@ -354,6 +359,8 @@
   uint32_t* flags;
   int32_t* ticket;
   uint32_t epoch32;
+  uint32_t cnt_epoch;
+  uint32_t ticket_base;
   int32_t pivot_base;
   int32_t R;
   int32_t nblk;
@@ -369,6 +376,15 @@
   double* scal;
   int32_t red_total;
 };
+
+__device__ __forceinline__ bool count_reached(int32_t seen, int32_t target) {
+  return int32_t(uint32_t(seen) - uint32_t(target)) >= 0;
+}
+__device__ __forceinline__ int32_t count_arrive(int32_t* word, uint32_t ce) {
+  uint32_t* w = reinterpret_cast<uint32_t*>(word);
+  (void)__hip_atomic_fetch_max(w, ce, __ATOMIC_RELAXED, __HIP_MEMORY_SCOPE_AGENT);
+  return int32_t(__hip_atomic_fetch_add(w, 1u, __ATOMIC_RELAXED, __HIP_MEMORY_SCOPE_AGENT) - ce);
+}
 
 template <int NAP>
 __device__ __forceinline__ void chain_wait(const uint32_t* f0, uint32_t v0, const uint32_t* f1, uint32_t v1,
@@ -397,19 +413,19 @@
   __syncthreads();
 }
 
-__device__ __forceinline__ void chain_publish(uint32_t* word, uint32_t value, int32_t* colcnt = nullptr) {
+__device__ __forceinline__ void chain_publish(uint32_t* word, uint32_t value, int32_t* colcnt = nullptr, uint32_t ce = 0) {
   asm volatile("s_waitcnt vmcnt(0)" ::: "memory");
   __syncthreads();
   if (threadIdx.x == 0) {
     __hip_atomic_store(word, value, __ATOMIC_RELAXED, __HIP_MEMORY_SCOPE_AGENT);
-    if (colcnt != nullptr) __hip_atomic_fetch_add(colcnt, 1, __ATOMIC_RELAXED, __HIP_MEMORY_SCOPE_AGENT);
+    if (colcnt != nullptr) (void)count_arrive(colcnt, ce);
   }
 }
 
 __device__ void potf2_prefix_wait(const int32_t* count, int32_t target, int32_t* info) {
   PollClock clk;
   for (unsigned spin = 0;; ++spin) {
-    if (__hip_atomic_load(count, __ATOMIC_RELAXED, __HIP_MEMORY_SCOPE_AGENT) >= target) break;
+    if (count_reached(__hip_atomic_load(count, __ATOMIC_RELAXED, __HIP_MEMORY_SCOPE_AGENT), target)) break;
     __builtin_amdgcn_s_sleep(8);
     if ((spin & 255) == 255 && (clk.expired(spin) || poisoned(info))) {
       atomicExch(info, STEP_TIMEOUT);
@@ -424,7 +440,7 @@
   if (threadIdx.x != 0) return;
   PollClock clk;
   for (unsigned spin = 0;; ++spin) {
-    if (__hip_atomic_load(count, __ATOMIC_RELAXED, __HIP_MEMORY_SCOPE_AGENT) >= target) break;
+    if (count_reached(__hip_atomic_load(count, __ATOMIC_RELAXED, __HIP_MEMORY_SCOPE_AGENT), target)) break;
     __builtin_amdgcn_s_sleep(16);
     if ((spin & 255) == 255 && (clk.expired(spin) || poisoned(info))) {
       atomicExch(info, STEP_TIMEOUT);
@@ -861,7 +877,7 @@
   PollClock clk;
   for (unsigned spin = 0;; ++spin) {
     const int v = __hip_atomic_load(p, __ATOMIC_RELAXED, __HIP_MEMORY_SCOPE_AGENT);
-    if (v >= want) return v;
+    if (count_reached(v, want)) return v;
     __builtin_amdgcn_s_sleep(1);
     if ((spin & 255) == 255 && (clk.expired(spin) || poisoned(info))) {
       if ((threadIdx.x & 63) == 0) atomicExch(info, STEP_TIMEOUT);
@@ -920,7 +936,8 @@
     }
     if (j >= 1) asm volatile("s_waitcnt vmcnt(0)" ::: "memory");
     chain_lds_barrier();
-    if (j >= 1 && threadIdx.x == 0) __hip_atomic_store(xstep, j, __ATOMIC_RELAXED, __HIP_MEMORY_SCOPE_AGENT);
+    if (j >= 1 && threadIdx.x == 0)
+      __hip_atomic_store(xstep, int32_t(q.cnt_epoch + uint32_t(j)), __ATOMIC_RELAXED, __HIP_MEMORY_SCOPE_AGENT);
     have = j < 7 && known > j + 1;
     if (have) issue_loads(j + 1);
     {
@@ -977,7 +994,9 @@
   for (int j = 0; j < 8; ++j) {
     T* Xc = S + (j & 1) * CS::XC;
     if (!have) {
-      if (known <= j) known = __builtin_amdgcn_readfirstlane(chain_wave_wait_count(xstep, j + 1, q.info));
+      if (known <= j)
+        known = __builtin_amdgcn_readfirstlane(
+            int(uint32_t(chain_wave_wait_count(xstep, int32_t(q.cnt_epoch + uint32_t(j + 1)), q.info)) - q.cnt_epoch));
       issue_loads(j);
     }
 #pragma unroll
@@ -1010,7 +1029,7 @@
     const int want = lane == 0 ? want0 : (lane == 1 ? want1 : want2);
     auto ready = [&]() {
       const int v = __hip_atomic_load(f, __ATOMIC_RELAXED, __HIP_MEMORY_SCOPE_AGENT);
-      return lane == 1 ? v == want : v >= want;
+      return lane == 1 ? v == want : count_reached(v, want);
     };
     bool ok = f == nullptr || ready();
     unsigned spin = 0;
@@ -1186,13 +1205,19 @@
   __shared__ int s_task[7];
   using acc_t = typename Mfma<T>::acc_t;
   if (threadIdx.x == 0) {
-    const int t = atomicAdd(q.ticket, 1);
+    const int t = int(uint32_t(atomicAdd(q.ticket, 1)) - q.ticket_base);
     s_task[4] = t;
-    const ChainTask task = chain_unpack(q.tasks[t]);
-    const int kind = task.kind, ti = task.i, tc = task.c, tk = task.k;
-    s_task[5] = task.part;
-    s_task[6] = task.k0;
-    s_task[0] = kind; s_task[1] = ti; s_task[2] = tc; s_task[3] = tk;
+    if (uint32_t(t) < gridDim.x) {
+      const ChainTask task = chain_unpack(q.tasks[t]);
+      const int kind = task.kind, ti = task.i, tc = task.c, tk = task.k;
+      s_task[5] = task.part;
+      s_task[6] = task.k0;
+      s_task[0] = kind; s_task[1] = ti; s_task[2] = tc; s_task[3] = tk;
+    } else {
+      atomicExch(q.info, STEP_TIMEOUT);
+      s_task[0] = 9; s_task[1] = s_task[2] = s_task[3] = 0;
+      s_task[5] = s_task[6] = 0;
+    }
   }
   __syncthreads();
   const int kind = __builtin_amdgcn_readfirstlane(s_task[0]);
@@ -1210,35 +1235,41 @@
     chain_stamp(st, 0);
   }
   const uint32_t E = q.epoch32;
+  const uint32_t CE = q.cnt_epoch;
   const bool head_final = q.cb == 0;
   if (kind == 7) {
     const int c = tc;
     const int g = c / q.fgs;
     const bool prev = c > 0 || q.fprev != 0;
-    chain_wait_counts(c - 1 > q.cb ? q.ticket + CHAIN_YSTATE_OFF + g : nullptr, c - 1 - q.cb,
+    chain_wait_counts(c - 1 > q.cb ? q.ticket + CHAIN_YSTATE_OFF + g : nullptr, int32_t(CE + uint32_t(c - 1 - q.cb)),
                       (c == 0 && head_final) ? nullptr : reinterpret_cast<const int32_t*>(q.flags + c * CHAIN_FLAG_LD + c),
-                      int32_t(E + CHAIN_FINAL), c > q.cb ? q.ticket + CHAIN_ZFLAG_OFF + (c - 1) : nullptr, 1, q.info);
+                      int32_t(E + CHAIN_FINAL), c > q.cb ? q.ticket + CHAIN_ZFLAG_OFF + (c - 1) : nullptr, int32_t(CE + 1u),
+                      q.info);
     chain_stamp(st, 1);
     chain_fsolve<T>(q, S, c, prev);
     chain_stamp(st, 2);
     asm volatile("s_waitcnt vmcnt(0)" ::: "memory");
     __syncthreads();
-    if (threadIdx.x == 0) __hip_atomic_store(q.ticket + CHAIN_ZFLAG_OFF + c, 1, __ATOMIC_RELAXED, __HIP_MEMORY_SCOPE_AGENT);
+    if (threadIdx.x == 0)
+      __hip_atomic_store(q.ticket + CHAIN_ZFLAG_OFF + c, int32_t(CE + 1u), __ATOMIC_RELAXED, __HIP_MEMORY_SCOPE_AGENT);
     chain_stamp(st, 3);
     return;
   }
   if (kind == 8) {
     const int c = tc, g = ti;
     const int target = q.R - c - ((c == 0 && head_final) ? 1 : 0);
-    chain_wait_counts(q.ticket + CHAIN_COLCNT_OFF + c, target, q.ticket + CHAIN_ZFLAG_OFF + c, 1,
-                      c > q.cb ? q.ticket + CHAIN_YSTATE_OFF + g : nullptr, c - q.cb, q.info);
+    chain_wait_counts(target > 0 ? q.ticket + CHAIN_COLCNT_OFF + c : nullptr, int32_t(CE + uint32_t(target)),
+                      q.ticket + CHAIN_ZFLAG_OFF + c, int32_t(CE + 1u),
+                      c > q.cb ? q.ticket + CHAIN_YSTATE_OFF + g : nullptr, int32_t(CE + uint32_t(c - q.cb)),
+                      q.info);
     chain_stamp(st, 1);
     chain_fupdate<T>(q, S, c, g);
     chain_stamp(st, 2);
     asm volatile("s_waitcnt vmcnt(0)" ::: "memory");
     __syncthreads();
     if (threadIdx.x == 0)
-      __hip_atomic_store(q.ticket + CHAIN_YSTATE_OFF + g, c - q.cb + 1, __ATOMIC_RELAXED, __HIP_MEMORY_SCOPE_AGENT);
+      __hip_atomic_store(q.ticket + CHAIN_YSTATE_OFF + g, int32_t(CE + uint32_t(c - q.cb + 1)), __ATOMIC_RELAXED,
+                         __HIP_MEMORY_SCOPE_AGENT);
     chain_stamp(st, 3);
     return;
   }
@@ -1276,9 +1307,7 @@
     if (kind == 4) {
       asm volatile("s_waitcnt vmcnt(0)" ::: "memory");
       __syncthreads();
-      if (threadIdx.x == 0 &&
-          __hip_atomic_fetch_add(q.ticket + CHAIN_QCNT_OFF + k, 1, __ATOMIC_RELAXED, __HIP_MEMORY_SCOPE_AGENT) ==
-              CHAIN_CRIT_PARTS - 1)
+      if (threadIdx.x == 0 && count_arrive(q.ticket + CHAIN_QCNT_OFF + k, CE) == CHAIN_CRIT_PARTS - 1)
         __hip_atomic_store(wt, E + uint32_t(k + 1), __ATOMIC_RELAXED, __HIP_MEMORY_SCOPE_AGENT);
     } else {
       chain_publish(wt, E + uint32_t(k + 1));
@@ -1297,7 +1326,7 @@
     if (!(c == 0 && head_final)) chain_wait<4>(wl, E + CHAIN_FINAL, nullptr, 0, nullptr, 0, q.info);
     chain_stamp(st, 1);
     chain_solve<T>(q, S, i, c, V, st, 2);
-    chain_publish(wt, E + CHAIN_FINAL, q.ticket + CHAIN_COLCNT_OFF + c);
+    chain_publish(wt, E + CHAIN_FINAL, q.ticket + CHAIN_COLCNT_OFF + c, CE);
     chain_stamp(st, 4);
     return;
   }
@@ -1317,8 +1346,8 @@
     int32_t* xstep = q.ticket + CHAIN_XSTEP_OFF + c;
     chain_xsolve_stream<T>(q, S, c, c - 1, Vx, steps, q.flags + (c - 1) * CHAIN_FLAG_LD + (c - 1), E, xstep);
     chain_stamp(st, 3);
-    chain_publish(frow + (c - 1), E + CHAIN_FINAL, q.ticket + CHAIN_COLCNT_OFF + (c - 1));
-    if (threadIdx.x == 0) __hip_atomic_store(xstep, 8, __ATOMIC_RELAXED, __HIP_MEMORY_SCOPE_AGENT);
+    chain_publish(frow + (c - 1), E + CHAIN_FINAL, q.ticket + CHAIN_COLCNT_OFF + (c - 1), CE);
+    if (threadIdx.x == 0) __hip_atomic_store(xstep, int32_t(CE + 8u), __ATOMIC_RELAXED, __HIP_MEMORY_SCOPE_AGENT);
     chain_stamp(st, 4);
     return;
   }
@@ -1349,7 +1378,7 @@
 #undef POTF2_ST
   }
   chain_stamp(st, 6);
-  chain_publish(frow + c, E + CHAIN_FINAL, q.ticket + CHAIN_COLCNT_OFF + c);
+  chain_publish(frow + c, E + CHAIN_FINAL, q.ticket + CHAIN_COLCNT_OFF + c, CE);
   chain_stamp(st, 7);
 }
 
@@ -2013,7 +2042,7 @@
   }
   if (ctx->rescue_stream == nullptr) TGP_HIP_TRY(hipStreamCreateWithFlags(&ctx->rescue_stream, hipStreamNonBlocking));
   for (int c = 0; c < CHAIN_FLAG_LD; ++c)
-    (void)hipStreamWriteValue32(ctx->rescue_stream, ctx->d_chain_ticket + CHAIN_COLCNT_OFF + c, 0x7fffffffu, 0);
+    (void)hipStreamWriteValue32(ctx->rescue_stream, ctx->d_chain_ticket + CHAIN_COLCNT_OFF + c, ctx->counters.release_value(), 0);
   for (hipStream_t q : {ctx->rescue_stream, ctx->asm_stream, ctx->panel_stream, ctx->update_stream, ctx->solve_stream, ctx->stream})
     if (q) (void)hipStreamSynchronize(q);
   (void)hipGetLastError();
@@ -2029,12 +2058,14 @@
     return TGP_OK;
   }
   const int32_t* wc = ctx->potf2_wait_counter;
-  const int32_t wt = (int32_t)ctx->potf2_wait_target;
+  const int32_t wt = (int32_t)(uint32_t)ctx->potf2_wait_target;
   ctx->potf2_wait_counter = nullptr;
+  const int32_t clr = ctx->info_clear_pending ? 1 : 0;
+  ctx->info_clear_pending = false;
   if (Xp != nullptr)
-    hipLaunchKernelGGL((potf2_kernel<T, true>), dim3(1), dim3(512), 0, st, A, ld, dinv, info, pivot_base, Xp, ldx, wc, wt);
+    hipLaunchKernelGGL((potf2_kernel<T, true>), dim3(1), dim3(512), 0, st, A, ld, dinv, info, pivot_base, Xp, ldx, wc, wt, clr);
   else
-    hipLaunchKernelGGL((potf2_kernel<T, false>), dim3(1), dim3(512), 0, st, A, ld, dinv, info, pivot_base, Xp, ldx, wc, wt);
+    hipLaunchKernelGGL((potf2_kernel<T, false>), dim3(1), dim3(512), 0, st, A, ld, dinv, info, pivot_base, Xp, ldx, wc, wt, clr);
   TGP_HIP_TRY(hipGetLastError());
   return TGP_OK;
 }
@@ -2064,6 +2095,10 @@
   }
   const unsigned grid = (unsigned)(m / TILE) + (has_p ? 1u : 0u);
   if (grid == 0) return TGP_OK;
+  if (ctx->info_clear_pending) {
+    ctx->info_clear_pending = false;
+    TGP_HIP_TRY(hipMemsetAsync(info, 0, sizeof(int32_t), st));
+  }
   const uint32_t epoch = ++ctx->step_epoch;
   if (Xp != nullptr)
     hipLaunchKernelGGL((panel_step_kernel<T, true>), dim3(grid), dim3(512), 0, st, Ljj, ld, dj, info, pivot_base,
@@ -2075,6 +2110,19 @@
   return TGP_OK;
 }
 
+int counters_resync(tgp_ctx* ctx) {
+  if (!ctx->counters.needs_resync()) return TGP_OK;
+  for (hipStream_t q : {ctx->asm_stream, ctx->panel_stream, ctx->update_stream, ctx->solve_stream, ctx->stream})
+    if (q) TGP_HIP_TRY(hipStreamSynchronize(q));
+  ctx->counters.start = (uint32_t)ctx->counter_start;
+  const uint32_t v = ctx->counters.resync();
+  ctx->counter_resyncs++;
+  TGP_HIP_TRY(hipMemsetD32Async((hipDeviceptr_t)ctx->d_chain_ticket, (int)v, size_t(CHAIN_PREFIX_OFF + ChainCounters::PREFIX_WORDS),
+                                ctx->stream));
+  TGP_HIP_TRY(hipStreamSynchronize(ctx->stream));
+  return TGP_OK;
+}
+
 template <typename T>
 ChainPolicy chain_policy(const tgp_ctx* ctx) {
   if (sizeof(T) != 8 || ctx->chain_batch <= 1) return ChainPolicy{1, 1, 2, 0};
@@ -2086,6 +2134,7 @@
                  int64_t nblk, int64_t cb, int64_t ce, bool head_done, hipEvent_t counters_ready, T* y0, bool fprev) {
   TGP_ARG_CHECK(R >= 1 && R <= CHAIN_MAX_ROW_TILES && cb >= 0 && cb < ce && ce <= nblk && nblk <= CHAIN_FLAG_LD && nblk <= R,
                 "chain: bad panel shape (R=%lld, columns [%lld, %lld))", (long long)R, (long long)cb, (long long)ce);
+  if (!ctx->trace && !ctx->in_potrf) TGP_TRY(counters_resync(ctx));
   if (cb == 0 && !head_done) {
     TGP_TRY(launch_potf2<T>(ctx, st, A0, ld, dinv0, ctx->d_info, (int32_t)pivot_base));
     if (!ctx->trace) TGP_TRY(run_deferred_asm(ctx, st));
@@ -2135,6 +2184,8 @@
   ChainArgs<T> q;
   q.A0 = A0; q.ld = ld; q.dinv = dinv0; q.info = ctx->d_info; q.flags = ctx->d_chain_flags;
   q.ticket = ctx->d_chain_ticket; q.epoch32 = epoch * 128u; q.pivot_base = (int32_t)pivot_base; q.R = (int32_t)R;
+  q.cnt_epoch = ctx->counters.next_epoch();
+  q.ticket_base = ctx->counters.take_tickets((uint32_t)tasks);
   q.nblk = (int32_t)nblk;
   q.cb = (int32_t)cb; q.ce = (int32_t)ce;
   q.stamps = nullptr;
@@ -2153,7 +2204,6 @@
     q.stamps = ctx->d_chain_stamps + ctx->chain_stamp_base * 16;
     ctx->chain_stamp_base += tasks;
   }
-  TGP_HIP_TRY(hipMemsetAsync(ctx->d_chain_ticket, 0, size_t(CHAIN_TICKET_WORDS) * sizeof(int32_t), st));
   if (counters_ready != nullptr) TGP_TRY(ev_record(ctx, counters_ready, st));
   const size_t dyn = ctx->chain_lds_pad > 0 ? size_t(ctx->chain_lds_pad) + (sizeof(T) == 4 ? 36 * 256 * 4 : 0) : 0;
   hipLaunchKernelGGL((chain_kernel<T>), dim3((unsigned)tasks), dim3(512), dyn, st, q);
@@ -2166,7 +2216,9 @@
     trace_push(ctx, 12, st, trace_off(ctx, static_cast<const double*>(A0)), ld, c);
     return TGP_OK;
   }
-  const int32_t target = (int32_t)(R - c - ((c == 0 && first_external) ? 1 : 0));
+  const int32_t tiles = (int32_t)(R - c - ((c == 0 && first_external) ? 1 : 0));
+  if (tiles <= 0) return TGP_OK;
+  const int32_t target = (int32_t)(ctx->counters.epoch + (uint32_t)tiles);
   int32_t* count = ctx->d_chain_ticket + CHAIN_COLCNT_OFF + c;
   if (ctx->chain_polls == 3 && ctx->can_wait_value) {
     ctx->wait_values_inflight = true;
@@ -2356,10 +2408,28 @@
 }
 
 template <typename T>
+static int potrf_queue(tgp_ctx* ctx, int64_t n, T* A, int64_t ld, T* dinv, int32_t* info_host, T* y);
+
+template <typename T>
 int potrf(tgp_ctx* ctx, int64_t n, T* A, int64_t ld, T* dinv, int32_t* info_host, T* y) {
   TGP_ARG_CHECK(n % TILE == 0 && ld >= n, "potrf: n must be a multiple of %d and ld >= n", TILE);
   if (info_host) *info_host = 0;
   if (n == 0) return TGP_OK;
+  if (ctx->trace) return potrf_queue<T>(ctx, n, A, ld, dinv, info_host, y);
+  TGP_TRY(counters_resync(ctx));
+  ctx->in_potrf = true;
+  const int rc = potrf_queue<T>(ctx, n, A, ld, dinv, info_host, y);
+  ctx->in_potrf = false;
+  if (ctx->info_clear_pending) {
+    ctx->info_clear_pending = false;
+    if (rc == TGP_OK) TGP_HIP_TRY(hipMemsetAsync(ctx->d_info, 0, sizeof(int32_t), ctx->stream));
+  }
+  if (rc != TGP_OK) ctx->counters.dirty = true;
+  return rc;
+}
+
+template <typename T>
+static int potrf_queue(tgp_ctx* ctx, int64_t n, T* A, int64_t ld, T* dinv, int32_t* info_host, T* y) {
   ctx->potf2_wait_counter = nullptr;
   ctx->prefix_hint_cols = 0;
   ctx->prefix_hint_counter = nullptr;
@@ -2374,7 +2444,7 @@
   int64_t NB = ctx->nb_outer;
   if (NB < TILE) NB = TILE;
   NB = NB / TILE * TILE;
-  if (!ctx->trace) TGP_HIP_TRY(hipMemsetAsync(ctx->d_info, 0, sizeof(int32_t), S0));
+  ctx->info_clear_pending = !ctx->trace;
   ctx->chain_stamp_base = 0;
   ctx->chain_launches = 0;
   ctx->chain_polls_pending = false;
@@ -2474,8 +2544,9 @@
       if (p == 0 && asm_side) TGP_TRY(st_wait(ctx, S0, ctx->ev_asm));
       const bool prefix = wn < mt && ctx->chain_polls != 0;
       int32_t* counter = ctx->d_chain_ticket + CHAIN_PREFIX_OFF + (p & 3);
+      const int64_t pfx_tiles = (wn / TILE) * (mt / TILE) - (wn / TILE) * (wn / TILE - 1) / 2;
+      const int64_t pfx_target = prefix && !ctx->trace ? (int64_t)ctx->counters.prefix_target((int)(p & 3), (uint32_t)pfx_tiles) : pfx_tiles;
       if (prefix) {
-        if (!ctx->trace) TGP_HIP_TRY(hipMemsetAsync(counter, 0, sizeof(int32_t), S0));
         TGP_TRY(ev_record(ctx, ev_pfx[p & 1], S0));
         ctx->prefix_hint_cols = wn;
         ctx->prefix_hint_counter = counter;
@@ -2485,13 +2556,12 @@
       TGP_TRY(trailing(S0, mt, mt, kb, Pp, C, 0));
       if (!prefix) TGP_TRY(ev_record(ctx, ev_T[p & 1], S0));
       if (prefix) {
-        const int64_t tm = mt / TILE, tp = wn / TILE;
         TGP_TRY(st_wait(ctx, S1, ev_pfx[p & 1]));
         if (ctx->trace || ctx->chain_polls == 2) {
-          TGP_TRY(launch_prefix_poll(ctx, S1, counter, tp * tm - tp * (tp - 1) / 2, trace_off(ctx, C), ld));
+          TGP_TRY(launch_prefix_poll(ctx, S1, counter, pfx_target, trace_off(ctx, C), ld));
         } else {
           ctx->potf2_wait_counter = counter;
-          ctx->potf2_wait_target = tp * tm - tp * (tp - 1) / 2;
+          ctx->potf2_wait_target = pfx_target;
         }
       } else {
         TGP_TRY(st_wait(ctx, S1, ev_T[p & 1]));
diff --git a/tinygp_amd/csrc/tgp_common.h b/tinygp_amd/csrc/tgp_common.h
--- a/tinygp_amd/csrc/tgp_common.h
+++ b/tinygp_amd/csrc/tgp_common.h
@@ -13,6 +13,7 @@
 #include <vector>
 
 #include "../../include/tgp_hip.h"
+#include "chain_counters.h"
 
 namespace tgp {
 
@@ -126,6 +127,12 @@
   int64_t chain_kernel = 1;
   uint32_t* d_chain_flags = nullptr;
   int32_t* d_chain_ticket = nullptr;
+  tgp::ChainCounters counters;
+  int64_t counter_resyncs = 0;
+  int64_t counter_start = 0;
+  bool in_potrf = false;
+  bool info_clear_pending = false;
+  uint32_t gemm_prefix_base = 0;
   int64_t chain_fast_update = 0;
   int64_t chain_batch = 1;
   int64_t chain_batch_lag = 1;
@@ -170,6 +177,7 @@
   bool chain_polls_pending = false;
   double* d_scal = nullptr;
   int32_t* d_info = nullptr;
+  double* h_eval = nullptr;
   void* d_dinv = nullptr;
   size_t dinv_bytes = 0;
   void* d_gemm_ws = nullptr;
```

New measurement: 40.04 evals/s (median of 6 runs). No clear change (+0.2%).
